# mimbres/neural-audio-fp

Hardware: AMD Instinct MI355X
Metric: fingerprint generation throughput (1-s segments/s) (higher is better)
Workload: dtype f32

## Files before the change

### include/nafp.h

```cpp
#ifndef NAFP_H
#define NAFP_H

#include <stdint.h>

#ifdef __cplusplus
extern "C" {
#endif

#define NAFP_ABI_VERSION 1

enum {
    NAFP_OK = 0,
    NAFP_ERR_INVALID_ARG = 1,
    NAFP_ERR_UNSUPPORTED = 2,
    NAFP_ERR_HIP = 3,
    NAFP_ERR_WORKSPACE = 4,
    NAFP_ERR_NO_WEIGHTS = 5
};

typedef struct nafp_melspec nafp_melspec;
typedef struct nafp_encoder nafp_encoder;

int nafp_abi_version(void);
const char* nafp_status_string(int status);
// ... 162 lines not shown
    int64_t n_indexed;
    int64_t indexed_samples;
    int32_t rate, channels, bps, min_block, max_block, refusal;
    uint8_t md5[16];
} nafp_flac_info;

typedef struct nafp_flac_index_entry {
    int64_t offset;
    int64_t first_sample;
    int64_t n_bytes;
    int32_t block_size;
    int32_t reserved;
} nafp_flac_index_entry;

typedef struct nafp_flac_frame {
    int64_t raw_off;
    int64_t scratch_off;
    int32_t n_bytes;
    int32_t block_size;
    int32_t channels;
    int32_t bps;
    int32_t rate;
    int32_t reserved;
} nafp_flac_frame;

int nafp_flac_streaminfo_host(const void* bytes, int64_t n_bytes, nafp_flac_info* info);
int nafp_flac_index_host(const void* bytes, int64_t n_bytes, nafp_flac_info* info, nafp_flac_index_entry* frames_out, int64_t cap);
int nafp_flac_decode_host(const void* raw, int64_t raw_size, const nafp_flac_frame* frames_host, int64_t n_frames, void* scratch,
                          int64_t scratch_size, int32_t* status_out);
int nafp_flac_check_frames_host(const nafp_flac_frame* frames_host, int64_t n_frames, int64_t raw_size, int64_t scratch_size);
int nafp_flac_decode(const uint8_t* raw, int64_t raw_size, const nafp_flac_frame* frames_dev, int64_t n_frames, uint8_t* scratch,
                     int64_t scratch_size, int32_t* status_dev, void* stream);


int nafp_encoder_create(nafp_encoder** enc, int in_f, int in_t, int emb_sz);
int nafp_encoder_destroy(nafp_encoder* enc);

#define NAFP_NORM_LAYER2D 0
#define NAFP_NORM_LAYER1D 1
#define NAFP_NORM_BATCH 2
int nafp_encoder_create_ex(nafp_encoder** enc, int in_f, int in_t, int emb_sz, int norm);
int nafp_encoder_norm(const nafp_encoder* enc);
int nafp_encoder_n_trainable(const nafp_encoder* enc);

int nafp_encoder_n_tensors(const nafp_encoder* enc);
int64_t nafp_encoder_tensor_numel(const nafp_encoder* enc, int index);
int nafp_encoder_tensor_shape(const nafp_encoder* enc, int index, int64_t dims_out[4]);
int64_t nafp_encoder_flat_dim(const nafp_encoder* enc);

int nafp_encoder_set_weights(nafp_encoder* enc, const float* const* tensors_host_array,
                             void* stream);

int64_t nafp_encoder_workspace_bytes(const nafp_encoder* enc, int64_t n_seg);

int nafp_encoder_forward(nafp_encoder* enc, const float* feat, int64_t n_seg,
                         void* workspace, int64_t workspace_bytes,
                         float* out_flat, float* out_emb, int l2norm, void* stream);

int nafp_encoder_forward_raw(nafp_encoder* enc, const float* raw_feat, const float* group_stat, int group_size,
                             int segment_norm, int64_t n_seg, void* workspace, int64_t workspace_bytes,
                             float* out_flat, float* out_emb, int l2norm, void* stream);

int64_t nafp_encoder_conv0_numel(const nafp_encoder* enc);
int nafp_encoder_conv0(nafp_encoder* enc, const float* feat, const float* group_stat, int group_size, int segment_norm,
                       int64_t n_seg, float* z0_out, long long* stats_out, void* stream);

#define NAFP_ENCODER_PROFILE_KERNELS 17
int nafp_encoder_profile_enable(nafp_encoder* enc, int max_forwards);
int nafp_encoder_profile_count(const nafp_encoder* enc);
int nafp_encoder_profile_coarse(nafp_encoder* enc, int coarse);
int nafp_encoder_profile_read(nafp_encoder* enc, int slot, float* ms_out_host);
int nafp_conv_timeline(void* dev_buf, int64_t capacity_u64, int cin, int cout, int positions);
int nafp_conv_timeline_grid(int* out5_host);
#define NAFP_CONV_PLAN_FIELDS 30
#define NAFP_PLAN_PLAIN 1
#define NAFP_PLAN_DGRAD 2
#define NAFP_PLAN_V_OUT 4
#define NAFP_PLAN_TICKETS 8
#define NAFP_PLAN_SPLIT_WEIGHTS 16
#define NAFP_PLAN_FUSE0 32
#define NAFP_PLAN_SIZE_DGRAD 64
int nafp_conv_plan(int in_f, int in_t, int layer, int64_t n_seg, int64_t plan_b, int flags, int64_t slab_floats,
                   int64_t* record_host, char* kernel_name_host, int name_capacity);

int64_t nafp_encoder_train_workspace_bytes(const nafp_encoder* enc, int64_t n_seg);
int nafp_encoder_forward_train(nafp_encoder* enc, const float* feat, int64_t n_seg, void* workspace,
                               int64_t workspace_bytes, float* out_emb, int l2norm, void* stream);
int nafp_encoder_backward(nafp_encoder* enc, const float* feat, const float* d_emb, int64_t n_seg,
                          void* workspace, int64_t workspace_bytes, float* const* grads_host_array,
                          int l2norm, void* stream);

#define NAFP_GRAD_GROUPS 4
int nafp_encoder_grad_group_range(const nafp_encoder* enc, int group, int* first_tensor, int* last_tensor);
int nafp_encoder_grad_group_wait(nafp_encoder* enc, int group, void* stream);

#define NAFP_OPT_FUSE_CONV0 1
#define NAFP_OPT_FUSED_LN_BWD 2
#define NAFP_OPT_BWD_OVERLAP 4
#define NAFP_OPT_SMALLNET 5
#define NAFP_OPT_BF16X3 3
#define NAFP_OPT_NONMATRIX 8
#define NAFP_NONMATRIX_CONV0 1
#define NAFP_NONMATRIX_KEEP_OWN 2
#define NAFP_NONMATRIX_ALL 3
#define NAFP_NONMATRIX_DEFAULT NAFP_NONMATRIX_ALL
int nafp_encoder_set_option(nafp_encoder* enc, int option, int value);

int nafp_encoder_div_enc(nafp_encoder* enc, const float* flat, int64_t n_seg,
                         float* out_emb, int l2norm, void* stream);

int nafp_l2_normalize_rows(const float* x, int64_t n_rows, int dim, float* out, void* stream);

int nafp_pack_embedding_grads(const float* d_a_all, const float* d_b_all, const float* loss_sum, float loss_scale,
                              int64_t world, int64_t n_anchors, int dim, float* send, void* stream);


int64_t nafp_ntxent_workspace_bytes(int64_t n_local, int64_t n_global);

int nafp_ntxent_forward(const float* emb_org_local, const float* emb_rep_local,
                        const float* emb_org_all, const float* emb_rep_all,
                        int64_t n_local, int64_t n_global, int64_t rank_offset, int d,
                        float tau, float* loss_sum, float* sim_mtx,
                        float* d_org_all, float* d_rep_all,
                        void* workspace, int64_t workspace_bytes, void* stream);


typedef struct { int f0, f1, t0, t1; } nafp_rect;

int nafp_specaug_apply(float* feat, int64_t n_seg, int F, int T, const nafp_rect* rects_host,
                       int n_rects, const unsigned char* active, float fill_value, void* stream);

int nafp_specaug_apply_fill_dev(float* feat, int64_t n_seg, int F, int T, const nafp_rect* rects_host,
                                int n_rects, const unsigned char* active, const float* fill_value_dev,
                                void* stream);
int64_t nafp_specaug_mean_workspace_bytes(void);
int nafp_specaug_mean(const float* feat, int64_t n, float* mean_out, void* workspace, int64_t workspace_bytes,
                      void* stream);

int nafp_specaug_apply_ex(float* feat, int64_t n_seg, int F, int T, const int32_t* rects_dev, int n_rects, int64_t n_sets,
                          const unsigned char* active_dev, const float* filler, int64_t n_fill_seg,
                          const float* scale_offset_dev, void* stream);
int nafp_specaug_range(const float* feat, int64_t n, float* scale_offset_out, void* workspace, int64_t workspace_bytes,
                       void* stream);


typedef struct {
    float* param; const float* grad; float* m; float* v;
    int64_t numel; int64_t var_len;
} nafp_opt_tensor;

float nafp_cosine_decay_lr_host(float lr0, int64_t step, int64_t decay_steps, float alpha);
float nafp_cosine_decay_restarts_lr_host(float lr0, int64_t step, int64_t first_decay_steps, float t_mul,
                                         float m_mul, float alpha);

int nafp_adam_step(const nafp_opt_tensor* tensors_host, int n, float lr, float beta1, float beta2,
                   float eps, int64_t step, void* stream);

int64_t nafp_lamb_workspace_bytes(const nafp_opt_tensor* tensors_host, int n);
int nafp_lamb_step(const nafp_opt_tensor* tensors_host, int n, float lr, float beta1, float beta2,
                   float eps, float weight_decay, int64_t step, void* workspace,
                   int64_t workspace_bytes, void* stream);

int64_t nafp_triplet_workspace_bytes(int64_t n_anchor, int64_t n_pos);
int nafp_triplet_forward(const float* emb_anchor, const float* emb_pos, int64_t n_anchor, int64_t n_pos, int dim,
                         int mode, float margin, float* loss_out, float* pairwise_dist, float* d_anchor,
                         float* d_pos, void* workspace, int64_t workspace_bytes, void* stream);

typedef struct nafp_aug_row {
    int64_t ev_off;
    int64_t nz_off;
    int64_t nz2_off;
    int64_t ir_off;
    int32_t ev_valid;
    int32_t nz_valid, nz2_valid;
    int32_t ir_len;
    float snr_db;
    float amp;
    int32_t mix;
    int32_t reserved;
} nafp_aug_row;

int nafp_augment_rows(const int16_t* pcm, const nafp_aug_row* rows, int64_t n_rows, int seg_len, float* out,
                      void* stream);


int64_t nafp_search_index_aux_floats(int64_t n_index);
int nafp_search_index_prepare(const float* index, int64_t n_index, int dim, float* aux, void* stream);

// ... 134 lines not shown
```

### neural-audio-fp_amd/_lib.py

```python
import ctypes
import os

import torch

_HERE = os.path.dirname(os.path.abspath(__file__))
LIB_PATH = os.environ.get('NAFP_LIB') or os.path.join(_HERE, 'libnafp.so')

c_i64 = ctypes.c_int64
c_int = ctypes.c_int
c_float = ctypes.c_float
c_void_p = ctypes.c_void_p

PROTOTYPES = {
    'nafp_abi_version': (c_int, []),
    'nafp_status_string': (ctypes.c_char_p, [c_int]),
    'nafp_last_hip_error': (c_int, []),
    'nafp_crc32c_host': (ctypes.c_uint32, [c_void_p, c_i64, ctypes.c_uint32]),
    'nafp_mel_filterbank_host': (c_int, [c_int, c_int, c_int, c_float, c_float, c_void_p]),
    'nafp_melspec_create': (c_int, [ctypes.POINTER(c_void_p), c_int, c_int, c_int, c_int, c_int, c_float, c_float]),
    'nafp_melspec_create_ex': (c_int, [ctypes.POINTER(c_void_p), c_int, c_int, c_int, c_int, c_int, c_float, c_float, c_int]),
    'nafp_melspec_plan_host': (c_int, [c_int, c_int, c_int, c_int, c_int, c_float, c_float, c_int, c_void_p]),
    'nafp_melspec_kernel': (c_int, [c_void_p]),
    'nafp_melspec_destroy': (c_int, [c_void_p]),
    'nafp_melspec_n_frames': (c_int, [c_void_p]),
    'nafp_melspec_n_mels': (c_int, [c_void_p]),
    'nafp_melspec_forward_f32': (c_int, [c_void_p, c_void_p, c_i64, c_int, c_int, c_void_p, c_void_p, c_void_p]),
    'nafp_melspec_forward_i16': (c_int, [c_void_p, c_void_p, c_i64, c_int, c_int, c_void_p, c_void_p, c_void_p]),
    'nafp_melspec_finish': (c_int, [c_void_p, c_void_p, c_void_p, c_i64, c_int, c_int, c_void_p]),
    'nafp_melspec_forward_windows_i16': (c_int, [c_void_p, c_void_p, c_void_p, c_void_p, c_i64, c_int, c_int, c_void_p,
                                                 c_void_p, c_void_p]),
    'nafp_resample_geometry': (c_int, [c_int, c_int, ctypes.POINTER(c_int), ctypes.POINTER(c_int), ctypes.POINTER(c_int),
                                       ctypes.POINTER(c_int)]),
    'nafp_resample_table_host': (c_int, [c_int, c_int, c_void_p]),
    'nafp_resample_n_out': (c_i64, [c_i64, c_int, c_int]),
    'nafp_resample_input_range': (c_int, [c_i64, c_i64, c_i64, c_int, c_int, ctypes.POINTER(c_i64), ctypes.POINTER(c_i64)]),
    'nafp_resample_check_pieces_host': (c_int, [c_int, c_int, c_void_p, c_i64, c_i64, c_i64]),
    'nafp_resample_create': (c_int, [ctypes.POINTER(c_void_p), c_int, c_int]),
    'nafp_resample_destroy': (c_int, [c_void_p]),
    'nafp_resample_i16': (c_int, [c_void_p, c_void_p, c_i64, c_void_p, c_i64, c_void_p, c_i64, c_void_p]),
    'nafp_ingest_geometry': (c_int, [c_int, c_int, ctypes.POINTER(c_int), ctypes.POINTER(c_int), ctypes.POINTER(c_int),
                                     ctypes.POINTER(c_int)]),
    'nafp_ingest_table_host': (c_int, [c_int, c_int, c_void_p]),
    'nafp_ingest_n_out': (c_i64, [c_i64, c_int, c_int]),
    'nafp_ingest_input_range': (c_int, [c_i64, c_i64, c_i64, c_int, c_int, ctypes.POINTER(c_i64), ctypes.POINTER(c_i64)]),
    'nafp_ingest_decode_host': (c_int, [c_int, c_void_p, c_i64, c_void_p]),
    'nafp_ingest_check_pieces_host': (c_int, [c_int, c_int, c_void_p, c_i64, c_i64, c_i64]),
    'nafp_ingest_create': (c_int, [ctypes.POINTER(c_void_p), c_int, c_int]),
    'nafp_ingest_destroy': (c_int, [c_void_p]),
    'nafp_ingest_i16': (c_int, [c_void_p, c_void_p, c_i64, c_void_p, c_i64, c_void_p, c_i64, c_void_p]),
    'nafp_varispeed_geometry': (c_int, [ctypes.c_uint32, ctypes.POINTER(c_int), ctypes.POINTER(c_int)]),
    'nafp_varispeed_table_host': (c_int, [ctypes.c_uint32, c_void_p]),
    'nafp_varispeed_n_out': (c_i64, [c_i64, ctypes.c_uint32]),
    'nafp_varispeed_input_range': (c_int, [c_i64, c_i64, c_i64, ctypes.c_uint32, ctypes.POINTER(c_i64), ctypes.POINTER(c_i64)]),
    'nafp_varispeed_check_pieces_host': (c_int, [ctypes.c_uint32, c_void_p, c_i64, c_i64, c_i64]),
    'nafp_varispeed_create': (c_int, [ctypes.POINTER(c_void_p), ctypes.c_uint32]),
    'nafp_varispeed_destroy': (c_int, [c_void_p]),
    'nafp_varispeed_i16': (c_int, [c_void_p, c_void_p, c_i64, c_void_p, c_i64, c_void_p, c_i64, c_void_p]),
    'nafp_codec_samples_per_block': (c_int, [c_int, c_int, c_int]),
    'nafp_codec_blocks_per_group': (c_int, [c_int, c_int, c_int]),
    'nafp_codec_decode_host': (c_int, [c_int, c_int, c_int, c_void_p, c_i64, c_void_p]),
    'nafp_codec_check_pieces_host': (c_int, [c_void_p, c_i64, c_i64, c_i64]),
    'nafp_codec_decode_i16': (c_int, [c_void_p, c_i64, c_void_p, c_i64, c_void_p, c_i64, c_void_p]),
    'nafp_flac_streaminfo_host': (c_int, [c_void_p, c_i64, c_void_p]),
    'nafp_flac_index_host': (c_int, [c_void_p, c_i64, c_void_p, c_void_p, c_i64]),
    'nafp_flac_decode_host': (c_int, [c_void_p, c_i64, c_void_p, c_i64, c_void_p, c_i64, c_void_p]),
    'nafp_flac_check_frames_host': (c_int, [c_void_p, c_i64, c_i64, c_i64]),
    'nafp_flac_decode': (c_int, [c_void_p, c_i64, c_void_p, c_i64, c_void_p, c_i64, c_void_p, c_void_p]),
    'nafp_encoder_create': (c_int, [ctypes.POINTER(c_void_p), c_int, c_int, c_int]),
    'nafp_encoder_create_ex': (c_int, [ctypes.POINTER(c_void_p), c_int, c_int, c_int, c_int]),
    'nafp_encoder_norm': (c_int, [c_void_p]),
    'nafp_encoder_n_trainable': (c_int, [c_void_p]),
    'nafp_encoder_destroy': (c_int, [c_void_p]),
    'nafp_encoder_n_tensors': (c_int, [c_void_p]),
    'nafp_encoder_tensor_numel': (c_i64, [c_void_p, c_int]),
    'nafp_encoder_tensor_shape': (c_int, [c_void_p, c_int, ctypes.POINTER(c_i64)]),
    'nafp_encoder_flat_dim': (c_i64, [c_void_p]),
    'nafp_encoder_set_weights': (c_int, [c_void_p, ctypes.POINTER(c_void_p), c_void_p]),
    'nafp_encoder_workspace_bytes': (c_i64, [c_void_p, c_i64]),
    'nafp_encoder_forward': (c_int, [c_void_p, c_void_p, c_i64, c_void_p, c_i64, c_void_p, c_void_p, c_int, c_void_p]),
    'nafp_encoder_forward_raw': (c_int, [c_void_p, c_void_p, c_void_p, c_int, c_int, c_i64, c_void_p, c_i64, c_void_p, c_void_p,
                                         c_int, c_void_p]),
    'nafp_encoder_conv0_numel': (c_i64, [c_void_p]),
    'nafp_encoder_conv0': (c_int, [c_void_p, c_void_p, c_void_p, c_int, c_int, c_i64, c_void_p, c_void_p, c_void_p]),
    'nafp_encoder_profile_enable': (c_int, [c_void_p, c_int]),
    'nafp_encoder_profile_count': (c_int, [c_void_p]),
    'nafp_encoder_profile_coarse': (c_int, [c_void_p, c_int]),
    'nafp_encoder_profile_read': (c_int, [c_void_p, c_int, c_void_p]),
    'nafp_conv_timeline': (c_int, [c_void_p, c_i64, c_int, c_int, c_int]),
    'nafp_conv_timeline_grid': (c_int, [c_void_p]),
    'nafp_conv_plan': (c_int, [c_int, c_int, c_int, c_i64, c_i64, c_int, c_i64, c_void_p, c_void_p, c_int]),
    'nafp_encoder_set_option': (c_int, [c_void_p, c_int, c_int]),
    'nafp_encoder_train_workspace_bytes': (c_i64, [c_void_p, c_i64]),
    'nafp_encoder_forward_train': (c_int, [c_void_p, c_void_p, c_i64, c_void_p, c_i64, c_void_p, c_int, c_void_p]),
    'nafp_encoder_backward': (c_int, [c_void_p, c_void_p, c_void_p, c_i64, c_void_p, c_i64,
                                      ctypes.POINTER(c_void_p), c_int, c_void_p]),
    'nafp_encoder_grad_group_range': (c_int, [c_void_p, c_int, ctypes.POINTER(c_int), ctypes.POINTER(c_int)]),
    'nafp_encoder_grad_group_wait': (c_int, [c_void_p, c_int, c_void_p]),
    'nafp_encoder_div_enc': (c_int, [c_void_p, c_void_p, c_i64, c_void_p, c_int, c_void_p]),
    'nafp_ntxent_workspace_bytes': (c_i64, [c_i64, c_i64]),
    'nafp_ntxent_forward': (c_int, [c_void_p, c_void_p, c_void_p, c_void_p, c_i64, c_i64, c_i64, c_int,
                                    c_float, c_void_p, c_void_p, c_void_p, c_void_p, c_void_p, c_i64, c_void_p]),
    'nafp_specaug_apply': (c_int, [c_void_p, c_i64, c_int, c_int, c_void_p, c_int, c_void_p, c_float, c_void_p]),
    'nafp_specaug_apply_fill_dev': (c_int, [c_void_p, c_i64, c_int, c_int, c_void_p, c_int, c_void_p, c_void_p, c_void_p]),
    'nafp_specaug_mean_workspace_bytes': (c_i64, []),
    'nafp_specaug_mean': (c_int, [c_void_p, c_i64, c_void_p, c_void_p, c_i64, c_void_p]),
    'nafp_specaug_apply_ex': (c_int, [c_void_p, c_i64, c_int, c_int, c_void_p, c_int, c_i64, c_void_p, c_void_p, c_i64, c_void_p, c_void_p]),
    'nafp_specaug_range': (c_int, [c_void_p, c_i64, c_void_p, c_void_p, c_i64, c_void_p]),
    'nafp_l2_normalize_rows': (c_int, [c_void_p, c_i64, c_int, c_void_p, c_void_p]),
    'nafp_pack_embedding_grads': (c_int, [c_void_p, c_void_p, c_void_p, c_float, c_i64, c_i64, c_int, c_void_p, c_void_p]),
    'nafp_cosine_decay_lr_host': (c_float, [c_float, c_i64, c_i64, c_float]),
    'nafp_cosine_decay_restarts_lr_host': (c_float, [c_float, c_i64, c_i64, c_float, c_float, c_float]),
    'nafp_adam_step': (c_int, [c_void_p, c_int, c_float, c_float, c_float, c_float, c_i64, c_void_p]),
    'nafp_lamb_workspace_bytes': (c_i64, [c_void_p, c_int]),
    'nafp_triplet_workspace_bytes': (c_i64, [c_i64, c_i64]),
    'nafp_triplet_forward': (c_int, [c_void_p, c_void_p, c_i64, c_i64, c_int, c_int, c_float, c_void_p, c_void_p, c_void_p,
                                     c_void_p, c_void_p, c_i64, c_void_p]),
    'nafp_augment_rows': (c_int, [c_void_p, c_void_p, c_i64, c_int, c_void_p, c_void_p]),
    'nafp_search_index_aux_floats': (c_i64, [c_i64]),
    'nafp_search_index_prepare': (c_int, [c_void_p, c_i64, c_int, c_void_p, c_void_p]),
    'nafp_search_workspace_bytes': (c_i64, [c_i64, c_i64, c_int]),
    'nafp_search_topk_l2': (c_int, [c_void_p, c_i64, c_void_p, c_void_p, c_i64, c_int, c_int, c_void_p, c_void_p,
                                    c_void_p, c_i64, c_void_p]),
    'nafp_search_topk_l2_excl': (c_int, [c_void_p, c_i64, c_void_p, c_void_p, c_i64, c_int, c_int, c_void_p, c_void_p, c_void_p,
                                         c_void_p, c_i64, c_void_p]),
    'nafp_search_seq_scores': (c_int, [c_void_p, c_void_p, c_i64, c_int, c_void_p, c_void_p, c_i64, c_void_p, c_int,
                                       c_void_p, c_void_p]),
    'nafp_search_seq_match': (c_int, [c_void_p, c_i64, c_void_p, c_i64, c_int, c_void_p, c_int, c_void_p, c_void_p, c_i64, c_int,
                                      c_int, c_void_p, c_void_p, c_void_p, c_void_p]),
    'nafp_search_identify': (c_int, [c_void_p, c_i64, c_void_p, c_i64, c_int, c_void_p, c_int, c_void_p, c_void_p, c_i64, c_int,
                                     c_void_p, c_int, c_int, c_int, c_int, c_int, c_void_p, c_void_p, c_void_p, c_void_p, c_void_p,
                                     c_void_p, c_void_p]),
    'nafp_search_identify_check_tracks_host': (c_int, [c_void_p, c_int, c_i64]),
    'nafp_search_identify_tempo': (c_int, [c_void_p, c_i64, c_void_p, c_i64, c_int, c_void_p, c_int, c_void_p, c_void_p, c_i64, c_int,
                                           c_void_p, c_int, c_void_p, c_int, c_int, c_int, c_int, c_int, c_void_p, c_void_p, c_void_p,
                                           c_void_p, c_void_p, c_void_p, c_void_p, c_void_p]),
    'nafp_ivf_bucket_workspace_bytes': (c_i64, [c_i64, c_int, c_int]),
    'nafp_ivf_bucket': (c_int, [c_void_p, c_int, c_i64, c_int, c_int, c_void_p, c_void_p, c_void_p, c_i64, c_void_p]),
    'nafp_ivf_kmeans_update': (c_int, [c_void_p, c_i64, c_int, c_int, c_void_p, c_void_p, c_int, c_void_p, c_void_p, c_void_p]),
    'nafp_ivf_residuals': (c_int, [c_void_p, c_i64, c_int, c_void_p, c_void_p, c_void_p, c_void_p]),
    'nafp_ivf_pq_encode': (c_int, [c_void_p, c_i64, c_int, c_void_p, c_void_p, c_void_p, c_int, c_void_p, c_void_p]),
    'nafp_ivf_probe': (c_int, [c_void_p, c_i64, c_void_p, c_int, c_int, c_int, c_void_p, c_void_p]),
    'nafp_ivf_flat_rows_bound': (c_i64, [c_i64, c_int]),
    'nafp_ivf_flat_lists': (c_int, [c_void_p, c_i64, c_int, c_void_p, c_void_p, c_int, c_void_p, c_void_p, c_void_p, c_void_p,
                                    c_void_p]),
    'nafp_ivf_pq_lists': (c_int, [c_void_p, c_i64, c_int, c_void_p, c_void_p, c_void_p]),
    'nafp_ivf_search_workspace_bytes': (c_i64, [c_i64, c_int, c_int, c_int, c_int]),
    'nafp_ivf_flat_search': (c_int, [c_void_p, c_i64, c_void_p, c_int, c_int, c_int, c_void_p, c_void_p, c_void_p, c_void_p, c_int,
                                     c_void_p, c_void_p, c_void_p, c_i64, c_void_p]),
    'nafp_ivf_pq_search': (c_int, [c_void_p, c_i64, c_void_p, c_int, c_int, c_int, c_void_p, c_int, c_void_p, c_void_p, c_void_p,
                                   c_int, c_void_p, c_void_p, c_void_p, c_i64, c_void_p]),
    'nafp_ivf_pq_search_ex': (c_int, [c_void_p, c_i64, c_void_p, c_int, c_int, c_int, c_void_p, c_int, c_void_p, c_void_p, c_void_p,
                                      c_int, c_void_p, c_void_p, c_int, c_void_p, c_i64, c_void_p]),
    'nafp_ivf_pq_adc_tables': (c_int, [c_void_p, c_i64, c_void_p, c_void_p, c_i64, c_void_p, c_int, c_int, c_void_p, c_int, c_int,
                                       c_void_p, c_void_p]),
    'nafp_ivf_pq_residuals': (c_int, [c_void_p, c_i64, c_int, c_void_p, c_int, c_void_p, c_void_p, c_void_p]),
    'nafp_ivf_refine_encode': (c_int, [c_void_p, c_i64, c_int, c_void_p, c_int, c_int, c_int, c_void_p, c_void_p]),
    'nafp_ivf_pq_wide_workspace_bytes': (c_i64, [c_i64, c_int, c_int, c_int]),
    'nafp_ivf_pq_search_wide': (c_int, [c_void_p, c_i64, c_void_p, c_int, c_int, c_int, c_void_p, c_int, c_void_p, c_void_p, c_void_p,
                                        c_int, c_void_p, c_void_p, c_int, c_void_p, c_i64, c_void_p]),
    'nafp_ivf_pqr_rerank': (c_int, [c_void_p, c_i64, c_int, c_void_p, c_int, c_void_p, c_void_p, c_void_p, c_int, c_void_p, c_void_p,
                                    c_int, c_int, c_void_p, c_i64, c_int, c_void_p, c_void_p, c_void_p]),
    'nafp_ivf_pqr_search': (c_int, [c_void_p, c_i64, c_void_p, c_int, c_int, c_int, c_void_p, c_int, c_void_p, c_void_p, c_void_p,
                                    c_void_p, c_void_p, c_void_p, c_int, c_int, c_void_p, c_i64, c_int, c_int, c_void_p, c_void_p,
                                    c_void_p, c_void_p, c_int, c_void_p, c_i64, c_void_p]),
    'nafp_hnsw_default_max_expansions': (c_int, [c_int]),
    'nafp_hnsw_reverse_workspace_bytes': (c_i64, [c_i64, c_i64, c_int, c_int]),
    'nafp_hnsw_search_workspace_bytes': (c_i64, [c_i64, c_int, c_int]),
    'nafp_hnsw_search_layer': (c_int, [c_void_p, c_i64, c_int, c_void_p, c_void_p, c_i64, c_i64, c_int, c_int, c_void_p, c_i64, c_void_p,
                                       c_void_p, c_int, c_int, c_int, c_void_p, c_void_p, c_void_p]),
    'nafp_hnsw_select_forward': (c_int, [c_void_p, c_i64, c_int, c_i64, c_i64, c_void_p, c_int, c_int, c_void_p, c_void_p, c_int, c_void_p,
                                         c_void_p, c_i64, c_i64, c_void_p]),
    'nafp_hnsw_reverse_links': (c_int, [c_void_p, c_i64, c_int, c_i64, c_i64, c_void_p, c_int, c_int, c_void_p, c_void_p, c_i64, c_i64,
                                        c_void_p, c_i64, c_void_p]),
# ... 96 lines not shown
```

### neural-audio-fp_amd/csrc/api.hip

```cpp
#include "nafp_common.h"

#include <algorithm>
#include <cstdio>
#include <cstdlib>
#include <cstring>
#include <vector>

namespace nafp {

thread_local int g_last_hip_error = 0;

static const int kHiddenCh[8] = {128, 128, 256, 256, 512, 512, 1024, 1024};
static const int kStrideT[8] = {2, 2, 2, 2, 1, 2, 1, 2};

std::vector<ConvGeom> encoder_geometry(int in_f, int in_t) {
    std::vector<ConvGeom> g;
    int F = in_f, T = in_t, C = 1;
    for (int i = 0; i < 8; ++i) {
        SamePad pt = same_pad(T, 3, kStrideT[i]);
        g.push_back(ConvGeom{0, F, T, C, F, pt.n_out, kHiddenCh[i], kStrideT[i], pt.before});
        T = pt.n_out; C = kHiddenCh[i];
        SamePad pf = same_pad(F, 3, 2);
        g.push_back(ConvGeom{1, F, T, C, pf.n_out, T, kHiddenCh[i], 2, pf.before});
        F = pf.n_out;
    }
    return g;
}

struct CopyTable { const float* src[96]; float* dst[96]; int64_t n[96]; int nz[96]; int count; int* nonfinite; };
__device__ __forceinline__ float nz_scale(float g) { return fabsf(g) < 1e-30f ? copysignf(1e-30f, g) : g; }
__device__ __forceinline__ bool nonfinite4(float4 v) {
    return !(fabsf(v.x) <= 3.4028234664e38f) || !(fabsf(v.y) <= 3.4028234664e38f) || !(fabsf(v.z) <= 3.4028234664e38f) || !(fabsf(v.w) <= 3.4028234664e38f);
}
__global__ __launch_bounds__(256) void multi_copy_kernel(const CopyTable t) {
    const int e = blockIdx.y;
    const float* __restrict__ s = t.src[e]; float* __restrict__ d = t.dst[e];
    const int64_t n = t.n[e];
    const bool nz = t.nz[e] != 0;
    bool bad = false;
    if ((((uintptr_t)s | (uintptr_t)d) & 15) == 0) {
        for (int64_t i = blockIdx.x * 256ll + threadIdx.x; i < n / 4; i += (int64_t)gridDim.x * 256) {
            float4 v = ((const float4*)s)[i];
            bad = bad || nonfinite4(v);
            if (nz) { v.x = nz_scale(v.x); v.y = nz_scale(v.y); v.z = nz_scale(v.z); v.w = nz_scale(v.w); }
            ((float4*)d)[i] = v;
        }
        for (int64_t i = n / 4 * 4 + blockIdx.x * 256ll + threadIdx.x; i < n; i += (int64_t)gridDim.x * 256) {
            bad = bad || !(fabsf(s[i]) <= 3.4028234664e38f);
            d[i] = nz ? nz_scale(s[i]) : s[i];
        }
    } else {
        for (int64_t i = blockIdx.x * 256ll + threadIdx.x; i < n; i += (int64_t)gridDim.x * 256) {
            bad = bad || !(fabsf(s[i]) <= 3.4028234664e38f);
            d[i] = nz ? nz_scale(s[i]) : s[i];
        }
    }
    if (bad && t.nonfinite) atomicOr(t.nonfinite, 1);
}
#define NAFP_OPT_DEBUG_SIDE_DELAY 6
#define NAFP_OPT_DEBUG_SW_DELAY 7
__global__ void debug_delay_kernel(long long us) {
    const unsigned long long t0 = __builtin_amdgcn_s_memrealtime();
    while ((long long)(__builtin_amdgcn_s_memrealtime() - t0) < us * 100) __builtin_amdgcn_s_sleep(32);
}
struct BiasTable { float* hb[16]; const float* bias[16]; int64_t n[16]; int cout[16]; int count; };
__global__ __launch_bounds__(256) void add_bias_kernel(const BiasTable t) {
    const int e = blockIdx.y;
    float* __restrict__ h = t.hb[e]; const float* __restrict__ b = t.bias[e];
    const int64_t n = t.n[e]; const int C = t.cout[e];
    for (int64_t i = blockIdx.x * 256ll + threadIdx.x; i < n; i += (int64_t)gridDim.x * 256) h[i] += b[i % C];
}

}

using namespace nafp;

constexpr int NAFP_PROF_EV = 34;
struct nafp_encoder {
    int in_f, in_t, emb_sz;
    int norm = NAFP_NORM_LAYER2D;
    int n_trainable = 68;
    std::vector<float*> d_gc, d_bc, d_mm, d_mv;
    bool ln1d_images_set = false;
    std::vector<ConvGeom> geom;
    int64_t flat_dim; int S;
    std::vector<std::vector<int64_t>> shapes;
    float* d_blob = nullptr;
    int64_t blob_floats = 0;
    std::vector<float*> d_w;
    std::vector<float*> d_bias, d_gamma, d_beta;
    std::vector<float*> d_G, d_Hb;
    float *d_w1p = nullptr, *d_b1p = nullptr, *d_w2p = nullptr, *d_b2 = nullptr;
    std::vector<float*> d_wd;
    float *d_w1k = nullptr, *d_b1k = nullptr, *d_w2k = nullptr;
    double* d_inv_n = nullptr;
    int* d_wflag = nullptr;
    float* d_sw_slab = nullptr; int64_t sw_slab_floats = 0;
    bool has_weights = false;
    hipEvent_t sw_copied = nullptr, sw_l1 = nullptr, sw_done = nullptr;
    hipStream_t sw_stream = nullptr;
    bool sw_recorded = false;
    bool opt_fuse_conv0 = []() { const char* v = getenv("NAFP_FUSE0"); return v && v[0] == '1'; }();
    int opt_fused_ln_bwd = []() { const char* v = getenv("NAFP_DGRAD_LN"); return v ? atoi(v) : 0; }();
    int64_t bufA_per_seg = 0, bufB_per_seg = 0;
    std::vector<hipEvent_t> prof_events;
    int prof_max = 0, prof_count = 0;
    int opt_nonmatrix = []() { const char* v = getenv("NAFP_NONMATRIX"); return v ? (int)strtol(v, nullptr, 0) & NAFP_NONMATRIX_ALL : NAFP_NONMATRIX_DEFAULT; }();
    int opt_bf16x3 = 0;
    float* d_x6_blob = nullptr; std::vector<float*> d_whm; std::vector<void*> d_wl; bool x6_dirty = true;
    std::vector<float*> d_wdhm; std::vector<void*> d_wdl;
    int prof_coarse = 0;
    hipEvent_t grad_events[NAFP_GRAD_GROUPS] = {nullptr, nullptr, nullptr, nullptr};
    bool grad_events_valid = false;
    int opt_bwd_overlap = []() { const char* v = getenv("NAFP_BWD_OVERLAP"); return v ? atoi(v) : 2; }();
    bool keep_t_env = []() { const char* v = getenv("NAFP_KEEP_T"); return v && v[0] == '1'; }();
    bool keep_t() const { return keep_t_env || (opt_fused_ln_bwd != 0 && norm == NAFP_NORM_LAYER2D) || norm == NAFP_NORM_LAYER1D; }
    struct TrainRec { const void* ws; int64_t B; bool keep_t; };
    std::vector<TrainRec> train_recs;
    void train_rec_put(const void* ws, int64_t B, bool kt) {
        for (auto& r : train_recs) if (r.ws == ws) { r.B = B; r.keep_t = kt; return; }
        if (train_recs.size() >= 16) train_recs.erase(train_recs.begin());
        train_recs.push_back({ws, B, kt});
    }
    bool train_rec_ok(const void* ws, int64_t B, bool kt) const {
        for (const auto& r : train_recs) if (r.ws == ws) return r.B == B && r.keep_t == kt;
        return false;
    }
    hipStream_t side_stream = nullptr;
    hipEvent_t ev_main[16] = {}, ev_side[16] = {};
    int debug_side_delay_us = 0;
    int debug_sw_delay_us = 0;
    static constexpr int NAFP_SW_STREAMS = 4;
    hipStream_t sw_streams[NAFP_SW_STREAMS] = {};
    hipEvent_t sw_fork = nullptr, sw_join[NAFP_SW_STREAMS] = {};
};

static const int kGroupFirst[NAFP_GRAD_GROUPS] = {48, 32, 16, 0};
static const int kGroupLast[NAFP_GRAD_GROUPS] = {67, 47, 31, 15};

static void profile_free(nafp_encoder* e) {
    for (auto ev : e->prof_events) (void)hipEventDestroy(ev);
    e->prof_events.clear();
    e->prof_max = 0; e->prof_count = 0;
}

static int64_t numel(const std::vector<int64_t>& s) {
    int64_t n = 1;
    for (auto d : s) n *= d;
    return n;
}

extern "C" int nafp_abi_version(void) { return NAFP_ABI_VERSION; }

extern "C" const char* nafp_status_string(int status) {
    switch (status) {
        case NAFP_OK: return "ok";
        case NAFP_ERR_INVALID_ARG: return "invalid argument";
        case NAFP_ERR_UNSUPPORTED: return "unsupported geometry or option";
        case NAFP_ERR_HIP: return "HIP runtime error";
        case NAFP_ERR_WORKSPACE: return "workspace too small";
        case NAFP_ERR_NO_WEIGHTS: return "encoder weights not set";
        default: return "unknown status";
    }
}

extern "C" int nafp_last_hip_error(void) { return g_last_hip_error; }

extern "C" uint32_t nafp_crc32c_host(const void* data, int64_t n, uint32_t crc) {
    static uint32_t T[8][256];
    static bool init = false;
    if (!init) {
        for (uint32_t i = 0; i < 256; ++i) {
            uint32_t c = i;
            for (int k = 0; k < 8; ++k) c = (c >> 1) ^ (0x82F63B78u & (0u - (c & 1u)));
            T[0][i] = c;
        }
        for (uint32_t i = 0; i < 256; ++i)
            for (int t = 1; t < 8; ++t) T[t][i] = (T[t - 1][i] >> 8) ^ T[0][T[t - 1][i] & 0xffu];
        init = true;
    }
    const unsigned char* p = (const unsigned char*)data;
    uint32_t c = ~crc;
    while (n > 0 && ((uintptr_t)p & 7)) { c = (c >> 8) ^ T[0][(c ^ *p++) & 0xffu]; --n; }
    while (n >= 8) {
        uint64_t w; memcpy(&w, p, 8);
        w ^= c;
        c = T[7][w & 0xff] ^ T[6][(w >> 8) & 0xff] ^ T[5][(w >> 16) & 0xff] ^ T[4][(w >> 24) & 0xff] ^
            T[3][(w >> 32) & 0xff] ^ T[2][(w >> 40) & 0xff] ^ T[1][(w >> 48) & 0xff] ^ T[0][(w >> 56) & 0xff];
        p += 8; n -= 8;
    }
// ... 75 lines not shown
        for (int j = 0; j < 16; ++j) inv_n[j] = 1.0 / ((double)e->geom[j].Fout * e->geom[j].Tout * e->geom[j].Cout);
        err = hipMemcpy(e->d_inv_n, inv_n, sizeof(inv_n), hipMemcpyHostToDevice);
        if (err != hipSuccess) { g_last_hip_error = (int)err; (void)hipFree(e->d_blob); delete e; return NAFP_ERR_HIP; }
    }
    for (int j = 0; j < 16; ++j) {
        const ConvGeom& g = e->geom[j];
        const int64_t n = (int64_t)g.Fout * g.Tout * g.Cout;
        if (j % 2 == 0) e->bufA_per_seg = std::max(e->bufA_per_seg, n);
        else            e->bufB_per_seg = std::max(e->bufB_per_seg, n);
    }
    if (norm != NAFP_NORM_LAYER2D) {
        for (int j = 0; j < 16; ++j) { e->shapes[4 * j + 2] = {e->geom[j].Cout}; e->shapes[4 * j + 3] = {e->geom[j].Cout}; }
        if (norm == NAFP_NORM_BATCH)
            for (int j = 0; j < 16; ++j) { e->shapes.push_back({e->geom[j].Cout}); e->shapes.push_back({e->geom[j].Cout}); }
    }
    *out = e;
    return NAFP_OK;
}

extern "C" int nafp_encoder_destroy(nafp_encoder* e) {
    if (!e) return NAFP_OK;
    if (e->d_blob) (void)hipFree(e->d_blob);
    if (e->d_x6_blob) (void)hipFree(e->d_x6_blob);
    profile_free(e);
    for (auto& ev : e->grad_events) if (ev) (void)hipEventDestroy(ev);
    for (auto& ev : e->ev_main) if (ev) (void)hipEventDestroy(ev);
    for (auto& ev : e->ev_side) if (ev) (void)hipEventDestroy(ev);
    if (e->side_stream) (void)hipStreamDestroy(e->side_stream);
    for (auto& q : e->sw_streams) if (q) (void)hipStreamDestroy(q);
    for (auto& ev : e->sw_join) if (ev) (void)hipEventDestroy(ev);
    if (e->sw_fork) (void)hipEventDestroy(e->sw_fork);
    if (e->sw_copied) (void)hipEventDestroy(e->sw_copied);
    if (e->sw_l1) (void)hipEventDestroy(e->sw_l1);
    if (e->sw_done) (void)hipEventDestroy(e->sw_done);
    delete e;
    return NAFP_OK;
}

static int split_weights(nafp_encoder* e, hipStream_t st, int j_lo, int j_hi) {
    SplitTable t; t.count = 0;
    for (int j = j_lo; j <= j_hi; ++j) {
        const int64_t n = (int64_t)e->geom[j].Cout * 3 * e->geom[j].Cin;
        t.wp[t.count] = e->d_w[j]; t.hm[t.count] = e->d_whm[j]; t.wl[t.count] = e->d_wl[j]; t.n8[t.count] = n / 8; t.K[t.count] = 3 * e->geom[j].Cin; ++t.count;
        if (e->geom[j].Cout % 16 == 0 && e->d_wd[j]) {
            t.wp[t.count] = e->d_wd[j]; t.hm[t.count] = e->d_wdhm[j]; t.wl[t.count] = e->d_wdl[j]; t.n8[t.count] = n / 8; t.K[t.count] = 3 * e->geom[j].Cout; ++t.count;
        }
    }
    return launch_split_weights_multi(t, st);
}
static int split_all_weights(nafp_encoder* e, hipStream_t st) {
    { int rcs = split_weights(e, st, 1, 15); if (rcs != NAFP_OK) return rcs; }
    e->x6_dirty = false;
    return NAFP_OK;
}

extern "C" int nafp_encoder_set_option(nafp_encoder* e, int option, int value) {
    if (!e) return NAFP_ERR_INVALID_ARG;
    switch (option) {
        case NAFP_OPT_FUSE_CONV0: e->opt_fuse_conv0 = value != 0; return NAFP_OK;
        case NAFP_OPT_BF16X3:
            if (value < 0 || value > 2) return NAFP_ERR_INVALID_ARG;
            if (value == 2 && !e->d_x6_blob) {
                int64_t tot = 0;
                for (int j = 1; j < 16; ++j) tot += 2 * (((int64_t)e->geom[j].Cout * 3 * e->geom[j].Cin * 3 / 2 + 63) / 64 * 64);
                hipError_t er = hipMalloc(&e->d_x6_blob, sizeof(float) * tot);
                if (er != hipSuccess) { g_last_hip_error = (int)er; e->d_x6_blob = nullptr; return NAFP_ERR_HIP; }
                float* q = e->d_x6_blob;
                e->d_whm.assign(16, nullptr); e->d_wl.assign(16, nullptr); e->d_wdhm.assign(16, nullptr); e->d_wdl.assign(16, nullptr);
                for (int j = 1; j < 16; ++j) {
                    const int64_t n = (int64_t)e->geom[j].Cout * 3 * e->geom[j].Cin;
                    e->d_whm[j] = q; e->d_wl[j] = q + n; q += (n * 3 / 2 + 63) / 64 * 64;
                    e->d_wdhm[j] = q; e->d_wdl[j] = q + n; q += (n * 3 / 2 + 63) / 64 * 64;
                }
                e->x6_dirty = true;
            }
            e->opt_bf16x3 = value; return NAFP_OK;
        case NAFP_OPT_FUSED_LN_BWD:
            if (value < 0 || value > 2) return NAFP_ERR_INVALID_ARG;
            e->opt_fused_ln_bwd = value; return NAFP_OK;
        case NAFP_OPT_BWD_OVERLAP: e->opt_bwd_overlap = value < 0 ? 0 : (value > 2 ? 1 : value); return NAFP_OK;
        case NAFP_OPT_NONMATRIX:
            if (value < 0 || (value & ~NAFP_NONMATRIX_ALL)) return NAFP_ERR_INVALID_ARG;
            e->opt_nonmatrix = value; return NAFP_OK;
        case NAFP_OPT_SMALLNET: return NAFP_OK;
        case NAFP_OPT_DEBUG_SIDE_DELAY:
        case NAFP_OPT_DEBUG_SW_DELAY: {
            static const bool hooks = []() { const char* v = getenv("NAFP_TEST_HOOKS"); return v && v[0] == '1'; }();
            if (!hooks) return NAFP_ERR_UNSUPPORTED;
            (option == NAFP_OPT_DEBUG_SIDE_DELAY ? e->debug_side_delay_us : e->debug_sw_delay_us) = value < 0 ? 0 : value; return NAFP_OK;
        }
        default: return NAFP_ERR_INVALID_ARG;
    }
}

extern "C" int nafp_encoder_n_tensors(const nafp_encoder* e) { return e ? (int)e->shapes.size() : -1; }

extern "C" int64_t nafp_encoder_tensor_numel(const nafp_encoder* e, int index) {
    if (!e || index < 0 || index >= (int)e->shapes.size()) return -1;
    return numel(e->shapes[index]);
}

extern "C" int nafp_encoder_tensor_shape(const nafp_encoder* e, int index, int64_t dims_out[4]) {
    if (!e || !dims_out || index < 0 || index >= (int)e->shapes.size()) return -1;
    const auto& s = e->shapes[index];
    for (size_t i = 0; i < s.size(); ++i) dims_out[i] = s[i];
    return (int)s.size();
}

extern "C" int64_t nafp_encoder_flat_dim(const nafp_encoder* e) { return e ? e->flat_dim : -1; }

extern "C" int nafp_encoder_set_weights(nafp_encoder* e, const float* const* t, void* stream) {
    if (!e || !t) return NAFP_ERR_INVALID_ARG;
    for (size_t i = 0; i < e->shapes.size(); ++i)
        if (!t[i]) return NAFP_ERR_INVALID_ARG;
    hipStream_t st = (hipStream_t)stream;
    CopyTable ct; ct.count = 0;
    auto add_copy = [&](const float* src, float* dst, int64_t n, int nz = 0) { ct.src[ct.count] = src; ct.dst[ct.count] = dst; ct.n[ct.count] = n; ct.nz[ct.count] = nz; ++ct.count; };
    add_copy(t[0], e->d_w[0], 3 * e->geom[0].Cout);
    for (int j = 0; j < 16; ++j) {
        const ConvGeom& g = e->geom[j];
        const int64_t nln = (int64_t)g.Fout * g.Tout * g.Cout;
        add_copy(t[4 * j + 1], e->d_bias[j], g.Cout);
        if (e->norm == NAFP_NORM_LAYER2D) {
            add_copy(t[4 * j + 2], e->d_gamma[j], nln, 1);
            add_copy(t[4 * j + 3], e->d_beta[j], nln);
        } else {
            add_copy(t[4 * j + 2], e->d_gc[j], g.Cout);
            add_copy(t[4 * j + 3], e->d_bc[j], g.Cout);
            if (e->norm == NAFP_NORM_BATCH) { add_copy(t[68 + 2 * j], e->d_mm[j], g.Cout); add_copy(t[69 + 2 * j], e->d_mv[j], g.Cout); }
        }
    }
    add_copy(t[64], e->d_w1k, numel(e->shapes[64]));
    add_copy(t[65], e->d_b1k, numel(e->shapes[65]));
    add_copy(t[66], e->d_w2k, numel(e->shapes[66]));
    add_copy(t[67], e->d_b2, e->emb_sz);
    if (!e->sw_copied) {
        NAFP_HIP_CHECK(hipEventCreateWithFlags(&e->sw_copied, hipEventDisableTiming));
        NAFP_HIP_CHECK(hipEventCreateWithFlags(&e->sw_done, hipEventDisableTiming));
        NAFP_HIP_CHECK(hipEventCreateWithFlags(&e->sw_l1, hipEventDisableTiming));
    }
    e->sw_recorded = false;
    NAFP_HIP_CHECK(hipMemsetAsync(e->d_wflag, 0, sizeof(int), st));
    ct.nonfinite = e->d_wflag;
    multi_copy_kernel<<<dim3(32, ct.count), 256, 0, st>>>(ct);
    NAFP_LAUNCH_CHECK();
    if (e->norm == NAFP_NORM_LAYER1D && !e->ln1d_images_set) {
        e->ln1d_images_set = true;
        for (int j = 0; j < 16; ++j) {
            const int64_t nln = (int64_t)e->geom[j].Fout * e->geom[j].Tout * e->geom[j].Cout;
            NAFP_HIP_CHECK(hipMemsetD32Async((hipDeviceptr_t)e->d_gamma[j], 0x3f800000, nln, st));
            NAFP_HIP_CHECK(hipMemsetAsync(e->d_beta[j], 0, sizeof(float) * nln, st));
        }
    } else if (e->norm == NAFP_NORM_BATCH) {
        BnExpandTable bx; bx.count = 16;
        for (int j = 0; j < 16; ++j) {
            bx.gamma_c[j] = e->d_gc[j]; bx.beta_c[j] = e->d_bc[j]; bx.mmean[j] = e->d_mm[j]; bx.mvar[j] = e->d_mv[j];
            bx.gamma_pos[j] = e->d_gamma[j]; bx.n[j] = (int64_t)e->geom[j].Fout * e->geom[j].Tout * e->geom[j].Cout; bx.C[j] = e->geom[j].Cout;
        }
        int rcx = launch_bn_expand(bx, st);
        if (rcx != NAFP_OK) return rcx;
    }
    NAFP_HIP_CHECK(hipEventRecord(e->sw_copied, st));
    auto sw_delay = [&]() -> int {
        if (e->debug_sw_delay_us <= 0) return NAFP_OK;
        debug_delay_kernel<<<1, 64, 0, st>>>((long long)e->debug_sw_delay_us);
        NAFP_LAUNCH_CHECK();
// ... 131 lines not shown
                                        int segment_norm, int64_t n_seg, void* workspace, int64_t workspace_bytes,
                                        float* out_flat, float* out_emb, int l2norm, void* stream) {
    if (!group_stat) return NAFP_ERR_INVALID_ARG;
    if (group_size <= 0 || group_size > n_seg) group_size = (int)std::min<int64_t>(n_seg, INT32_MAX);
    return encoder_forward_impl(e, raw_feat, group_stat, group_size, segment_norm & 1, n_seg, workspace, workspace_bytes,
                                out_flat, out_emb, l2norm, stream);
}

extern "C" int64_t nafp_encoder_conv0_numel(const nafp_encoder* e) {
    return e ? (int64_t)e->geom[0].Fout * e->geom[0].Tout * e->geom[0].Cout : -1;
}

extern "C" int nafp_encoder_conv0(nafp_encoder* e, const float* feat, const float* gstat, int group_size, int segment_norm,
                                  int64_t n_seg, float* z0_out, long long* stats_out, void* stream) {
    if (!e || !feat || !z0_out || !stats_out || n_seg < 0) return NAFP_ERR_INVALID_ARG;
    if (!e->has_weights) return NAFP_ERR_NO_WEIGHTS;
    if (n_seg == 0) return NAFP_OK;
    hipStream_t st = (hipStream_t)stream;
    { int wrc = wait_weights(e, st); if (wrc != NAFP_OK) return wrc; }
    if (gstat && (group_size <= 0 || group_size > n_seg)) group_size = (int)std::min<int64_t>(n_seg, INT32_MAX);
    NAFP_HIP_CHECK(hipMemsetAsync(stats_out, 0, sizeof(stat_t) * 2 * n_seg, st));
    return launch_conv0(feat, e->d_w[0], e->d_bias[0], e->d_gamma[0], z0_out, nullptr, (stat_t*)stats_out, n_seg, e->geom[0], st,
                        gstat, group_size, segment_norm & 1, e->norm != NAFP_NORM_LAYER2D, (e->opt_nonmatrix & NAFP_NONMATRIX_CONV0) != 0);
}

static int encoder_forward_impl(nafp_encoder* e, const float* feat, const float* gstat, int group_size, int segment_norm,
                                int64_t n_seg, void* workspace, int64_t workspace_bytes, float* out_flat,
                                float* out_emb, int l2norm, void* stream) {
    if (!e || !feat || !workspace || n_seg < 0) return NAFP_ERR_INVALID_ARG;
    if (!e->has_weights) return NAFP_ERR_NO_WEIGHTS;
    if (n_seg == 0) return NAFP_OK;
    if (workspace_bytes < nafp_encoder_workspace_bytes(e, n_seg)) return NAFP_ERR_WORKSPACE;
    if (n_seg * e->bufA_per_seg >= ((int64_t)1 << 40)) return NAFP_ERR_UNSUPPORTED;
    hipStream_t st = (hipStream_t)stream;
    char* ws = (char*)align_up((int64_t)(uintptr_t)workspace, 256);
    const int64_t stats_only = align_up((int64_t)sizeof(double) * 2 * 16 * n_seg, 256);
    const int64_t stats_bytes = stats_only + NAFP_TICKET_SLOTS * (int64_t)sizeof(unsigned);
    stat_t* stats = (stat_t*)ws;
    unsigned* tickets = (unsigned*)(ws + stats_only);
    float* bufA = (float*)(ws + stats_bytes);
    float* bufB = (float*)(ws + stats_bytes + align_up((int64_t)sizeof(float) * e->bufA_per_seg * n_seg, 256));
    float* slab = (float*)((char*)bufB + align_up((int64_t)sizeof(float) * e->bufB_per_seg * n_seg, 256));
    const int64_t slab_floats = forward_slab_floats(e, n_seg);
    { int wrc = wait_weights(e, st); if (wrc != NAFP_OK) return wrc; }
    if (e->opt_bf16x3 == 2 && e->x6_dirty) {
        { int rcs = split_all_weights(e, st); if (rcs != NAFP_OK) return rcs; }
        if (!e->sw_done) NAFP_HIP_CHECK(hipEventCreateWithFlags(&e->sw_done, hipEventDisableTiming));
        NAFP_HIP_CHECK(hipEventRecord(e->sw_done, st));
        e->sw_stream = st; e->sw_recorded = true;
    }
    NAFP_HIP_CHECK(hipMemsetAsync(stats, 0, stats_bytes, st));
    hipEvent_t* ev = nullptr;
    if (e->prof_max > 0 && e->prof_count < e->prof_max) ev = e->prof_events.data() + (size_t)NAFP_PROF_EV * e->prof_count++;
    if (ev && e->prof_coarse < 2) NAFP_HIP_CHECK(hipEventRecord(ev[0], st));

    const bool alt = e->norm != NAFP_NORM_LAYER2D;
    auto stats_of = [&](int j) { return stats + 2 * n_seg * j; };
    auto row_pass = [&](float* z, int j) -> int {
        if (e->norm != NAFP_NORM_LAYER1D) return NAFP_OK;
        return launch_ln1d_fwd(z, n_seg * e->geom[j].Fout * e->geom[j].Tout, e->geom[j].Cout, e->d_gc[j], e->d_bc[j], st);
    };
    static const bool x6_fuse0 = []() { const char* v = getenv("NAFP_X6_FUSE0"); return !v || v[0] != '0'; }();
    const bool fuse0 = !alt && (e->opt_fuse_conv0 || (e->opt_bf16x3 == 2 && x6_fuse0)) && e->geom[1].axis == 1 && e->geom[1].Cin % 16 == 0 &&
                       e->geom[0].Tin <= 64 && (e->opt_bf16x3 != 2 || e->geom[1].Cin == 128);
    int rc = fuse0 ? launch_conv0_stats(feat, e->d_w[0], e->d_bias[0], stats, n_seg, e->geom[0], st, gstat, group_size, segment_norm)
                   : launch_conv0(feat, e->d_w[0], e->d_bias[0], e->d_gamma[0], bufA, nullptr, stats, n_seg, e->geom[0], st,
                                  gstat, group_size, segment_norm, alt, (e->opt_nonmatrix & NAFP_NONMATRIX_CONV0) != 0);
    if (rc != NAFP_OK) return rc;
    if (!fuse0) { rc = row_pass(bufA, 0); if (rc != NAFP_OK) return rc; }
    if (ev && e->prof_coarse < 2) NAFP_HIP_CHECK(hipEventRecord(ev[1], st));
    float* cur = bufA;
    for (int j = 1; j < 16; ++j) {
        float* nxt = (j % 2 == 0) ? bufA : bufB;
        ConvGemmArgs a{};
        a.x = cur; a.stats_in = stats_of(j - 1); a.ident_stats = alt;
        a.wp = e->d_w[j]; a.G = e->d_G[j]; a.Hb = e->d_Hb[j]; a.gamma_out = e->d_gamma[j];
        a.y = nxt; a.stats_out = stats + 2 * n_seg * j; a.plain = false;
        a.slab = slab_floats ? slab : nullptr; a.slab_floats = slab_floats; a.tickets = tickets; a.bf16x3 = e->opt_bf16x3;
        static const int x6_layers = []() { const char* v = getenv("NAFP_X6_LAYERS"); return v ? (int)strtol(v, nullptr, 0) : 0xffff; }();
        if (!((x6_layers >> j) & 1)) a.bf16x3 = 0;
        if (a.bf16x3 == 2) { a.wp_hm = e->d_whm[j]; a.wp_l = e->d_wl[j]; }
        a.plan_b = fwd_plan_b();
        a.nonmatrix = e->opt_nonmatrix;
        if (j == 1 && fuse0) {
            a.x = nullptr; a.f0_feat = feat; a.f0_w = e->d_w[0]; a.f0_bias = e->d_bias[0];
            a.f0_gamma = e->d_gamma[0]; a.f0_geom = &e->geom[0];
            a.f0_gstat = gstat; a.f0_group = group_size; a.f0_segnorm = segment_norm;
        }
        if (ev && e->prof_coarse == 0) { a.ev_start = ev[2 * j]; a.ev_stop = ev[2 * j + 1]; }
        if (ev && e->prof_coarse == 2) {
            if (j == 1) a.ev_start = ev[2];
            if (j == 15) a.ev_stop = ev[31];
        }
        rc = launch_conv_gemm(a, n_seg, e->geom[j], st);
        if (rc != NAFP_OK) return rc;
        rc = row_pass(nxt, j);
        if (rc != NAFP_OK) return rc;
        cur = nxt;
    }
    TailArgs t;
    t.x = cur; t.stats = stats_of(15); t.ident_stats = alt; t.gamma = e->d_gamma[15]; t.beta = e->d_beta[15];
    t.w1p = e->d_w1p; t.b1p = e->d_b1p; t.w2p = e->d_w2p; t.b2 = e->d_b2;
    t.out_flat = out_flat; t.out_emb = out_emb;
    t.D = (int)e->flat_dim; t.Q = e->emb_sz; t.S = e->S; t.l2norm = l2norm; t.nonfinite_weights = e->d_wflag; t.launch_error = nullptr;
    if (ev && e->prof_coarse < 2) NAFP_HIP_CHECK(hipEventRecord(ev[32], st));
    rc = launch_tail(t, n_seg, st);
    if (rc != NAFP_OK) return rc;
    if (ev && e->prof_coarse < 2) NAFP_HIP_CHECK(hipEventRecord(ev[33], st));
    return NAFP_OK;
}

extern "C" int nafp_encoder_profile_enable(nafp_encoder* e, int max_forwards) {
    if (!e || max_forwards < 0 || max_forwards > 4096) return NAFP_ERR_INVALID_ARG;
    profile_free(e);
    for (int i = 0; i < max_forwards * NAFP_PROF_EV; ++i) {
        hipEvent_t ev;
        static const int ev_mode = []() { const char* v = getenv("NAFP_PROF_EVENT_FENCE"); return v ? atoi(v) : 0; }();
        hipError_t err = ev_mode == 1 ? hipEventCreate(&ev)
                         : hipEventCreateWithFlags(&ev, ev_mode == 2 ? hipEventReleaseToDevice : hipEventDisableSystemFence);
        if (err != hipSuccess) { g_last_hip_error = (int)err; profile_free(e); return NAFP_ERR_HIP; }
        e->prof_events.push_back(ev);
    }
    e->prof_max = max_forwards;
    return NAFP_OK;
}

extern "C" int nafp_encoder_profile_coarse(nafp_encoder* e, int coarse) {
    if (!e) return NAFP_ERR_INVALID_ARG;
    e->prof_coarse = coarse < 0 ? 0 : (coarse > 2 ? 2 : coarse);
    return NAFP_OK;
}

extern "C" int nafp_encoder_profile_count(const nafp_encoder* e) { return e ? e->prof_count : -1; }

extern "C" int nafp_encoder_profile_read(nafp_encoder* e, int slot, float* ms_out_host) {
    if (!e || !ms_out_host || slot < 0 || slot >= e->prof_count) return NAFP_ERR_INVALID_ARG;
    hipEvent_t* ev = e->prof_events.data() + (size_t)NAFP_PROF_EV * slot;
    NAFP_HIP_CHECK(hipEventSynchronize(e->prof_coarse == 2 ? ev[31] : ev[33]));
    for (int k = 0; k < 17; ++k) ms_out_host[k] = 0.f;
    if (e->prof_coarse == 2) {
        NAFP_HIP_CHECK(hipEventElapsedTime(ms_out_host + 1, ev[2], ev[31]));
        return NAFP_OK;
    }
    NAFP_HIP_CHECK(hipEventElapsedTime(ms_out_host + 0, ev[0], ev[1]));
    NAFP_HIP_CHECK(hipEventElapsedTime(ms_out_host + 16, ev[32], ev[33]));
    if (e->prof_coarse) {
        NAFP_HIP_CHECK(hipEventElapsedTime(ms_out_host + 1, ev[1], ev[32]));
        return NAFP_OK;
    }
    for (int j = 1; j < 16; ++j) NAFP_HIP_CHECK(hipEventElapsedTime(ms_out_host + j, ev[2 * j], ev[2 * j + 1]));
    return NAFP_OK;
}

extern "C" int nafp_conv_timeline(void* dev_buf, int64_t capacity_u64, int cin, int cout, int positions) {
    if (dev_buf && capacity_u64 <= 0) return NAFP_ERR_INVALID_ARG;
    return conv_timeline_set((unsigned long long*)dev_buf, capacity_u64, cin, cout, positions);
}
extern "C" int nafp_conv_timeline_grid(int* out5_host) {
    if (!out5_host) return NAFP_ERR_INVALID_ARG;
    return conv_timeline_grid(out5_host);
}

extern "C" int nafp_conv_plan(int in_f, int in_t, int layer, int64_t n_seg, int64_t plan_b, int flags, int64_t slab_floats,
                              int64_t* record_host, char* kernel_name_host, int name_capacity) {
    if (in_f <= 0 || in_t <= 0 || layer < 1 || layer > 15 || n_seg <= 0 || plan_b < 0 || slab_floats < 0 || !record_host) return NAFP_ERR_INVALID_ARG;
    const std::vector<ConvGeom> geom = encoder_geometry(in_f, in_t);
    ConvPlanIn in{};
    in.B = n_seg; in.plan_b = plan_b; in.slab_floats = slab_floats;
    in.plain = flags & NAFP_PLAN_PLAIN; in.dgrad = flags & NAFP_PLAN_DGRAD; in.v_out = flags & NAFP_PLAN_V_OUT; in.tickets = flags & NAFP_PLAN_TICKETS;
    in.split_weights = flags & NAFP_PLAN_SPLIT_WEIGHTS; in.bf16x3 = (flags >> 8) & 3;
    in.fuse0 = flags & NAFP_PLAN_FUSE0; in.f0_geom = in.fuse0 ? &geom[0] : nullptr;
    const ConvPlan pl = plan_conv_gemm(in, geom[layer], conv_knobs());
    for (int i = 0; i < NAFP_CONV_PLAN_FIELDS; ++i) record_host[i] = 0;
    record_host[29] = conv_gemm_slab_floats(n_seg, geom[layer], (flags & NAFP_PLAN_SIZE_DGRAD) != 0, plan_b);
    if (pl.rc != NAFP_OK) return pl.rc;
    const ConvKernelRow& row = conv_kernel_rows[pl.kernel];
    const int64_t rec[29] = {pl.kernel, pl.BM, pl.bn, row.ring, pl.lds_bytes, pl.grid.x, pl.grid.y, pl.grid.z, pl.PT, pl.ST, pl.n_sg, pl.n_pb, pl.k_steps,
                             pl.S, pl.finish, pl.finish_f4, pl.finish_grid, pl.mode, row.epi, row.arith, pl.perm_on, pl.perm_n0, pl.perm_c0,
                             pl.opt, pl.xcd_group, pl.xcd_full, pl.log2_ncol, pl.range_step, pl.abl};
    for (int i = 0; i < 29; ++i) record_host[i] = rec[i];
    if (kernel_name_host && name_capacity > 0) snprintf(kernel_name_host, (size_t)name_capacity, "%s", row.name);
    return NAFP_OK;
}

extern "C" int nafp_encoder_div_enc(nafp_encoder* e, const float* flat, int64_t n_seg,
                                    float* out_emb, int l2norm, void* stream) {
    if (!e || !flat || !out_emb || n_seg < 0) return NAFP_ERR_INVALID_ARG;
    if (!e->has_weights) return NAFP_ERR_NO_WEIGHTS;
    TailArgs t;
    t.x = flat; t.stats = nullptr; t.ident_stats = false; t.gamma = nullptr; t.beta = nullptr;
    t.w1p = e->d_w1p; t.b1p = e->d_b1p; t.w2p = e->d_w2p; t.b2 = e->d_b2;
    t.out_flat = nullptr; t.out_emb = out_emb;
    t.D = (int)e->flat_dim; t.Q = e->emb_sz; t.S = e->S; t.l2norm = l2norm; t.nonfinite_weights = e->d_wflag; t.launch_error = nullptr;
    { int wrc = wait_weights(e, (hipStream_t)stream); if (wrc != NAFP_OK) return wrc; }
    return launch_tail(t, n_seg, (hipStream_t)stream);
}


namespace {
struct TrainLayout {
    int64_t B;
    stat_t* stats; unsigned* tickets; float* mr; float* sc;
    char* zero_begin; int64_t zero_bytes;
    double* lnsum[16]; float* S1[16]; float* S2[16];
    float* z[16]; float* v[16];
    float* slab; int64_t slab_floats;
    float* slab2; int64_t slab2_floats; unsigned* tickets2;
    float* dA; float* dB; float* dy;
    float* dts[16];
    float* dgp; float* dbp;
    int64_t bytes;
};

TrainLayout train_layout(const nafp_encoder* e, int64_t B, void* ws) {
    TrainLayout L; L.B = B;
    char* p = (char*)(((uintptr_t)ws + 255) & ~(uintptr_t)255);
    char* p0 = p;
    auto take = [&](int64_t bytes) { char* r = p; p += (bytes + 255) / 256 * 256; return r; };
    L.stats = (stat_t*)take((int64_t)sizeof(stat_t) * 2 * 16 * B);
    L.tickets = (unsigned*)take(2 * NAFP_TICKET_SLOTS * (int64_t)sizeof(unsigned));
    L.tickets2 = L.tickets + NAFP_TICKET_SLOTS;
    L.mr = (float*)take((int64_t)sizeof(float) * 2 * 16 * B);
    L.sc = (float*)take((int64_t)sizeof(float) * 8 * B);
    L.zero_begin = p;
    for (int j = 0; j < 16; ++j) L.lnsum[j] = (double*)take((int64_t)sizeof(double) * 2 * B);
    for (int j = 0; j < 16; ++j) {
        const int64_t n = (int64_t)e->geom[j].Fout * e->geom[j].Tout * e->geom[j].Cout;
        L.S1[j] = (float*)take((int64_t)sizeof(float) * n);
        L.S2[j] = (float*)take((int64_t)sizeof(float) * n);
    }
    L.zero_bytes = p - L.zero_begin;
    int64_t max_n = 0;
    for (int j = 0; j < 16; ++j) {
        const int64_t n = (int64_t)e->geom[j].Fout * e->geom[j].Tout * e->geom[j].Cout;
        max_n = std::max(max_n, n);
        L.z[j] = (float*)take((int64_t)sizeof(float) * n * B);
        L.v[j] = ((j == 0 && e->norm != NAFP_NORM_LAYER1D) || !e->keep_t()) ? nullptr : (float*)take((int64_t)sizeof(float) * n * B);
    }
    L.slab_floats = 0;
    for (int j = 1; j < 16; ++j)
        L.slab_floats = std::max(L.slab_floats, std::max(conv_gemm_slab_floats(B, e->geom[j], true), wgrad_slab_floats(B, e->geom[j])));
    L.slab = (float*)take((int64_t)sizeof(float) * L.slab_floats);
    L.slab2_floats = 0;
    for (int j = 1; j < 16; ++j)
        if (e->geom[j].Fout * e->geom[j].Tout < 16) L.slab2_floats = std::max(L.slab2_floats, wgrad_slab_floats(B, e->geom[j]));
    L.slab2 = (float*)take((int64_t)sizeof(float) * L.slab2_floats);
    L.dA = (float*)take((int64_t)sizeof(float) * max_n * B);
    L.dB = (float*)take((int64_t)sizeof(float) * max_n * B);
    L.dy = (float*)take((int64_t)sizeof(float) * e->emb_sz * B);
    for (int j = 0; j < 16; ++j) {
        const int64_t n = (int64_t)e->geom[j].Fout * e->geom[j].Tout * e->geom[j].Cout;
        L.dts[j] = (j >= 1 && e->geom[j].Fout * e->geom[j].Tout < 16) ? (float*)take((int64_t)sizeof(float) * n * B) : nullptr;
    }
    L.dgp = nullptr; L.dbp = nullptr;
// ... 265 lines not shown
```

### neural-audio-fp_amd/csrc/conv.hip

```cpp
#include "nafp_common.h"
#include <hip/hip_ext.h>

#include <cstdlib>

namespace nafp {

using f32x16 = __attribute__((ext_vector_type(16))) float;
using f32x2 = __attribute__((ext_vector_type(2))) float;
#ifndef NAFP_Z_AUX
#define NAFP_Z_AUX 0
#endif
#ifndef NAFP_T_AUX
#define NAFP_T_AUX 2
#endif
__device__ __forceinline__ int f2i(float x) { return __builtin_bit_cast(int, x); }

__device__ __forceinline__ f32x2 elu2(f32x2 t) {
    const f32x2 m = t * 1.44269504088896341f;
    f32x2 e;
    e.x = fminf(fmaxf(__builtin_amdgcn_exp2f(m.x), 0.f), 1.f);
    e.y = fminf(fmaxf(__builtin_amdgcn_exp2f(m.y), 0.f), 1.f);
    e = e - 1.0f;
    f32x2 r;
    r.x = fmaxf(t.x, e.x); r.y = fmaxf(t.y, e.y);
// ... 372 lines not shown
    u32x4 r;
    r.x = __builtin_amdgcn_readfirstlane((unsigned)a);
    r.y = __builtin_amdgcn_readfirstlane((unsigned)(a >> 32) & 0xffffu);
    r.z = __builtin_amdgcn_readfirstlane(bytes);
    r.w = 0x00020000u;
    return r;
}

__device__ __forceinline__ void lds_dma16(unsigned lds_addr, unsigned voff, u32x4 rsrc, unsigned soff) {
    unsigned keep;
    lds_addr = __builtin_amdgcn_readfirstlane(lds_addr);
    soff = __builtin_amdgcn_readfirstlane(soff);
    asm volatile("s_mov_b32 %0, m0\n\ts_mov_b32 m0, %1\n\ts_nop 4\n\t"
                 "buffer_load_dwordx4 %2, %3, %4 offen lds\n\ts_mov_b32 m0, %0"
                 : "=&s"(keep) : "s"(lds_addr), "v"(voff), "s"(rsrc), "s"(soff) : "memory");
}

struct RowGeom { int inner; unsigned mask; };
__device__ __forceinline__ RowGeom row_geom(const ConvKernelParams& p, int pos) {
    const int fo = pos / p.Tout, to = pos - fo * p.Tout;
    RowGeom g; g.mask = 0;
    if (!p.dgrad) {
        int pos0, lim;
        if (p.axis == 0) { pos0 = to * p.stride - p.pad; lim = p.Tin; g.inner = (fo * p.Tin + pos0) * p.Cin; }
        else             { pos0 = fo * p.stride - p.pad; lim = p.Fin; g.inner = (pos0 * p.Tin + to) * p.Cin; }
#pragma unroll
        for (int t = 0; t < 3; ++t)
            if (pos0 + t >= 0 && pos0 + t < lim) g.mask |= 1u << t;
    } else {
        const int u = (p.axis == 0 ? to : fo) + p.pad;
        const int n_out = p.axis == 0 ? p.Tin : p.Fin;
        const int S = p.axis == 0 ? p.Cin : p.Tin * p.Cin;
        const int A0 = p.axis == 0 ? (fo * p.Tin) * p.Cin : to * p.Cin;
        const int sh = p.stride == 2 ? 1 : 0;
        g.inner = A0 + ((u * S) >> sh);
#pragma unroll
        for (int k = 0; k < 3; ++k) {
            const int d = u - k;
            if (d >= 0 && (d & sh) == 0 && (d >> sh) < n_out) g.mask |= 1u << k;
        }
    }
    return g;
}

__device__ __forceinline__ int tile_pos(const ConvKernelParams& p, int idx) {
    if (!p.perm_on || idx >= p.P) return idx;
    if (p.perm_on == 2) {
        const int L = p.Tout, lines = p.P / L, n0 = L - 1;
        if (idx < lines * n0) { const int line = idx / n0; return line * L + (idx - line * n0); }
        return (idx - lines * n0) * L + n0;
    }
    const int n0 = p.perm_n0;
    if (p.axis == 0) {
        const int L = p.Tout, lines = p.P / L, n1 = L - n0;
        if (idx < lines * n0) { const int line = idx / n0; return line * L + 2 * (idx - line * n0) + p.perm_c0; }
        const int j = idx - lines * n0, line = j / n1;
        return line * L + 2 * (j - line * n1) + 1 - p.perm_c0;
    }
    if (idx < n0 * p.Tout) { const int e = idx / p.Tout; return (2 * e + p.perm_c0) * p.Tout + (idx - e * p.Tout); }
    const int j = idx - n0 * p.Tout, e = j / p.Tout;
    return (2 * e + 1 - p.perm_c0) * p.Tout + (j - e * p.Tout);
}

__device__ __forceinline__ float half_wave_sum_dpp(float x) {
    int v = __builtin_bit_cast(int, x);
#define NAFP_DPP_ADD(ctrl_, rmask_)                                                                       \
    v = __builtin_bit_cast(int, __builtin_bit_cast(float, v) +                                            \
                                    __builtin_bit_cast(float, __builtin_amdgcn_update_dpp(0, v, ctrl_, rmask_, 0xf, true)));
    NAFP_DPP_ADD(0x111, 0xf)
    NAFP_DPP_ADD(0x112, 0xf)
    NAFP_DPP_ADD(0x114, 0xf)
    NAFP_DPP_ADD(0x118, 0xf)
    NAFP_DPP_ADD(0x142, 0xa)
#undef NAFP_DPP_ADD
    return __builtin_bit_cast(float, v);
}

#ifndef NAFP_EXP_X6_NOSPLIT
#define NAFP_EXP_X6_NOSPLIT 0
#endif
#ifndef NAFP_EXP_SKIP_TAP2
#define NAFP_EXP_SKIP_TAP2 0
#endif
template <int BM, int BNT, int BK, int NSTAGE, bool FUSE0, int EPI, int PREC = 0>
__device__ __forceinline__ bool conv_gemm_body(const ConvKernelParams& p) {
    static_assert(!FUSE0 || (BK == 16 && BM == 128), "the in-kernel conv0 generator is written for BK = 16, BM = 128");
    static_assert(BM == 128 || BM == 256, "tile rows");
    static_assert(BNT == 128 || (BNT == 64 && BM == 128 && !FUSE0), "tile columns");
    constexpr int NIW = BNT / 64;
    constexpr int NT = 2 * BM;
    constexpr int NW = BM / 32;
    constexpr int CH = BK / 4;
    constexpr int RPI = 64 / CH;
    constexpr int NI = 32 / RPI;
    constexpr int BROWS = BNT / NW;
    constexpr int NIB = BROWS / RPI;
    static_assert(NIB >= 1, "B rows per wave");
    constexpr int TILE = (FUSE0 && PREC == 2) ? BM * 24 : BM * BK;
    constexpr int TILEB = BNT * BK;
    constexpr int LROWS = BNT / NW;
    constexpr int TILEL = PREC == 2 ? BNT * 8 : 0;
    constexpr int STAGE = TILE + TILEB + TILEL;
    constexpr int NDMA = NI + NIB + (PREC == 2 ? 1 : 0);
    extern __shared__ __attribute__((aligned(16))) float smem[];
    float* sRB = smem + NSTAGE * STAGE;
    float* sCB = sRB + BM;
    int* sPos = (int*)(sCB + BM);
    int* sInner = sPos + 32;
    unsigned* sMask = (unsigned*)(sPos + 64);
    float* sW0 = sCB + BM + 96;
    const int tid = threadIdx.x, lane = tid & 63;
    const int wave = __builtin_amdgcn_readfirstlane(tid >> 6);
    const int wm = wave >> 1, wn = wave & 1;
    int sg = blockIdx.x, pb = blockIdx.y, colz = blockIdx.z, zsp = 0;
    if (p.opt & 8) {
        const unsigned lin = blockIdx.x, G = (unsigned)p.xcd_group;
        unsigned v = lin;
        if (lin < (unsigned)p.xcd_full) {
            const unsigned xcd = lin & 7u, j = lin >> 3;
            const unsigned blk = j / G, i = j - blk * G;
            v = (blk * 8u + xcd) * G + i;
        }
        unsigned rt;
        if (p.opt & 16) {
            const unsigned n_rt = (unsigned)(p.n_sg * p.n_pb);
            unsigned t = v / n_rt; rt = v - t * n_rt;
            if (p.n_split > 1) { const unsigned c = t / (unsigned)p.n_split; zsp = (int)(t - c * (unsigned)p.n_split); t = c; }
            colz = (int)t;
        } else {
            colz = (int)(v & ((1u << p.log2_ncol) - 1u)); v >>= p.log2_ncol;
            if (p.n_split > 1) { const unsigned r = v / (unsigned)p.n_split; zsp = (int)(v - r * (unsigned)p.n_split); v = r; }
            rt = v;
        }
        pb = (int)(rt / (unsigned)p.n_sg); sg = (int)(rt - (unsigned)pb * (unsigned)p.n_sg);
    } else
    if (!(p.opt & 4)) { pb = blockIdx.x / p.n_sg; sg = blockIdx.x - pb * p.n_sg; colz = blockIdx.y; zsp = blockIdx.z; }
    if ((EPI == 3 || EPI == 5) && p.sj.sc) {
        const long long wg = blockIdx.x + (long long)gridDim.x * (blockIdx.y + (long long)gridDim.y * blockIdx.z);
        const long long n_wg = (long long)gridDim.x * gridDim.y * gridDim.z;
        for (long long b = wg * NT + tid; b < p.sj.B; b += n_wg * NT) {
            const float mean = p.sj.mr[2 * b], rstd = p.sj.mr[2 * b + 1];
            float* o = p.sj.sc + 8 * b;
            o[0] = mean; o[1] = rstd;
            o[2] = (float)(p.sj.lnsum[2 * b] * p.sj.inv_n); o[3] = (float)(p.sj.lnsum[2 * b + 1] * p.sj.inv_n);
            o[4] = 1.f / rstd;
            o[5] = p.sj.mr_prev ? p.sj.mr_prev[2 * b + 1] : 1.f;
            o[6] = p.sj.mr_prev ? -p.sj.mr_prev[2 * b] : 0.f;
            o[7] = 0.f;
        }
    }
    const int tile_n0 = colz * BNT;
    const int K = 3 * p.Cin;
#define NAFP_TL(k_)                                                                            \
    if (p.tl && lane == 0)                                                                                 \
        p.tl[(((size_t)blockIdx.x + (size_t)gridDim.x * (blockIdx.y + (size_t)gridDim.y * blockIdx.z)) * 8 + wave) * 8 + (k_)] = \
            __builtin_readcyclecounter();
    if (p.tl && lane == 0)
        p.tl[(((size_t)blockIdx.x + (size_t)gridDim.x * (blockIdx.y + (size_t)gridDim.y * blockIdx.z)) * 8 + wave) * 8] =
            (unsigned long long)__builtin_amdgcn_s_getreg(0xF804) |
            ((unsigned long long)__builtin_amdgcn_s_getreg(0xF814) << 32);
    NAFP_TL(1)
    if (p.opt & 1) __builtin_amdgcn_s_setprio(3);
    const int ST1 = p.ST - 1;
    const int b0 = sg * p.ST;
    const int nb = min(p.ST, p.B - b0);

    const bool stat_thread = tid >= 64 && tid < 64 + p.ST;
    double st_sum = 0.0, st_sq = 0.0;
    if (stat_thread && p.mode != 1 && b0 + tid - 64 < p.B) {
        st_sum = stat_get(p.stats_in + 2 * (int64_t)(b0 + tid - 64));
        st_sq = stat_get(p.stats_in + 2 * (int64_t)(b0 + tid - 64) + 1);
        if (st_sq != st_sq && p.stats_out) stat_poison(p.stats_out + 2 * (int64_t)(b0 + tid - 64));
    }
    if (tid < 32) {
        int pos = p.P, inner = 0; unsigned mask = 0;
        if (tid < p.PT) {
            pos = tile_pos(p, pb * p.PT + tid);
            if (pos < p.P) { const RowGeom rg = row_geom(p, pos); inner = rg.inner; mask = rg.mask; }
        }
        sPos[tid] = pos; sInner[tid] = inner; sMask[tid] = mask;
    }
    __syncthreads();

    constexpr unsigned OOB = 0x80000000u;
    unsigned voffA[NI];
    unsigned vmaskA[NI];
    unsigned voffB[NIB];
#pragma unroll
    for (int q = 0; q < NIB; ++q) {
        const int lr = wave * BROWS + q * RPI + lane / CH;
        const int pc = lane % CH;
        const int swz = BK == 32 ? ((lr >> 1) & 7) : ((lr >> 2) & 3);
        voffB[q] = (unsigned)((tile_n0 + lr) * K + (pc ^ swz) * 4) * 4u;
    }
#pragma unroll
    for (int q = 0; q < NI; ++q) {
        const int lr = wave * 32 + q * RPI + lane / CH;
        const int pc = lane % CH;
        const int swz = BK == 32 ? ((lr >> 1) & 7) : ((lr >> 2) & 3);
        const int lc = pc ^ swz;
        const int slot_q = lr >> p.log2ST;
        const int sl = lr & ST1;
        voffA[q] = 0; vmaskA[q] = 0;
        if (sPos[slot_q] < p.P && sl < nb) {
            voffA[q] = (unsigned)(sl * (int)p.sample_in + sInner[slot_q] + lc * 4) * 4u;
            vmaskA[q] = sMask[slot_q];
        }
    }
    float x0[3][3];
    unsigned g_valid = 0;
    int g_off = 0;
    const int g_row = tid >> 1, g_ch = (tid & 1) * 8;
    const int g_swz = (g_row >> 2) & 3;
    if (FUSE0) {
        for (int i = tid; i < 4 * p.Cin; i += NT) sW0[i] = i < 3 * p.Cin ? p.f0_w[i] : p.f0_bias[i - 3 * p.Cin];
#pragma unroll
        for (int t = 0; t < 3; ++t) { x0[t][0] = 0.f; x0[t][1] = 0.f; x0[t][2] = 0.f; }
        const int pos = pb * p.PT + (g_row >> p.log2ST);
        const int sl = g_row & ST1;
        if (pos < p.P && sl < nb) {
            float f0_gmax = 0.f, f0_nh = 0.f, f0_nd = 1.f;
            if (p.f0_gstat) {
                const int64_t gi = p.f0_group > 0 ? (int64_t)(b0 + sl) / p.f0_group : 0;
                f0_gmax = p.f0_gstat[2 * gi];
                if (p.f0_segnorm) { const float mn = fmaxf(p.f0_gstat[2 * gi + 1] - f0_gmax, -80.f); f0_nh = mn / 2.f; f0_nd = fabsf(f0_nh + 1e-10f); }
            }
            const int fo = pos / p.Tout, to = pos - fo * p.Tout;
            const int f00 = fo * p.stride - p.pad;
            g_off = (f00 * p.Tin + to) * p.Cin;
            const int t00 = to * p.f0_stride - p.f0_pad;
            const float* fb = p.f0_feat + ((int64_t)(b0 + sl) * p.Fin) * p.f0_T;
#pragma unroll
            for (int t = 0; t < 3; ++t) {
                const int f = f00 + t;
                if (f >= 0 && f < p.Fin) {
                    g_valid |= 1u << t;
#pragma unroll
                    for (int k = 0; k < 3; ++k) {
                        const int tt = t00 + k;
                        float xv = 0.f;
                        if (tt >= 0 && tt < p.f0_T) {
                            xv = fb[(int64_t)f * p.f0_T + tt];
                            if (p.f0_gstat) {
                                xv = max_keep_nan(xv - f0_gmax, -80.f);
                                if (p.f0_segnorm) xv = (xv - f0_nh) / f0_nd;
                            }
                        }
                        x0[t][k] = xv;
                    }
                }
            }
        }
        __syncthreads();
    }
    unsigned live = 0;
    {
        const unsigned m = sMask[lane & 31];
#pragma unroll
        for (int t = 0; t < 3; ++t)
            if (__ballot((m >> t) & 1u) != 0ull) live |= 1u << t;
    }
    unsigned tap_pack = 0; int n_live = 0;
#pragma unroll
    for (int t = 0; t < 3; ++t)
        if (live & (1u << t)) { tap_pack |= (unsigned)t << (2 * n_live); ++n_live; }
    const int cpt = p.Cin / BK;
    const int n_steps_all = n_live * cpt;
    int s_begin = 0, n_steps = n_steps_all;
    if (p.n_split > 1) {
        s_begin = (int)((unsigned)(n_steps_all * zsp) / (unsigned)p.n_split);
        n_steps = (int)((unsigned)(n_steps_all * (zsp + 1)) / (unsigned)p.n_split);
    }
#define NAFP_STEP_AT(step_, tsel_, c0_)                                                        \
    const int tsel_ = s_begin == 0 ? ((step_) >= cpt ? 1 : 0) : (step_) / cpt;                 \
    const int c0_ = ((step_) - tsel_ * cpt) * BK;

    const u32x4 rsA = make_rsrc(p.x + (int64_t)b0 * p.sample_in,
                                NAFP_ABL(p, 512) ? 0u : (unsigned)nb * (unsigned)p.sample_in * 4u);
    const u32x4 rsB = make_rsrc(PREC == 2 ? p.wp_hm : p.wp, NAFP_ABL(p, 4096) ? 0u : p.wp_bytes);
    const unsigned lds0 = (unsigned)(unsigned long long)(lds_ptr_t)smem + (unsigned)(wave * 32 * BK * 4);
    const unsigned ldsB0 = (unsigned)(unsigned long long)(lds_ptr_t)smem + (unsigned)((TILE + wave * BROWS * BK) * 4);
    const u32x4 rsL = make_rsrc((const float*)p.wp_l, NAFP_ABL(p, 4096) ? 0u : p.wp_bytes / 2);
    const unsigned ldsL0 = (unsigned)(unsigned long long)(lds_ptr_t)smem + (unsigned)((TILE + TILEB) * 4 + wave * LROWS * 32);
    const unsigned voffL = (unsigned)((tile_n0 + wave * LROWS + (lane >> 1)) * K) * 2u + (unsigned)(lane & 1) * 16u;
#define NAFP_DMA_L(slot_, k0_)                                                                 \
    if (PREC == 2 && lane < 2 * LROWS) lds_dma16(ldsL0 + (unsigned)((slot_) * STAGE * 4), voffL, rsL, (unsigned)((k0_) * 2));

#define NAFP_DMA_STEP(s_, slot_)                                                              \
    {                                                                                          \
        NAFP_STEP_AT(s_, tsel_l, c0_l)                                                         \
        const int tap_l = (int)((tap_pack >> (2 * tsel_l)) & 3u);                              \
        const unsigned la_l = lds0 + (unsigned)((slot_) * STAGE * 4);                          \
        const unsigned lb_l = ldsB0 + (unsigned)((slot_) * STAGE * 4);                         \
        const unsigned tapb_l = (unsigned)(tap_l * p.tap_stride) * 4u;                         \
        _Pragma("unroll") for (int q = 0; q < NI; ++q) {                                       \
            const unsigned va = ((vmaskA[q] >> tap_l) & 1u) ? voffA[q] + tapb_l : OOB;         \
            if (!FUSE0) lds_dma16(la_l + q * RPI * BK * 4, va, rsA, (unsigned)(c0_l * 4));     \
            if (q < NIB) lds_dma16(lb_l + q * RPI * BK * 4, voffB[q], rsB,                      \
                                   (unsigned)((tap_l * p.Cin + c0_l) * 4));                    \
        }                                                                                      \
        NAFP_DMA_L(slot_, tap_l * p.Cin + c0_l)                                                \
    }
    float4 gg0 = make_float4(0.f, 0.f, 0.f, 0.f), gg1 = gg0;
#define NAFP_GEN_LOAD(s_)                                                                     \
    {                                                                                          \
        const int tsel_l = (s_) / cpt;                                                         \
        const int tap_l = (int)((tap_pack >> (2 * tsel_l)) & 3u);                              \
        const int c0_l = ((s_) - tsel_l * cpt) * BK;                                           \
        const int go_l = ((g_valid >> tap_l) & 1u) ? g_off + tap_l * p.tap_stride + c0_l + g_ch : 0; \
        gg0 = *(const float4*)(p.f0_gamma + go_l);                                             \
        gg1 = *(const float4*)(p.f0_gamma + go_l + 4);                                         \
    }
#define NAFP_GEN_ONE(j_, G_) \
    __fmul_rn((ok_l ? elu1(fmaf(xc_l, wt_l[2 * p.Cin + (j_)], fmaf(xb_l, wt_l[p.Cin + (j_)], fmaf(xa_l, wt_l[(j_)], wt_l[3 * p.Cin + (j_)])))) : 0.f), (G_))
#define NAFP_GEN_STORE(s_, slot_)                                                             \
    {                                                                                          \
        const int tsel_l = (s_) / cpt;                                                         \
        const int tap_l = (int)((tap_pack >> (2 * tsel_l)) & 3u);                              \
        const int c0_l = ((s_) - tsel_l * cpt) * BK;                                           \
        const bool ok_l = (g_valid >> tap_l) & 1u;                                             \
        const float xa_l = tap_l == 0 ? x0[0][0] : (tap_l == 1 ? x0[1][0] : x0[2][0]);         \
        const float xb_l = tap_l == 0 ? x0[0][1] : (tap_l == 1 ? x0[1][1] : x0[2][1]);         \
        const float xc_l = tap_l == 0 ? x0[0][2] : (tap_l == 1 ? x0[1][2] : x0[2][2]);         \
        const float* wt_l = sW0 + c0_l + g_ch;                                                 \
        float* dst_l = smem + (slot_) * STAGE + g_row * BK;                                    \
        *(float4*)(dst_l + (((2 * (tid & 1)) ^ g_swz) * 4)) = make_float4(                      \
            NAFP_GEN_ONE(0, gg0.x), NAFP_GEN_ONE(1, gg0.y), NAFP_GEN_ONE(2, gg0.z), NAFP_GEN_ONE(3, gg0.w)); \
        *(float4*)(dst_l + (((2 * (tid & 1) + 1) ^ g_swz) * 4)) = make_float4(                  \
            NAFP_GEN_ONE(4, gg1.x), NAFP_GEN_ONE(5, gg1.y), NAFP_GEN_ONE(6, gg1.z), NAFP_GEN_ONE(7, gg1.w)); \
    }

    f32x16 acc[2][NIW];
#pragma unroll
    for (int mi = 0; mi < 2; ++mi)
#pragma unroll
        for (int ni = 0; ni < NIW; ++ni)
#pragma unroll
            for (int r = 0; r < 16; ++r) acc[mi][ni][r] = 0.f;

    NAFP_TL(2)
    if (p.opt & 1) __builtin_amdgcn_s_setprio(0);
#pragma unroll
    for (int s = 0; s < NSTAGE - 1; ++s)
        if (s_begin + s < n_steps) {
            NAFP_DMA_STEP(s_begin + s, s)
            if (FUSE0 && PREC != 2) {
                NAFP_GEN_LOAD(s_begin + s)
                NAFP_GEN_STORE(s_begin + s, s)
            }
        }

    if (stat_thread) {
        float r = 0.f, c = 0.f;
        if (p.mode != 1 && b0 + tid - 64 < p.B) {
            if (p.inv_n_in < 0.0) {
                const double z = st_sq * 0.0;
                r = (float)(1.0 + z); c = (float)z;
            } else {
                const double mean = st_sum * p.inv_n_in;
                double var = st_sq * p.inv_n_in - mean * mean;
                var = var < 0.0 ? 0.0 : var;
                const double rstd = 1.0 / sqrt(var + (double)LN_EPS);
                r = (float)rstd; c = (float)(-mean * rstd);
            }
        }
        sRB[tid - 64] = r; sCB[tid - 64] = c;
    }

    const int rl = lane & 31, hh = lane >> 5;
    const int rswz = BK == 32 ? ((rl >> 1) & 7) : ((rl >> 2) & 3);
    const int aoff = (wm * 64 + rl) * BK, boff = TILE + (wn * (BNT / 2) + rl) * BK;
    const int ncol = lane & 31;
    const int n_base = tile_n0 + wn * (BNT / 2) + ncol;
    const int g4 = p.ST >> 2;
    constexpr int MIL = 1;
    float Gv[MIL][4][NIW], Hv[MIL][4][NIW], gv[MIL][4][NIW];
    const int pc_bytes = p.P * p.Cout * 4;
    const __amdgpu_buffer_rsrc_t rsG = __builtin_amdgcn_make_buffer_rsrc(const_cast<float*>(p.G), 0, pc_bytes, 0x00020000);
    const __amdgpu_buffer_rsrc_t rsH = __builtin_amdgcn_make_buffer_rsrc(const_cast<float*>(p.Hb), 0, pc_bytes, 0x00020000);
    const __amdgpu_buffer_rsrc_t rsg = __builtin_amdgcn_make_buffer_rsrc(const_cast<float*>(p.gamma_out), 0, pc_bytes, 0x00020000);
#define NAFP_EPI_LOAD(mi_, slot_)                                                              \
    _Pragma("unroll") for (int rg = 0; rg < 4; ++rg) {                                         \
        const int grp_l = wm * 16 + (mi_) * 8 + 2 * rg + (lane >> 5);                          \
        const int pos_l = sPos[grp_l >> (p.log2ST - 2)];                \
        const int pofs_l = pos_l < p.P ? (pos_l * p.Cout + n_base) * 4 : (int)0x80000000;      \
        _Pragma("unroll") for (int ni = 0; ni < NIW; ++ni) {                                   \
            if NAFP_ABL(p, 32) { Gv[slot_][rg][ni] = 0.5f; Hv[slot_][rg][ni] = 0.25f; gv[slot_][rg][ni] = 1.5f; continue; } \
            Gv[slot_][rg][ni] = __builtin_bit_cast(float, __builtin_amdgcn_raw_buffer_load_b32(rsG, pofs_l, ni * 128, 0)); \
            Hv[slot_][rg][ni] = __builtin_bit_cast(float, __builtin_amdgcn_raw_buffer_load_b32(rsH, pofs_l, ni * 128, 0)); \
            gv[slot_][rg][ni] = __builtin_bit_cast(float, __builtin_amdgcn_raw_buffer_load_b32(rsg, pofs_l, ni * 128, 0)); \
        }                                                                                      \
    }
    int slot = 0;
    if NAFP_ABL(p, 8) {
        asm volatile("s_waitcnt vmcnt(0)" ::: "memory");
        if (acc[0][0][0] == 12345.678f) p.y[tid] = smem[tid];
        return false;
    }
#define NAFP_LD_FRAG(St_, kk_, a_, b_)                                                         \
    {                                                                                          \
        const int pc4_l = ((2 * (kk_) + hh) ^ rswz) * 4;                                       \
        _Pragma("unroll") for (int mi = 0; mi < 2; ++mi) a_[mi] = *(const float4*)((St_) + aoff + mi * 32 * BK + pc4_l);   \
        _Pragma("unroll") for (int ni = 0; ni < NIW; ++ni) b_[ni] = *(const float4*)((St_) + boff + ni * 32 * BK + pc4_l); \
    }
#define NAFP_MM_FRAG(a_, b_)                                                                   \
    _Pragma("unroll") for (int mi = 0; mi < 2; ++mi)                                           \
        _Pragma("unroll") for (int ni = 0; ni < NIW; ++ni) {                                   \
            acc[mi][ni] = __builtin_amdgcn_mfma_f32_32x32x2f32(a_[mi].x, b_[ni].x, acc[mi][ni], 0, 0, 0); \
            acc[mi][ni] = __builtin_amdgcn_mfma_f32_32x32x2f32(a_[mi].y, b_[ni].y, acc[mi][ni], 0, 0, 0); \
            acc[mi][ni] = __builtin_amdgcn_mfma_f32_32x32x2f32(a_[mi].z, b_[ni].z, acc[mi][ni], 0, 0, 0); \
            acc[mi][ni] = __builtin_amdgcn_mfma_f32_32x32x2f32(a_[mi].w, b_[ni].w, acc[mi][ni], 0, 0, 0); \
        }
#define NAFP_WAIT_STEP(s_)                                                                     \
    if (NSTAGE == 2 || (s_) + NSTAGE - 2 >= n_steps) asm volatile("s_waitcnt vmcnt(0)" ::: "memory"); \
    else asm volatile("s_waitcnt vmcnt(%0)" :: "i"((NSTAGE - 2) * NDMA) : "memory");
    if (!FUSE0 && BK == 16 && !NAFP_ABL(p, 4 | 2048) && s_begin < n_steps) {
        float4 a0[2], b0[NIW], a1[2], b1[NIW];
        NAFP_STEP_AT(s_begin + NSTAGE - 1, d_tsel0, d_c00)
        int d_tsel = d_tsel0, d_c0 = d_c00;
        int d_tap = 0; unsigned d_tapb = 0;
        unsigned cur_va[NI];
#define NAFP_DMA_TAP()                                                                         \
        {                                                                                      \
            d_tap = (int)((tap_pack >> (2 * d_tsel)) & 3u); d_tapb = (unsigned)(d_tap * p.tap_stride) * 4u; \
            _Pragma("unroll") for (int q = 0; q < NI; ++q) cur_va[q] = (((vmaskA[q] >> d_tap) & 1u) && !(NAFP_EXP_SKIP_TAP2 && d_tap == 2)) ? voffA[q] + d_tapb : OOB; \
        }
        NAFP_DMA_TAP()
#define NAFP_DMA_PIECE(q_, slot_)                                                              \
        {                                                                                      \
            lds_dma16(lds0 + (unsigned)((slot_) * STAGE * 4) + (q_) * RPI * BK * 4, cur_va[q_], rsA, (unsigned)(d_c0 * 4)); \
            if ((q_) < NIB) lds_dma16(ldsB0 + (unsigned)((slot_) * STAGE * 4) + (q_) * RPI * BK * 4, voffB[(q_) < NIB ? (q_) : 0], rsB, \
                                      (unsigned)((d_tap * p.Cin + d_c0) * 4));                 \
            if ((q_) == NI - 1) { d_c0 += BK; if (d_c0 == p.Cin) { d_c0 = 0; ++d_tsel; NAFP_DMA_TAP() } } \
        }
#define NAFP_MM_HALF(a_, b_, mi_)                                                              \
        _Pragma("unroll") for (int ni = 0; ni < NIW; ++ni) {                                   \
            acc[mi_][ni] = __builtin_amdgcn_mfma_f32_32x32x2f32(a_[mi_].x, b_[ni].x, acc[mi_][ni], 0, 0, 0); \
            acc[mi_][ni] = __builtin_amdgcn_mfma_f32_32x32x2f32(a_[mi_].y, b_[ni].y, acc[mi_][ni], 0, 0, 0); \
            acc[mi_][ni] = __builtin_amdgcn_mfma_f32_32x32x2f32(a_[mi_].z, b_[ni].z, acc[mi_][ni], 0, 0, 0); \
            acc[mi_][ni] = __builtin_amdgcn_mfma_f32_32x32x2f32(a_[mi_].w, b_[ni].w, acc[mi_][ni], 0, 0, 0); \
        }
        static_assert(NI == 2, "the DMA of a step is issued as two pieces");
        if (PREC >= 1) {
            typedef __bf16 bf16x8 __attribute__((ext_vector_type(8)));
            for (int s = s_begin; s < n_steps; ++s) {
                NAFP_WAIT_STEP(s)
                __builtin_amdgcn_s_barrier();
                if (s == s_begin) { NAFP_TL(3) }
                const bool has_next = s + NSTAGE - 1 < n_steps && !NAFP_ABL(p, 1);
                int nslot = slot + NSTAGE - 1; if (nslot >= NSTAGE) nslot -= NSTAGE;
                const float* St = smem + slot * STAGE;
                float4 af[2][2], bf[PREC == 2 ? 1 : NIW][2];
                bf16x8 ah[2], al[2], bh[NIW], bl[NIW];
                bf16x8 am[PREC == 2 ? 2 : 1], bm[PREC == 2 ? NIW : 1];
#pragma unroll
                for (int c = 0; c < 2; ++c) {
                    const int pc4 = ((2 * hh + c) ^ rswz) * 4;
#pragma unroll
                    for (int mi = 0; mi < 2; ++mi) af[mi][c] = *(const float4*)(St + aoff + mi * 32 * BK + pc4);
                    if (PREC != 2) {
#pragma unroll
                        for (int ni = 0; ni < NIW; ++ni) bf[ni][c] = *(const float4*)(St + boff + ni * 32 * BK + pc4);
                    }
                }
                if (PREC == 2) {
#pragma unroll
                    for (int ni = 0; ni < NIW; ++ni) {
                        bh[ni] = *(const bf16x8*)(St + boff + ni * 32 * BK + ((hh ^ rswz) * 4));
                        bm[ni] = *(const bf16x8*)(St + boff + ni * 32 * BK + (((2 + hh) ^ rswz) * 4));
                        bl[ni] = *(const bf16x8*)(St + TILE + TILEB + (wn * (BNT / 2) + ni * 32 + rl) * 8 + hh * 4);
                    }
                }
                if (has_next) { NAFP_DMA_PIECE(0, nslot) NAFP_DMA_L(nslot, d_tap * p.Cin + d_c0) NAFP_DMA_PIECE(1, nslot) }
#define NAFP_SPLIT8(f_, hi_, mid_, lo_)                                                        \
                {                                                                                  \
                    const float x_l[8] = {f_[0].x, f_[0].y, f_[0].z, f_[0].w, f_[1].x, f_[1].y, f_[1].z, f_[1].w}; \
                    _Pragma("unroll") for (int e = 0; e < 8; ++e) {                                \
                        const __bf16 h_l = (__bf16)x_l[e];                                         \
                        const float r1_l = x_l[e] - (float)h_l;                                    \
                        hi_[e] = h_l;                                                              \
                        if (PREC == 2 && NAFP_EXP_X6_NOSPLIT) {                                    \
                            mid_[e] = h_l; lo_[e] = h_l;       \
                        } else if (PREC == 2) {                                                    \
                            const __bf16 m_l = (__bf16)r1_l;                                       \
                            mid_[e] = m_l; lo_[e] = (__bf16)(r1_l - (float)m_l);                   \
                        } else {                                                                   \
                            lo_[e] = (__bf16)r1_l;                                                 \
                        }                                                                          \
                    }                                                                              \
                }
#define NAFP_SPLIT8_PAIRS(f_, hi_, mid_, lo_)                                                  \
                {                                                                                  \
                    typedef __bf16 bf16x2_l __attribute__((ext_vector_type(2)));                   \
                    typedef float f32x2_l __attribute__((ext_vector_type(2)));                     \
                    typedef unsigned u32x4_l __attribute__((ext_vector_type(4)));                  \
                    const float x_l[8] = {f_[0].x, f_[0].y, f_[0].z, f_[0].w, f_[1].x, f_[1].y, f_[1].z, f_[1].w}; \
                    u32x4_l uh_l, um_l, ul_l;                                                      \
                    _Pragma("unroll") for (int e = 0; e < 4; ++e) {                                \
                        f32x2_l x2; x2.x = x_l[2 * e]; x2.y = x_l[2 * e + 1];                      \
                        const unsigned h2 = __builtin_bit_cast(unsigned, __builtin_convertvector(x2, bf16x2_l)); \
                        f32x2_l r2; r2.x = x2.x - __uint_as_float(h2 << 16); r2.y = x2.y - __uint_as_float(h2 & 0xffff0000u); \
                        const unsigned m2 = __builtin_bit_cast(unsigned, __builtin_convertvector(r2, bf16x2_l)); \
                        f32x2_l t2; t2.x = r2.x - __uint_as_float(m2 << 16); t2.y = r2.y - __uint_as_float(m2 & 0xffff0000u); \
                        uh_l[e] = h2; um_l[e] = m2; ul_l[e] = __builtin_bit_cast(unsigned, __builtin_convertvector(t2, bf16x2_l)); \
                    }                                                                              \
                    hi_ = __builtin_bit_cast(bf16x8, uh_l); mid_ = __builtin_bit_cast(bf16x8, um_l); lo_ = __builtin_bit_cast(bf16x8, ul_l); \
                }
                if (PREC == 2 && !NAFP_EXP_X6_NOSPLIT) {
#pragma unroll
                    for (int mi = 0; mi < 2; ++mi) NAFP_SPLIT8_PAIRS(af[mi], ah[mi], am[PREC == 2 ? mi : 0], al[mi])
                } else {
#pragma unroll
                for (int mi = 0; mi < 2; ++mi) NAFP_SPLIT8(af[mi], ah[mi], am[PREC == 2 ? mi : 0], al[mi])
                }
#undef NAFP_SPLIT8_PAIRS
                if (PREC != 2) {
#pragma unroll
                    for (int ni = 0; ni < NIW; ++ni) NAFP_SPLIT8(bf[PREC == 2 ? 0 : ni], bh[ni], bm[0], bl[ni])
                }
#undef NAFP_SPLIT8
#pragma unroll
                for (int mi = 0; mi < 2; ++mi)
#pragma unroll
                    for (int ni = 0; ni < NIW; ++ni) {
                        if (PREC == 2) {
                            acc[mi][ni] = __builtin_amdgcn_mfma_f32_32x32x16_bf16(al[mi], bh[ni], acc[mi][ni], 0, 0, 0);
                            acc[mi][ni] = __builtin_amdgcn_mfma_f32_32x32x16_bf16(am[PREC == 2 ? mi : 0], bm[PREC == 2 ? ni : 0], acc[mi][ni], 0, 0, 0);
                            acc[mi][ni] = __builtin_amdgcn_mfma_f32_32x32x16_bf16(ah[mi], bl[ni], acc[mi][ni], 0, 0, 0);
                            acc[mi][ni] = __builtin_amdgcn_mfma_f32_32x32x16_bf16(am[PREC == 2 ? mi : 0], bh[ni], acc[mi][ni], 0, 0, 0);
                            acc[mi][ni] = __builtin_amdgcn_mfma_f32_32x32x16_bf16(ah[mi], bm[PREC == 2 ? ni : 0], acc[mi][ni], 0, 0, 0);
                            acc[mi][ni] = __builtin_amdgcn_mfma_f32_32x32x16_bf16(ah[mi], bh[ni], acc[mi][ni], 0, 0, 0);
                        } else {
                            acc[mi][ni] = __builtin_amdgcn_mfma_f32_32x32x16_bf16(al[mi], bh[ni], acc[mi][ni], 0, 0, 0);
                            acc[mi][ni] = __builtin_amdgcn_mfma_f32_32x32x16_bf16(ah[mi], bl[ni], acc[mi][ni], 0, 0, 0);
                            acc[mi][ni] = __builtin_amdgcn_mfma_f32_32x32x16_bf16(ah[mi], bh[ni], acc[mi][ni], 0, 0, 0);
                        }
                    }
                if (++slot == NSTAGE) slot = 0;
            }
        } else {
        {
            NAFP_WAIT_STEP(s_begin)
            __builtin_amdgcn_s_barrier();
            NAFP_TL(3)
            const float* St = smem + slot * STAGE;
            NAFP_LD_FRAG(St, 0, a0, b0)
            NAFP_LD_FRAG(St, 1, a1, b1)
            __builtin_amdgcn_sched_barrier(0);
            if (s_begin + NSTAGE - 1 < n_steps && !NAFP_ABL(p, 1)) { NAFP_DMA_PIECE(0, NSTAGE - 1) NAFP_DMA_PIECE(1, NSTAGE - 1) }
            __builtin_amdgcn_sched_barrier(0);
            NAFP_MM_FRAG(a0, b0)
            __builtin_amdgcn_sched_barrier(0);
            slot = 1;
        }
#define NAFP_K_STEP(SLOT_, NSLOT_)                                                             \
        {                                                                                      \
             \
            asm volatile("s_waitcnt lgkmcnt(0)" ::: "memory");                                 \
            NAFP_WAIT_STEP(s)                                                                  \
            __builtin_amdgcn_s_barrier();                                                      \
            const bool has_next = s + NSTAGE - 1 < n_steps && !NAFP_ABL(p, 1);                 \
            const int nslot = (NSLOT_);                                                        \
            const float* St = smem + (SLOT_) * STAGE;                                          \
            NAFP_LD_FRAG(St, 0, a0, b0)                                                        \
            __builtin_amdgcn_sched_barrier(0);                                                 \
            NAFP_MM_HALF(a1, b1, 0)                                                            \
            __builtin_amdgcn_sched_barrier(0);                                                 \
            if (has_next) { NAFP_DMA_PIECE(0, nslot) }                                         \
            __builtin_amdgcn_sched_barrier(0);                                                 \
            NAFP_MM_HALF(a1, b1, 1)                                                            \
            __builtin_amdgcn_sched_barrier(0);                                                 \
            if (has_next) { NAFP_DMA_PIECE(1, nslot) }                                         \
            NAFP_LD_FRAG(St, 1, a1, b1)                                                        \
            __builtin_amdgcn_sched_barrier(0);                                                 \
            if (s == n_steps - 1) break;           \
            NAFP_MM_FRAG(a0, b0)                                                               \
            __builtin_amdgcn_sched_barrier(0);                                                 \
            ++s;                                                                               \
        }
        static_assert(PREC != 0 || NSTAGE == 3 || BNT == 64, "the K-loop body is written out once per ring slot (128-column tiles)");
        if (s_begin + 1 < n_steps) {
            if (BNT == 128) {
                for (int s = s_begin + 1;;) {
                    NAFP_K_STEP(1, 0)
                    NAFP_K_STEP(2, 1)
                    NAFP_K_STEP(0, 2)
                }
            } else {
                int rs = 1;
                int s = s_begin + 1;
                for (; s < n_steps - 1;) {
                    NAFP_K_STEP(rs, (rs == 0 ? NSTAGE - 1 : rs - 1))
                    if (++rs == NSTAGE) rs = 0;
                }
                do { NAFP_K_STEP(rs, (rs == 0 ? NSTAGE - 1 : rs - 1)) } while (false);
            }
        }
#undef NAFP_K_STEP
        if ((EPI == 0 || EPI == 1) && BM == 128) { NAFP_EPI_LOAD(0, 0) }
        __builtin_amdgcn_sched_barrier(0);
        if (s_begin + 1 < n_steps) { NAFP_MM_FRAG(a0, b0) }
        NAFP_MM_FRAG(a1, b1)
        }
#undef NAFP_DMA_PIECE
#undef NAFP_DMA_TAP
#undef NAFP_MM_HALF
    } else if (FUSE0 && PREC == 2) {
        typedef __bf16 bf16x8 __attribute__((ext_vector_type(8)));
        static_assert(!(FUSE0 && PREC == 2) || NSTAGE == 2, "two ring slots");
        constexpr int C0 = 128;
        const int a_rd = (wm * 64 + rl) * 8 + ((hh ^ ((rl >> 3) & 1)) * 4);
        const int a_wr = g_row * 8 + (((tid & 1) ^ ((g_row >> 3) & 1)) * 4);
        const __amdgpu_buffer_rsrc_t rsG0 = __builtin_amdgcn_make_buffer_rsrc(const_cast<float*>(p.f0_gamma), 0, (int)((unsigned)p.sample_in * 4u), 0x00020000);
        int gvoff0, gvoff1, gvoff2;
        gvoff0 = (g_valid & 1u) ? (g_off + g_ch) * 4 : (int)0x80000000;
        gvoff1 = (g_valid & 2u) ? (g_off + p.tap_stride + g_ch) * 4 : (int)0x80000000;
        gvoff2 = (g_valid & 4u) ? (g_off + 2 * p.tap_stride + g_ch) * 4 : (int)0x80000000;
        const float* wrow = sW0 + g_ch;
        int g_tsel = 0, g_c0 = 0;
        float4 wq[8], gq[2];
        float gxa = 0.f, gxb = 0.f, gxc = 0.f;
#define NAFP_X6_GEN_REQ()                                                                      \
        {                                                                                      \
            const int tap_l = (int)((tap_pack >> (2 * g_tsel)) & 3u);                          \
            gxa = tap_l == 0 ? x0[0][0] : (tap_l == 1 ? x0[1][0] : x0[2][0]);                  \
            gxb = tap_l == 0 ? x0[0][1] : (tap_l == 1 ? x0[1][1] : x0[2][1]);                  \
            gxc = tap_l == 0 ? x0[0][2] : (tap_l == 1 ? x0[1][2] : x0[2][2]);                  \
            const int gv_l = tap_l == 0 ? gvoff0 : (tap_l == 1 ? gvoff1 : gvoff2);             \
            gq[0] = __builtin_bit_cast(float4, __builtin_amdgcn_raw_buffer_load_b128(rsG0, gv_l, g_c0 * 4, 0));      \
            gq[1] = __builtin_bit_cast(float4, __builtin_amdgcn_raw_buffer_load_b128(rsG0, gv_l + 16, g_c0 * 4, 0)); \
            const float* w_l = wrow + g_c0;                                                    \
            _Pragma("unroll") for (int r_ = 0; r_ < 4; ++r_) {                                 \
                wq[2 * r_] = *(const float4*)(w_l + r_ * C0); wq[2 * r_ + 1] = *(const float4*)(w_l + r_ * C0 + 4); \
            }                                                                                  \
            g_c0 += BK; if (g_c0 == C0) { g_c0 = 0; ++g_tsel; }                                \
        }
#define NAFP_X6_GEN_ONE(e_) \
        __fmul_rn(elu1(fmaf(gxc, ((const float*)&wq[4])[e_], fmaf(gxb, ((const float*)&wq[2])[e_], fmaf(gxa, ((const float*)&wq[0])[e_], ((const float*)&wq[6])[e_])))), ((const float*)&gq[0])[e_])
#define NAFP_X6_GEN(slot_)                                                                     \
        {                                                                                      \
            bf16x8 h_l, m_l, l_l;                                                              \
            _Pragma("unroll") for (int e = 0; e < 8; ++e) {                                    \
                const float v_l = NAFP_X6_GEN_ONE(e);                                          \
                const __bf16 hh_l = (__bf16)v_l;                                               \
                const float r1_l = v_l - (float)hh_l;                                          \
                const __bf16 mm_l = (__bf16)r1_l;                                              \
                h_l[e] = hh_l; m_l[e] = mm_l; l_l[e] = (__bf16)(r1_l - (float)mm_l);           \
            }                                                                                  \
            float* dst_l = smem + (slot_) * STAGE + a_wr;                                      \
            *(bf16x8*)dst_l = h_l; *(bf16x8*)(dst_l + BM * 8) = m_l; *(bf16x8*)(dst_l + 2 * BM * 8) = l_l; \
        }
        NAFP_X6_GEN_REQ()
        NAFP_X6_GEN(0)
#define NAFP_X6_MFMAS()                                                                        \
        _Pragma("unroll") for (int mi = 0; mi < 2; ++mi)                                       \
            _Pragma("unroll") for (int ni = 0; ni < NIW; ++ni) {                               \
                acc[mi][ni] = __builtin_amdgcn_mfma_f32_32x32x16_bf16(al[mi], bh[ni], acc[mi][ni], 0, 0, 0); \
                acc[mi][ni] = __builtin_amdgcn_mfma_f32_32x32x16_bf16(am[mi], bm[ni], acc[mi][ni], 0, 0, 0); \
                acc[mi][ni] = __builtin_amdgcn_mfma_f32_32x32x16_bf16(ah[mi], bl[ni], acc[mi][ni], 0, 0, 0); \
                acc[mi][ni] = __builtin_amdgcn_mfma_f32_32x32x16_bf16(am[mi], bh[ni], acc[mi][ni], 0, 0, 0); \
                acc[mi][ni] = __builtin_amdgcn_mfma_f32_32x32x16_bf16(ah[mi], bm[ni], acc[mi][ni], 0, 0, 0); \
                acc[mi][ni] = __builtin_amdgcn_mfma_f32_32x32x16_bf16(ah[mi], bh[ni], acc[mi][ni], 0, 0, 0); \
            }
#define NAFP_X6_READ_FRAGS(St_)                                                                \
        _Pragma("unroll") for (int mi = 0; mi < 2; ++mi) {                                     \
            ah[mi] = *(const bf16x8*)((St_) + a_rd + mi * 32 * 8);                             \
            am[mi] = *(const bf16x8*)((St_) + BM * 8 + a_rd + mi * 32 * 8);                    \
            al[mi] = *(const bf16x8*)((St_) + 2 * BM * 8 + a_rd + mi * 32 * 8);                \
        }                                                                                      \
        _Pragma("unroll") for (int ni = 0; ni < NIW; ++ni) {                                   \
            bh[ni] = *(const bf16x8*)((St_) + boff + ni * 32 * BK + ((hh ^ rswz) * 4));        \
            bm[ni] = *(const bf16x8*)((St_) + boff + ni * 32 * BK + (((2 + hh) ^ rswz) * 4));  \
            bl[ni] = *(const bf16x8*)((St_) + TILE + TILEB + (wn * (BNT / 2) + ni * 32 + rl) * 8 + hh * 4); \
        }
        int s = 0;
        for (; s + 1 < n_steps; ++s) {
            asm volatile("s_waitcnt vmcnt(0) lgkmcnt(0)" ::: "memory");
            __builtin_amdgcn_s_barrier();
            if (s == 0) { NAFP_TL(3) }
            const int nslot = slot ^ 1;
            const float* St = smem + slot * STAGE;
            bf16x8 ah[2], am[2], al[2], bh[NIW], bm[NIW], bl[NIW];
            NAFP_X6_READ_FRAGS(St)
            NAFP_DMA_STEP(s + 1, nslot)
            NAFP_X6_GEN_REQ()
            NAFP_X6_MFMAS()
            NAFP_X6_GEN(nslot)
            slot = nslot;
        }
        {
            asm volatile("s_waitcnt vmcnt(0) lgkmcnt(0)" ::: "memory");
            __builtin_amdgcn_s_barrier();
            const float* St = smem + slot * STAGE;
            bf16x8 ah[2], am[2], al[2], bh[NIW], bm[NIW], bl[NIW];
            NAFP_X6_READ_FRAGS(St)
            NAFP_X6_MFMAS()
        }
#undef NAFP_X6_GEN_REQ
#undef NAFP_X6_GEN_ONE
#undef NAFP_X6_GEN
#undef NAFP_X6_MFMAS
#undef NAFP_X6_READ_FRAGS
    } else
    for (int s = s_begin; s < n_steps; ++s) {
        if (FUSE0) asm volatile("s_waitcnt vmcnt(0) lgkmcnt(0)" ::: "memory");
        else if (NSTAGE == 2 || s + NSTAGE - 2 >= n_steps) asm volatile("s_waitcnt vmcnt(0)" ::: "memory");
        else asm volatile("s_waitcnt vmcnt(%0)" :: "i"((NSTAGE - 2) * (NI + NIB)) : "memory");
        __builtin_amdgcn_s_barrier();
        const bool has_next = s + NSTAGE - 1 < n_steps && !NAFP_ABL(p, 1);
        int nslot = slot + NSTAGE - 1; if (nslot >= NSTAGE) nslot -= NSTAGE;
        const float* St = smem + slot * STAGE;
        if NAFP_ABL(p, 4) {
            if (has_next) { NAFP_DMA_STEP(s + NSTAGE - 1, nslot) }
            if (++slot == NSTAGE) slot = 0;
            continue;
        }
        float4 a0[2], b0[NIW];
        {
            const int pc4 = ((0 + hh) ^ rswz) * 4;
#pragma unroll
            for (int mi = 0; mi < 2; ++mi) a0[mi] = *(const float4*)(St + aoff + mi * 32 * BK + pc4);
#pragma unroll
            for (int ni = 0; ni < NIW; ++ni) b0[ni] = *(const float4*)(St + boff + ni * 32 * BK + pc4);
        }
        if (has_next) {
            NAFP_DMA_STEP(s + NSTAGE - 1, nslot)
            if (FUSE0) NAFP_GEN_LOAD(s + NSTAGE - 1)
        }
#pragma unroll
        for (int kk = 0; kk < BK / 8; ++kk) {
            const int pc4 = ((2 * kk + hh) ^ rswz) * 4;
            float4 a[2], b[NIW];
#pragma unroll
            for (int mi = 0; mi < 2; ++mi) a[mi] = kk == 0 ? a0[mi] : *(const float4*)(St + aoff + mi * 32 * BK + pc4);
#pragma unroll
            for (int ni = 0; ni < NIW; ++ni) b[ni] = kk == 0 ? b0[ni] : *(const float4*)(St + boff + ni * 32 * BK + pc4);
#pragma unroll
            for (int mi = 0; mi < 2; ++mi)
#pragma unroll
                for (int ni = 0; ni < NIW; ++ni) {
                    acc[mi][ni] = __builtin_amdgcn_mfma_f32_32x32x2f32(a[mi].x, b[ni].x, acc[mi][ni], 0, 0, 0);
                    acc[mi][ni] = __builtin_amdgcn_mfma_f32_32x32x2f32(a[mi].y, b[ni].y, acc[mi][ni], 0, 0, 0);
                    acc[mi][ni] = __builtin_amdgcn_mfma_f32_32x32x2f32(a[mi].z, b[ni].z, acc[mi][ni], 0, 0, 0);
                    acc[mi][ni] = __builtin_amdgcn_mfma_f32_32x32x2f32(a[mi].w, b[ni].w, acc[mi][ni], 0, 0, 0);
                }
        }
        if (FUSE0 && has_next) NAFP_GEN_STORE(s + NSTAGE - 1, nslot)
        if (++slot == NSTAGE) slot = 0;
    }
    NAFP_TL(4)
    if (p.opt & 2) __builtin_amdgcn_s_setprio(3);
    asm volatile("s_waitcnt lgkmcnt(0)" ::: "memory");
    __builtin_amdgcn_s_barrier();
    NAFP_TL(5)

    if NAFP_ABL(p, 2) {
// ... 198 lines not shown
#undef NAFP_EPI_MAIN
    NAFP_TL(6)
    if NAFP_ABL(p, 16) {
        if (s2[0].x + s2[0].y + s2[1].x + s2[1].y + q2[0].x + q2[0].y + q2[1].x + q2[1].y == 12345.678f) p.y[tid] = 1.f;
        return false;
    }
    if (fast_stats) {
        double* red = (double*)smem;
        float hs[4], hq[4];
#pragma unroll
        for (int q = 0; q < 4; ++q) { hs[q] = half_wave_sum_dpp(s2[q >> 1][q & 1]); hq[q] = half_wave_sum_dpp(q2[q >> 1][q & 1]); }
        if ((lane & 31) == 31) {
#pragma unroll
            for (int q = 0; q < 4; ++q) {
                red[wave * 16 + (lane >> 5) * 8 + q] = (double)hs[q];
                red[wave * 16 + (lane >> 5) * 8 + 4 + q] = (double)hq[q];
            }
        }
        __syncthreads();
        if (tid < 2 * p.ST) {
            const int which = tid / p.ST, sl = tid - which * p.ST;
            const int b = sg * p.ST + sl;
            if (b < p.B) {
                double t = 0.0;
                if (p.ST == 8) {
#pragma unroll
                    for (int w = 0; w < NW; ++w) t += red[w * 16 + (sl >> 2) * 8 + which * 4 + (sl & 3)];
                } else {
#pragma unroll
                    for (int w = 0; w < NW; ++w) t += red[w * 16 + which * 4 + sl] + red[w * 16 + 8 + which * 4 + sl];
                }
                stat_add(p.stats_out + 2 * (int64_t)b + which, t, p.inv_n_in < 0.0);
            }
        }
    } else {
        __syncthreads();
        if (tid < p.ST) {
            const int b = sg * p.ST + tid;
            if (b < p.B) {
                double ds = 0.0, dq = 0.0;
                for (int pl = 0; pl < p.PT; ++pl) { ds += (double)rowS[pl * p.ST + tid]; dq += (double)rowQ[pl * p.ST + tid]; }
                stat_add(p.stats_out + 2 * (int64_t)b, ds, p.inv_n_in < 0.0);
                stat_add(p.stats_out + 2 * (int64_t)b + 1, dq, p.inv_n_in < 0.0);
            }
        }
    }
    NAFP_TL(7)
#undef NAFP_TL
    return true;
}

#define NAFP_GEMM_KERNEL(name_, BM_, BN_, BK_, NSTAGE_, MINW_, FUSE0_, EPI_)                 \
    __global__ __launch_bounds__(2 * BM_, MINW_) void name_(const ConvKernelParams p) {       \
        conv_gemm_body<BM_, BN_, BK_, NSTAGE_, FUSE0_, EPI_>(p);                              \
    }
#define NAFP_GEMM_KERNEL_BF16X3(name_, BM_, BN_, NSTAGE_, MINW_)                                \
    __global__ __launch_bounds__(2 * BM_, MINW_) void name_(const ConvKernelParams p) {       \
        conv_gemm_body<BM_, BN_, 16, NSTAGE_, false, 0, 1>(p);                                \
    }
#define NAFP_GEMM_KERNEL_BF16X6(name_, BM_, BN_, NSTAGE_, MINW_, EPI_)                          \
    __global__ __launch_bounds__(2 * BM_, MINW_) void name_(const ConvKernelParams p) {       \
        conv_gemm_body<BM_, BN_, 16, NSTAGE_, false, EPI_, 2>(p);                             \
    }
#define NAFP_GEMM_KERNELS(name_, BM_, BN_, MINW_)                                             \
    NAFP_GEMM_KERNEL(name_##_infer, BM_, BN_, 16, 3, MINW_, false, 0)                         \
    NAFP_GEMM_KERNEL(name_##_train, BM_, BN_, 16, 3, MINW_, false, 1)                         \
    NAFP_GEMM_KERNEL(name_##_any, BM_, BN_, 16, 3, MINW_, false, 2)                           \
    NAFP_GEMM_KERNEL(name_##_plain, BM_, BN_, 16, 3, MINW_, false, 3)
NAFP_GEMM_KERNELS(conv_gemm_k16s3, 128, 128, 3)
NAFP_GEMM_KERNEL(conv_gemm_k16s3_fuse0, 128, 128, 16, 3, 3, true, 0)
NAFP_GEMM_KERNEL(conv_gemm_n64k16s3_infer, 128, 64, 16, 3, 4, false, 0)
NAFP_GEMM_KERNEL(conv_gemm_n64k16s3_train, 128, 64, 16, 3, 4, false, 1)
NAFP_GEMM_KERNEL(conv_gemm_n64k16s3_any, 128, 64, 16, 3, 4, false, 2)
NAFP_GEMM_KERNEL(conv_gemm_n64k16s3_plain, 128, 64, 16, 3, 4, false, 3)
NAFP_GEMM_KERNEL(conv_gemm_n64k16s3_splitfin, 128, 64, 16, 3, 4, false, 4)
NAFP_GEMM_KERNEL(conv_gemm_n64k16s3_plainfin, 128, 64, 16, 3, 4, false, 5)
NAFP_GEMM_KERNEL(conv_gemm_k16s3_plainfin, 128, 128, 16, 3, 3, false, 5)
NAFP_GEMM_KERNEL(conv_gemm_n64k16s2_infer, 128, 64, 16, 2, 5, false, 0)
NAFP_GEMM_KERNEL(conv_gemm_n64k16s2_train, 128, 64, 16, 2, 5, false, 1)
NAFP_GEMM_KERNEL(conv_gemm_n64k16s2_splitfin, 128, 64, 16, 2, 5, false, 4)
NAFP_GEMM_KERNEL(conv_gemm_m256k16s3_infer, 256, 128, 16, 3, 4, false, 0)
NAFP_GEMM_KERNEL(conv_gemm_m256k16s3_train, 256, 128, 16, 3, 4, false, 1)
NAFP_GEMM_KERNEL(conv_gemm_m256k16s3_plain, 256, 128, 16, 3, 4, false, 3)

NAFP_GEMM_KERNEL_BF16X3(conv_gemm_k16s3_infer_bf16x3, 128, 128, 3, 3)
NAFP_GEMM_KERNEL_BF16X3(conv_gemm_m256k16s3_infer_bf16x3, 256, 128, 3, 4)
NAFP_GEMM_KERNEL_BF16X3(conv_gemm_n64k16s2_infer_bf16x3, 128, 64, 2, 5)
#ifndef NAFP_X6_K16_NSTAGE
#define NAFP_X6_K16_NSTAGE 2
#endif
#ifndef NAFP_X6_K16_MINW
#define NAFP_X6_K16_MINW 3
#endif
NAFP_GEMM_KERNEL_BF16X6(conv_gemm_k16s3_infer_bf16x6, 128, 128, NAFP_X6_K16_NSTAGE, NAFP_X6_K16_MINW, 0)
NAFP_GEMM_KERNEL_BF16X6(conv_gemm_n64k16s2_infer_bf16x6, 128, 64, 2, 4, 0)
NAFP_GEMM_KERNEL_BF16X6(conv_gemm_k16s3_plain_bf16x6, 128, 128, NAFP_X6_K16_NSTAGE, NAFP_X6_K16_MINW, 3)
NAFP_GEMM_KERNEL_BF16X6(conv_gemm_k16s3_train_bf16x6, 128, 128, NAFP_X6_K16_NSTAGE, NAFP_X6_K16_MINW, 1)
NAFP_GEMM_KERNEL_BF16X6(conv_gemm_n64k16s2_train_bf16x6, 128, 64, 2, 4, 1)
NAFP_GEMM_KERNEL_BF16X6(conv_gemm_k16s3_any_bf16x6, 128, 128, NAFP_X6_K16_NSTAGE, NAFP_X6_K16_MINW, 2)
NAFP_GEMM_KERNEL_BF16X6(conv_gemm_n64k16s2_any_bf16x6, 128, 64, 2, 4, 2)
NAFP_GEMM_KERNEL_BF16X6(conv_gemm_n64k16s2_plain_bf16x6, 128, 64, 2, 4, 3)
__global__ __launch_bounds__(256, 3) void conv_gemm_k16s2_fuse0_bf16x6(const ConvKernelParams p) {
    conv_gemm_body<128, 128, 16, 2, true, 0, 2>(p);
}

#define NAFP_ROW(k_, BM_, bn_, ring_, extra_, epi_, arith_, fuse0_) {k_, #k_, BM_, bn_, ring_, extra_, epi_, arith_, fuse0_},
const ConvKernelRow conv_kernel_rows[] = {
    NAFP_ROW(conv_gemm_k16s3_infer, 128, 128, 3, 0, 0, 0, false)
    NAFP_ROW(conv_gemm_k16s3_train, 128, 128, 3, 0, 1, 0, false)
    NAFP_ROW(conv_gemm_k16s3_any, 128, 128, 3, 0, 2, 0, false)
    NAFP_ROW(conv_gemm_k16s3_plain, 128, 128, 3, 0, 3, 0, false)
    NAFP_ROW(conv_gemm_k16s3_plainfin, 128, 128, 3, 0, 5, 0, false)
    NAFP_ROW(conv_gemm_k16s3_fuse0, 128, 128, 3, 0, 0, 0, true)
    NAFP_ROW(conv_gemm_n64k16s3_infer, 128, 64, 3, 0, 0, 0, false)
    NAFP_ROW(conv_gemm_n64k16s3_train, 128, 64, 3, 0, 1, 0, false)
    NAFP_ROW(conv_gemm_n64k16s3_any, 128, 64, 3, 0, 2, 0, false)
    NAFP_ROW(conv_gemm_n64k16s3_plain, 128, 64, 3, 0, 3, 0, false)
    NAFP_ROW(conv_gemm_n64k16s3_splitfin, 128, 64, 3, 0, 4, 0, false)
    NAFP_ROW(conv_gemm_n64k16s3_plainfin, 128, 64, 3, 0, 5, 0, false)
    NAFP_ROW(conv_gemm_n64k16s2_infer, 128, 64, 2, 0, 0, 0, false)
    NAFP_ROW(conv_gemm_n64k16s2_train, 128, 64, 2, 0, 1, 0, false)
    NAFP_ROW(conv_gemm_n64k16s2_splitfin, 128, 64, 2, 0, 4, 0, false)
    NAFP_ROW(conv_gemm_m256k16s3_infer, 256, 128, 3, 0, 0, 0, false)
    NAFP_ROW(conv_gemm_m256k16s3_train, 256, 128, 3, 0, 1, 0, false)
    NAFP_ROW(conv_gemm_m256k16s3_plain, 256, 128, 3, 0, 3, 0, false)
    NAFP_ROW(conv_gemm_k16s3_infer_bf16x3, 128, 128, 3, 0, 0, 1, false)
    NAFP_ROW(conv_gemm_m256k16s3_infer_bf16x3, 256, 128, 3, 0, 0, 1, false)
    NAFP_ROW(conv_gemm_n64k16s2_infer_bf16x3, 128, 64, 2, 0, 0, 1, false)
    NAFP_ROW(conv_gemm_k16s3_infer_bf16x6, 128, 128, NAFP_X6_K16_NSTAGE, 128 * 8, 0, 2, false)
    NAFP_ROW(conv_gemm_k16s3_train_bf16x6, 128, 128, NAFP_X6_K16_NSTAGE, 128 * 8, 1, 2, false)
    NAFP_ROW(conv_gemm_k16s3_any_bf16x6, 128, 128, NAFP_X6_K16_NSTAGE, 128 * 8, 2, 2, false)
    NAFP_ROW(conv_gemm_k16s3_plain_bf16x6, 128, 128, NAFP_X6_K16_NSTAGE, 128 * 8, 3, 2, false)
    NAFP_ROW(conv_gemm_n64k16s2_infer_bf16x6, 128, 64, 2, 64 * 8, 0, 2, false)
    NAFP_ROW(conv_gemm_n64k16s2_train_bf16x6, 128, 64, 2, 64 * 8, 1, 2, false)
    NAFP_ROW(conv_gemm_n64k16s2_any_bf16x6, 128, 64, 2, 64 * 8, 2, 2, false)
    NAFP_ROW(conv_gemm_n64k16s2_plain_bf16x6, 128, 64, 2, 64 * 8, 3, 2, false)
    NAFP_ROW(conv_gemm_k16s2_fuse0_bf16x6, 128, 128, 2, 128 * 8 + 128 * 8, 0, 2, true)
};
#undef NAFP_ROW
const int conv_kernel_row_count = (int)(sizeof(conv_kernel_rows) / sizeof(conv_kernel_rows[0]));

__global__ __launch_bounds__(256) void split_weights_multi_kernel(const SplitTable t) {
    const float* __restrict__ wp = t.wp[blockIdx.y];
    unsigned short* __restrict__ hm = (unsigned short*)t.hm[blockIdx.y];
    unsigned short* __restrict__ wl = (unsigned short*)t.wl[blockIdx.y];
    const int64_t n8 = t.n8[blockIdx.y];
    const int K = t.K[blockIdx.y];
    typedef unsigned short u16x8 __attribute__((ext_vector_type(8)));
    for (int64_t i8 = blockIdx.x * 256ll + threadIdx.x; i8 < n8; i8 += (int64_t)gridDim.x * 256) {
        const int64_t i = i8 * 8;
        const float4 a = *(const float4*)(wp + i), b = *(const float4*)(wp + i + 4);
        const float x[8] = {a.x, a.y, a.z, a.w, b.x, b.y, b.z, b.w};
        u16x8 vh, vm, vl;
#pragma unroll
        for (int e = 0; e < 8; ++e) {
            const __bf16 h = (__bf16)x[e];
            const float r1 = x[e] - (float)h;
            const __bf16 m = (__bf16)r1;
            vh[e] = __builtin_bit_cast(unsigned short, h);
            vm[e] = __builtin_bit_cast(unsigned short, m);
            vl[e] = __builtin_bit_cast(unsigned short, (__bf16)(r1 - (float)m));
        }
        const int64_t row = i / K;
        const int k = (int)(i - row * K);
        const int64_t base = row * 2 * K + (int64_t)(k >> 4) * 32 + (k & 8);
        *(u16x8*)(hm + base) = vh;
        *(u16x8*)(hm + base + 16) = vm;
        *(u16x8*)(wl + i) = vl;
    }
}

int launch_split_weights_multi(const SplitTable& t, hipStream_t st) {
    if (t.count <= 0) return NAFP_OK;
    int64_t n8_max = 0;
    for (int j = 0; j < t.count; ++j) {
        if (t.K[j] % 16 != 0) return NAFP_ERR_UNSUPPORTED;
        n8_max = std::max(n8_max, t.n8[j]);
    }
    split_weights_multi_kernel<<<dim3((unsigned)std::min<int64_t>((n8_max + 255) / 256, 1024), (unsigned)t.count), 256, 0, st>>>(t);
    NAFP_LAUNCH_CHECK();
    return NAFP_OK;
}

static int launch_variant(const ConvKernelRow& row, int lds, ConvKernelParams p, dim3 grid, hipStream_t st, hipEvent_t ev_start, hipEvent_t ev_stop) {
    NAFP_HIP_CHECK(hipFuncSetAttribute((const void*)row.fn, hipFuncAttributeMaxDynamicSharedMemorySize, lds));
    if (ev_start || ev_stop) {
        void* args[] = {(void*)&p};
        NAFP_HIP_CHECK(hipExtLaunchKernel((const void*)row.fn, grid, dim3(2 * row.BM), args, (size_t)lds, st, ev_start, ev_stop, 0));
    } else {
        row.fn<<<grid, 2 * row.BM, lds, st>>>(p);
    }
    NAFP_LAUNCH_CHECK();
    return NAFP_OK;
}

constexpr int FIN_MAXS = 64;
template <int FIN_F4>
__global__ __launch_bounds__(256) void splitk_finish_kernel(
        const float* __restrict__ slab, int S, const float* __restrict__ G, const float* __restrict__ Hb,
        const float* __restrict__ gamma_out, const stat_t* __restrict__ stats_in,
        stat_t* __restrict__ stats_out, float* __restrict__ y, float* __restrict__ v_out, int B, int P, int Cout,
        double inv_n_in) {
    __shared__ float sR[FIN_MAXS], sC[FIN_MAXS];
    __shared__ float sPart[4][FIN_F4 / 256][2][2];
    __shared__ int sPartB[4][FIN_F4 / 256][2];
    const int tid = threadIdx.x, lane = tid & 63;
    const int c4 = Cout / 4;
    const int64_t total = (int64_t)B * P * c4;
    const int64_t i0 = (int64_t)blockIdx.x * FIN_F4;
    const int64_t i_last = std::min<int64_t>(total, i0 + FIN_F4) - 1;
    const int b_first = (int)((i0 / c4) / P), b_last = (int)((i_last / c4) / P);
    if (tid <= b_last - b_first) {
        const int b = b_first + tid;
        stat_ln_scalars(stats_in + 2 * (int64_t)b, inv_n_in, &sR[tid], &sC[tid]);
        stat_forward_poison(stats_in + 2 * (int64_t)b, stats_out + 2 * (int64_t)b);
    }
    __syncthreads();
    const int64_t slab_stride4 = total;
#pragma unroll 1
    for (int e = 0; e < FIN_F4 / 256; ++e) {
        const int64_t idx = i0 + e * 256 + tid;
        const bool live = idx < total;
        const int64_t ii = live ? idx : i0;
        const int64_t row = ii / c4;
        const int n = (int)(ii - row * c4) * 4;
        const int b = (int)(row / P), pos = (int)(row - (int64_t)b * P);
        const float4* src = (const float4*)slab + ii;
        float4 acc = src[0];
        for (int sp = 1; sp < S; ++sp) {
            const float4 t = src[sp * slab_stride4];
            acc.x += t.x; acc.y += t.y; acc.z += t.z; acc.w += t.w;
        }
        const float4 g4 = *(const float4*)(G + (int64_t)pos * Cout + n);
        const float4 h4 = *(const float4*)(Hb + (int64_t)pos * Cout + n);
        const float4 go = *(const float4*)(gamma_out + (int64_t)pos * Cout + n);
        const float rb = sR[b - b_first], cb = sC[b - b_first];
        float4 tq, v;
        tq.x = fmaf(rb, acc.x, fmaf(cb, g4.x, h4.x));
        tq.y = fmaf(rb, acc.y, fmaf(cb, g4.y, h4.y));
        tq.z = fmaf(rb, acc.z, fmaf(cb, g4.z, h4.z));
        tq.w = fmaf(rb, acc.w, fmaf(cb, g4.w, h4.w));
        v.x = elu1(tq.x); v.y = elu1(tq.y); v.z = elu1(tq.z); v.w = elu1(tq.w);
        float s = live ? (v.x + v.y) + (v.z + v.w) : 0.f;
        float q = live ? (v.x * v.x + v.y * v.y) + (v.z * v.z + v.w * v.w) : 0.f;
        if (live) {
            ((float4*)y)[idx] = make_float4(v.x * go.x, v.y * go.y, v.z * go.z, v.w * go.w);
            if (v_out) ((float4*)v_out)[idx] = tq;
        }
        const int b_lo = __shfl(b, 0, 64), b_hi = __shfl(b, 63, 64);
        const float s_lo = wave_sum(b == b_lo ? s : 0.f), q_lo = wave_sum(b == b_lo ? q : 0.f);
        const float s_hi = wave_sum(b != b_lo ? s : 0.f), q_hi = wave_sum(b != b_lo ? q : 0.f);
        if (lane == 0) {
            const int w = tid >> 6;
            sPart[w][e][0][0] = s_lo; sPart[w][e][0][1] = q_lo; sPartB[w][e][0] = b_lo;
            sPart[w][e][1][0] = s_hi; sPart[w][e][1][1] = q_hi; sPartB[w][e][1] = b_hi != b_lo ? b_hi : -1;
        }
    }
    __syncthreads();
    if (tid <= b_last - b_first) {
        const int b = b_first + tid;
        double ds = 0.0, dq = 0.0;
        for (int w = 0; w < 4; ++w)
            for (int e = 0; e < FIN_F4 / 256; ++e)
                for (int h = 0; h < 2; ++h)
                    if (sPartB[w][e][h] == b) { ds += (double)sPart[w][e][h][0]; dq += (double)sPart[w][e][h][1]; }
        stat_add(stats_out + 2 * (int64_t)b, ds, inv_n_in < 0.0);
        stat_add(stats_out + 2 * (int64_t)b + 1, dq, inv_n_in < 0.0);
    }
}

__global__ __launch_bounds__(256) void plain_finish_kernel(const float* __restrict__ slab, int S, const float* __restrict__ bias,
                                                          float* __restrict__ y, int64_t n4, int Cout) {
    for (int64_t i = blockIdx.x * 256ll + threadIdx.x; i < n4; i += (int64_t)gridDim.x * 256) {
        float4 acc = ((const float4*)slab)[i];
        for (int sp = 1; sp < S; ++sp) {
            const float4 t = ((const float4*)slab)[i + sp * n4];
            acc.x += t.x; acc.y += t.y; acc.z += t.z; acc.w += t.w;
        }
        if (bias) {
            const float4 bv = *(const float4*)(bias + (4 * i) % Cout);
            acc.x += bv.x; acc.y += bv.y; acc.z += bv.z; acc.w += bv.w;
        }
        ((float4*)y)[i] = acc;
    }
}

static struct { unsigned long long* buf; int64_t capacity; int cin, cout, positions; int last_grid[5]; } g_timeline = {};
int conv_timeline_set(unsigned long long* buf, int64_t capacity_u64, int cin, int cout, int positions) {
    g_timeline.buf = buf; g_timeline.capacity = capacity_u64; g_timeline.cin = cin; g_timeline.cout = cout; g_timeline.positions = positions;
    return NAFP_OK;
}
int conv_timeline_grid(int* out5) { for (int i = 0; i < 5; ++i) out5[i] = g_timeline.last_grid[i]; return NAFP_OK; }

template <int FIN_F4>
static void launch_splitk_finish(const ConvGemmArgs& a, const ConvPlan& pl, const ConvKernelParams& p, hipStream_t st) {
    if (a.ev_stop) hipExtLaunchKernelGGL(splitk_finish_kernel<FIN_F4>, dim3(pl.finish_grid), dim3(256), 0, st, nullptr, a.ev_stop, 0, (const float*)a.slab,
                                         pl.S, a.G, a.Hb, a.gamma_out, a.stats_in, a.stats_out, a.y, a.v_out, p.B, p.P, p.Cout, p.inv_n_in);
    else splitk_finish_kernel<FIN_F4><<<pl.finish_grid, 256, 0, st>>>(a.slab, pl.S, a.G, a.Hb, a.gamma_out, a.stats_in, a.stats_out, a.y, a.v_out,
                                                                     p.B, p.P, p.Cout, p.inv_n_in);
}

int launch_conv_gemm(const ConvGemmArgs& a, int64_t B, const ConvGeom& g, hipStream_t st) {
    ConvPlanIn in{};
    in.B = B; in.plan_b = a.plan_b; in.plain = a.plain; in.dgrad = a.dgrad; in.v_out = a.v_out != nullptr; in.tickets = a.tickets != nullptr;
    in.split_weights = a.wp_hm && a.wp_l; in.bf16x3 = a.bf16x3; in.slab_floats = a.slab ? a.slab_floats : 0;
    in.fuse0 = a.f0_feat != nullptr; in.f0_geom = a.f0_geom;
    const ConvPlan pl = plan_conv_gemm(in, g, conv_knobs());
    if (pl.rc != NAFP_OK) return pl.rc;
    const ConvKernelRow& row = conv_kernel_rows[pl.kernel];
    const bool d = a.dgrad, in_kernel = pl.finish == CONV_FINISH_IN_KERNEL_FULL || pl.finish == CONV_FINISH_IN_KERNEL_PLAIN;

    ConvKernelParams p;
    p.x = a.x; p.wp = a.wp; p.G = a.G; p.Hb = a.Hb; p.gamma_out = a.gamma_out; p.bias = a.bias;
    p.wp_hm = row.arith == 2 ? a.wp_hm : nullptr; p.wp_l = row.arith == 2 ? (const unsigned short*)a.wp_l : nullptr;
    p.stats_in = a.stats_in; p.stats_out = a.stats_out; p.y = a.y; p.v_out = a.v_out;
    p.Fin = d ? g.Fout : g.Fin; p.Tin = d ? g.Tout : g.Tin; p.Cin = d ? g.Cout : g.Cin; p.Tout = d ? g.Tin : g.Tout; p.Cout = d ? g.Cin : g.Cout;
    p.axis = g.axis; p.stride = g.stride; p.pad = g.pad;
    p.B = (int)B; p.P = pl.P;
    p.PT = pl.PT; p.ST = pl.ST;
    p.log2ST = 0;
    while ((1 << p.log2ST) < p.ST) ++p.log2ST;
    p.n_sg = pl.n_sg; p.n_pb = pl.n_pb; p.log2_ncol = pl.log2_ncol; p.xcd_group = pl.xcd_group; p.xcd_full = pl.xcd_full;
    p.sample_in = (int64_t)p.Fin * p.Tin * p.Cin;
    p.tap_stride = d ? -((g.axis == 0 ? g.Cout : g.Tout * g.Cout) / g.stride) : (g.axis == 0 ? g.Cin : g.Tin * g.Cin);
    p.inv_n_in = d ? 1.0 : a.ident_stats ? -1.0 : 1.0 / (double)p.sample_in;
    p.mode = pl.mode; p.dgrad = d;
    p.perm_on = pl.perm_on; p.perm_n0 = pl.perm_n0; p.perm_c0 = pl.perm_c0;
    p.wp_bytes = pl.wp_bytes; p.n_split = pl.S; p.abl = pl.abl; p.opt = pl.opt;
    if (pl.S > 1) { p.y = a.slab; p.bias = pl.finish == CONV_FINISH_IN_KERNEL_PLAIN ? a.bias : nullptr; }
    p.tickets = in_kernel ? a.tickets : nullptr; p.y_final = a.y;
    p.keep_own = (a.nonmatrix & NAFP_NONMATRIX_KEEP_OWN) && pl.finish == CONV_FINISH_IN_KERNEL_FULL && pl.S == 2;
    p.f0_feat = nullptr; p.f0_w = nullptr; p.f0_bias = nullptr; p.f0_gamma = nullptr;
    p.f0_T = 0; p.f0_stride = 1; p.f0_pad = 0; p.f0_gstat = nullptr; p.f0_group = 0; p.f0_segnorm = 0;
    if (a.f0_feat) {
        p.f0_feat = a.f0_feat; p.f0_w = a.f0_w; p.f0_bias = a.f0_bias; p.f0_gamma = a.f0_gamma;
        p.f0_T = a.f0_geom->Tin; p.f0_stride = a.f0_geom->stride; p.f0_pad = a.f0_geom->pad;
        p.f0_gstat = a.f0_gstat; p.f0_group = a.f0_group; p.f0_segnorm = a.f0_segnorm;
    }
    p.sj = (a.sj && a.plain) ? *a.sj : ScalarsJob{nullptr, nullptr, nullptr, nullptr, 0, 0.0};
    p.tl = nullptr;
    if (g_timeline.buf && ((!a.plain && !a.dgrad && g.Cin == g_timeline.cin) || (a.dgrad && g.Cin == -g_timeline.cin)) &&
        g.Cout == g_timeline.cout && g.Fout * g.Tout == g_timeline.positions &&
        (int64_t)pl.grid.x * pl.grid.y * pl.grid.z * 64 <= g_timeline.capacity) {
        p.tl = g_timeline.buf;
        g_timeline.last_grid[0] = (int)pl.grid.x; g_timeline.last_grid[1] = (int)pl.grid.y; g_timeline.last_grid[2] = (int)pl.grid.z;
        g_timeline.last_grid[3] = pl.BM; g_timeline.last_grid[4] = pl.bn;
    }

    const bool finish_follows = pl.finish == CONV_FINISH_KERNEL;
    hipEvent_t ev_stop = finish_follows ? nullptr : a.ev_stop;
    if (pl.range_step > 0) {
        const int64_t out_per_sample = (int64_t)p.P * p.Cout;
        int rc = NAFP_OK;
        for (int64_t b0 = 0; b0 < B && rc == NAFP_OK; b0 += pl.range_step) {
            ConvKernelParams q = p;
            const int64_t bc = std::min<int64_t>(pl.range_step, B - b0);
            q.B = (int)bc; q.n_sg = (int)((bc + p.ST - 1) / p.ST);
            q.x = p.x + b0 * p.sample_in; q.y_final = p.y_final + b0 * out_per_sample;
            if (p.v_out) q.v_out = p.v_out + b0 * out_per_sample;
            q.stats_in = p.stats_in + 2 * b0; q.stats_out = p.stats_out + 2 * b0;
            rc = launch_variant(row, pl.lds_bytes, q, dim3((unsigned)((int64_t)q.n_sg * pl.n_pb), pl.grid.y, pl.grid.z), st,
                                b0 == 0 ? a.ev_start : nullptr, b0 + pl.range_step >= B ? ev_stop : nullptr);
        }
        return rc;
    }
    const int rc = launch_variant(row, pl.lds_bytes, p, pl.grid, st, a.ev_start, ev_stop);
    if (rc != NAFP_OK || !finish_follows) return rc;
    if (a.plain) {
        const int64_t n4 = B * p.P * p.Cout / 4;
        if (a.ev_stop) hipExtLaunchKernelGGL(plain_finish_kernel, dim3(pl.finish_grid), dim3(256), 0, st, nullptr, a.ev_stop, 0, (const float*)a.slab, pl.S, a.bias, a.y, n4, p.Cout);
        else plain_finish_kernel<<<pl.finish_grid, 256, 0, st>>>(a.slab, pl.S, a.bias, a.y, n4, p.Cout);
    } else if (pl.finish_f4 == 1024) launch_splitk_finish<1024>(a, pl, p, st);
    else if (pl.finish_f4 == 512) launch_splitk_finish<512>(a, pl, p, st);
    else launch_splitk_finish<256>(a, pl, p, st);
    NAFP_LAUNCH_CHECK();
    return NAFP_OK;
}

struct DgradLnParams {
    ConvKernelParams c;
    const float* t;
    const float* gamma;
    const float* G; const float* Hb;
    const float* sc;
    float* dts;
    float* dgamma; float* dbeta; float* dbias;
    float* S1; float* S2;
    double* lnsum_below;
    int n_groups, groups_per_wg, n_chunks;
};

__global__ __launch_bounds__(256, 3) void dgrad_ln_kernel(const DgradLnParams q) {
// ... 395 lines not shown
```

### neural-audio-fp_amd/csrc/conv_plan.hip

```cpp
#include <algorithm>
#include <climits>

#include "nafp_common.h"

namespace nafp {

constexpr int BN = 128;

const ConvKnobs& conv_knobs() {
    static const ConvKnobs k;
    return k;
}

int64_t fwd_plan_b() { return conv_knobs().plan_b; }

static int live_k_steps(const ConvGeom& g) {
    const int n_in = g.axis == 0 ? g.Tin : g.Fin, n_out = g.axis == 0 ? g.Tout : g.Fout;
    int n_live = 0;
    for (int t = 0; t < 3; ++t) {
        bool live = false;
        for (int o = 0; o < n_out && !live; ++o) { const int i = o * g.stride - g.pad + t; live = i >= 0 && i < n_in; }
        n_live += live;
    }
    return n_live * g.Cin / 16;
// ... 23 lines not shown
        if (S > 1) score *= 0.93;
        if (score > best_score + 1e-9) { best_score = score; best = S; }
    }
    return best;
}

static int tile_pt(int P) {
    int pt = 1;
    while (pt * 2 <= P && pt * 2 <= 32) pt *= 2;
    return pt;
}

struct FwdTile { int pt, perm; double saved; };
static FwdTile fwd_tile(const ConvGeom& g, int BM, const ConvKnobs& knobs) {
    const int P = g.Fout * g.Tout;
    FwdTile r{tile_pt(P), 0, 0.0};
    const int L = g.axis == 0 ? g.Tout : g.Fout, n_in = g.axis == 0 ? g.Tin : g.Fin;
    if (!knobs.tapclass || L < 2) return r;
    auto mask = [&](int o) { unsigned m = 0; for (int t = 0; t < 3; ++t) { const int i = o * g.stride - g.pad + t; if (i >= 0 && i < n_in) m |= 1u << t; } return m; };
    unsigned m0 = 0;
    for (int o = 0; o + 1 < L; ++o) m0 |= mask(o);
    const unsigned m1 = mask(L - 1);
    const int n_all = __builtin_popcount(m0 | m1), n0 = __builtin_popcount(m0), n1 = __builtin_popcount(m1);
    const int64_t c1 = P / L, c0 = (int64_t)c1 * (L - 1);
    const double saved = n_all == 0 ? 0.0 : (double)(c0 * (n_all - n0) + c1 * (n_all - n1)) / ((double)P * n_all);
    if (saved < 0.03) return r;
    int pt = 1;
    while (pt * 2 <= 32 && c0 % (pt * 2) == 0 && c1 % (pt * 2) == 0) pt *= 2;
    const int st = BM / pt, st_def = BM / r.pt;
    const bool fast = st == 4 || st == 8, fast_def = st_def == 4 || st_def == 8;
    if (st < 4 || (fast_def && !fast)) return r;
    r.pt = pt; r.perm = g.axis == 0 ? 2 : 0; r.saved = saved;
    return r;
}

static int dgrad_tile_pt(const ConvGeom& g) {
    const int P = g.Fin * g.Tin;
    int pt = tile_pt(P);
    const int L = g.axis == 0 ? g.Tin : g.Fin;
    if (g.stride == 1 && g.axis == 0 && L == 2 && g.pad == 1) {
        while (pt > 1 && (P / 2) % pt != 0) pt >>= 1;
        return pt;
    }
    if (g.stride != 2 || L < 2) return pt;
    const int c0 = g.pad & 1, n0 = (L - c0 + 1) / 2;
    const int per = P / L;
    const int s0 = per * n0, s1 = per * (L - n0);
    while (pt > 1 && (s0 % pt != 0 || s1 % pt != 0)) pt >>= 1;
    return pt;
}

static int pick_bm(int64_t B, int P, int Cout, const ConvKnobs& knobs) {
    if (knobs.bm256_min_tiles <= 0) return 128;
    const int pt = tile_pt(P), ST = 128 / pt;
    const int64_t n_tiles = ((B + ST - 1) / ST) * ((P + pt - 1) / pt) * (Cout / BN);
    return n_tiles >= knobs.bm256_min_tiles ? 256 : 128;
}

static int pick_bn(int64_t n_tiles128, int Cout, const ConvKnobs& knobs) {
    if (knobs.bn64 == 0 || Cout % 64 != 0) return 128;
    if (knobs.bn64 == 2) return 64;
    return (n_tiles128 < knobs.bn64_tiles && n_tiles128 >= knobs.bn64_min) ? 64 : 128;
}

struct FwdPlan { int BM, pt, perm; };
static FwdPlan fwd_plan(int64_t B, const ConvGeom& g, bool full_epilogue, bool fuse0, bool force128, const ConvKnobs& knobs) {
    const int P = g.Fout * g.Tout;
    FwdPlan r{(fuse0 || force128) ? 128 : pick_bm(B, P, g.Cout, knobs), tile_pt(P), 0};
    if (r.BM == 256 && full_epilogue && 256 / r.pt != 8) r.BM = 128;
    if (full_epilogue && !fuse0) {
        FwdTile ft = fwd_tile(g, r.BM, knobs);
        if (r.BM == 256 && ft.saved == 0.0) {
            const FwdTile f2 = fwd_tile(g, 128, knobs);
            if (f2.saved >= 0.10) { r.BM = 128; ft = f2; }
        }
        r.pt = ft.pt; r.perm = ft.perm;
    }
    return r;
}

static int find_kernel(int BM, int bn, int ring, int epi, int arith, bool fuse0) {
    for (int i = 0; i < conv_kernel_row_count; ++i) {
        const ConvKernelRow& r = conv_kernel_rows[i];
        if (r.BM == BM && r.bn == bn && (ring == 0 || r.ring == ring) && r.epi == epi && r.arith == arith && r.fuse0 == fuse0) return i;
    }
    return -1;
}

ConvPlan plan_conv_gemm(const ConvPlanIn& in, const ConvGeom& g, const ConvKnobs& knobs) {
    ConvPlan pl{};
    pl.rc = NAFP_ERR_UNSUPPORTED;
    const int64_t B = in.B;
    const bool full = !in.plain && !in.dgrad;
    if (g.Cin % 32 != 0 || g.Cout % BN != 0 || B > (1 << 24)) return pl;
    if (in.dgrad && (!in.plain || g.Cout % 32 != 0 || g.Cin % BN != 0 || (g.stride != 1 && g.stride != 2))) return pl;
    const int P = in.dgrad ? g.Fin * g.Tin : g.Fout * g.Tout, N = in.dgrad ? g.Cin : g.Cout;
    const int64_t sample_in = in.dgrad ? (int64_t)g.Fout * g.Tout * g.Cout : (int64_t)g.Fin * g.Tin * g.Cin;
    const int64_t Bp = (in.plan_b > 0 && full && !in.fuse0) ? in.plan_b : B;
    const bool x6 = in.bf16x3 == 2 && full && in.split_weights, x6d = in.bf16x3 == 2 && in.plain && in.dgrad && in.split_weights;
    pl.P = P;
    if (in.dgrad) {
        pl.BM = x6d ? 128 : pick_bm(B, P, N, knobs);
        pl.PT = dgrad_tile_pt(g);
        pl.k_steps = dgrad_k_steps(g);
        const int L = g.axis == 0 ? g.Tin : g.Fin;
        if (g.stride == 2 && L >= 2) {
            pl.perm_on = 1; pl.perm_c0 = g.pad & 1;
            pl.perm_n0 = (L - pl.perm_c0 + 1) / 2;
        } else if (g.stride == 1 && g.axis == 0 && L == 2 && g.pad == 1) {
            pl.perm_on = 2;
        }
    } else {
        const FwdPlan fp = fwd_plan(Bp, g, full, in.fuse0, x6, knobs);
        pl.BM = fp.BM; pl.PT = fp.pt; pl.perm_on = fp.perm;
        pl.k_steps = live_k_steps(g);
    }
    const int BM = pl.BM, ST = pl.ST = BM / pl.PT;
    pl.n_sg = (int)((B + ST - 1) / ST);
    const int n_pb = pl.n_pb = (P + pl.PT - 1) / pl.PT;
    if ((int64_t)ST * sample_in * 4 >= ((int64_t)1 << 31)) return pl;
    const int64_t wbytes = (int64_t)g.Cout * 3 * g.Cin * 4;
    if (wbytes >= ((int64_t)1 << 31)) return pl;
    pl.wp_bytes = (unsigned)wbytes;
    pl.abl = in.plain ? 0 : knobs.abl;
    pl.opt = knobs.gemm_prio;

    const int64_t n_tiles128 = (int64_t)pl.n_sg * n_pb * (N / BN);
    const int64_t n_tiles128_plan = ((Bp + ST - 1) / ST) * n_pb * (N / BN);
    int bn = (BM == 256 || in.fuse0) ? 128 : pick_bn(n_tiles128_plan, N, knobs);
    const PlanOverride ov = (full && !in.fuse0) ? knobs.fwd_plan : in.dgrad ? knobs.dgrad_plan : PlanOverride{};
    const bool forced = BM == 128 && ov.bn > 0 && !in.sizing;
    if (forced && (ov.bn == 128 || N % 64 == 0)) bn = ov.bn;
    const int64_t n_tiles = n_tiles128 * (BN / bn), n_tiles_plan = n_tiles128_plan * (BN / bn);
    const int64_t out_floats = B * P * N;
    int S = 1;
    if (in.slab_floats > 0 && !in.fuse0 && BM == 128) {
        S = choose_split(n_tiles_plan, pl.k_steps, Bp * P * N, bn == 64 ? ((knobs.n64_two_stage && !in.plain) ? 1280.0 : 1024.0) : 768.0, knobs);
        if (forced && ov.S > 0) { S = ov.S; while (S > 1 && pl.k_steps / S < 4) --S; }
        if (in.sizing && ov.S > 0) S = std::max(S, ov.S);
        if (S * out_floats > in.slab_floats) S = 1;
        if (x6 && bn == 64 && S == 2 && (ST == 4 || ST == 8)) S = 1;
    }
    pl.bn = bn; pl.S = S;
    pl.mode = in.plain ? 1 : S > 1 ? 2 : 0;

    const bool in_kernel_finish = knobs.split_inkernel > 0 && S > 1 && !in.plain && bn == 64 && in.tickets && n_tiles_plan >= knobs.split_inkernel &&
                                  (int64_t)n_pb * (N / bn) <= NAFP_TICKET_SLOTS;
    const bool plain_in_kernel = knobs.plain_inkernel > 0 && S > 1 && in.plain && in.tickets && n_tiles <= NAFP_TICKET_SLOTS && !x6d;
    pl.finish = S == 1 ? CONV_FINISH_NONE : in_kernel_finish ? CONV_FINISH_IN_KERNEL_FULL : plain_in_kernel ? CONV_FINISH_IN_KERNEL_PLAIN : CONV_FINISH_KERNEL;
    if (pl.finish == CONV_FINISH_KERNEL && in.plain) {
        pl.finish_grid = (unsigned)std::min<int64_t>((out_floats / 4 + 255) / 256, 8192);
    } else if (pl.finish == CONV_FINISH_KERNEL) {
        const int64_t f4_plan = Bp * P * N / 4;
        pl.finish_f4 = f4_plan >= 1024 * 1024 ? 1024 : f4_plan >= 1024 * 512 ? 512 : 256;
        pl.finish_grid = (unsigned)((out_floats / 4 + pl.finish_f4 - 1) / pl.finish_f4);
    }

    const int n_col = N / bn;
    pl.xcd_group = 1;
    while ((1 << pl.log2_ncol) < n_col) ++pl.log2_ncol;
    const int64_t total_wg = (int64_t)pl.n_sg * n_pb * n_col * S;
    bool xm = knobs.xcdmap != 0 && !in.fuse0 && !in_kernel_finish && !plain_in_kernel && (1 << pl.log2_ncol) == n_col && total_wg < ((int64_t)1 << 31);
    if (xm) {
        const double a_bytes = (double)B * (double)sample_in * 4.0, w_bytes = (double)pl.k_steps * 16.0 * N * 4.0;
        const bool row_fast = knobs.xcdmap == 3 || (knobs.xcdmap == 1 && w_bytes > a_bytes);
        pl.xcd_group = row_fast ? pl.n_sg * n_pb : n_col * S;
        pl.xcd_full = (int)(total_wg / (8 * (int64_t)pl.xcd_group) * (8 * (int64_t)pl.xcd_group));
        if (pl.xcd_group <= 1 || pl.xcd_full == 0) xm = false;
        else pl.opt |= row_fast ? (8 | 16) : 8;
    }
    const bool g3 = !xm && S == 1 && knobs.grid3d != 0 && (knobs.grid3d == 1 || BM == 256 || bn == 128);
    if (g3) pl.opt |= 4;
    pl.grid = xm ? dim3((unsigned)total_wg)
            : g3 ? dim3((unsigned)pl.n_sg, (unsigned)n_pb, (unsigned)n_col)
                 : dim3((unsigned)((int64_t)pl.n_sg * n_pb), (unsigned)n_col, (unsigned)S);
    if (!xm && (n_pb > 65535 || n_col > 65535)) return pl;
    if (in_kernel_finish && n_tiles > NAFP_TICKET_SLOTS) pl.range_step = NAFP_TICKET_SLOTS / ((int64_t)n_pb * n_col) * ST;

    const bool fast_st = ST == 4 || ST == 8;
    int epi, arith = 0;
    if (in.fuse0) {
        const ConvGeom* f0 = in.f0_geom;
        if (in.plain || S != 1 || !f0 || g.axis != 1 || f0->Cout != g.Cin || f0->Tout != g.Tin || f0->Fin != g.Fin || g.Cin % 16 != 0 ||
            in.v_out || !fast_st)
            return pl;
        epi = 0;
        if (in.bf16x3 == 2 && in.split_weights) {
            if (g.Cin != 128) return pl;
            arith = 2;
        }
    } else {
        epi = plain_in_kernel ? 5 : in_kernel_finish ? 4 : pl.mode != 0 ? 3 : !fast_st ? 2 : in.v_out ? 1 : 0;
    }
    const bool two_stage = knobs.n64_two_stage && bn == 64 && (epi == 0 || epi == 1 || epi == 4);
    if (!in.fuse0) {
        const bool ring_ok = bn == 128 || two_stage;
        if (x6) arith = (epi <= 1 ? ring_ok : epi == 2 ? knobs.x6_any : epi == 3 ? bn == 128 : false) ? 2 : 0;
        if (x6d && epi == 3) arith = 2;
        if (!arith && in.bf16x3 && epi == 0 && ring_ok) arith = 1;
    }
    pl.kernel = find_kernel(BM, bn, arith ? 0 : two_stage ? 2 : 3, epi, arith, in.fuse0);
    if (pl.kernel < 0) return pl;
    const ConvKernelRow& row = conv_kernel_rows[pl.kernel];
    pl.lds_bytes = (row.ring * ((BM + bn) * 16 + row.extra_stage_floats) + 2 * BM + 96 + (in.fuse0 ? 4 * g.Cin : 0)) * (int)sizeof(float) + knobs.lds_pad;
    pl.rc = NAFP_OK;
    return pl;
}

int64_t conv_gemm_slab_floats(int64_t B, const ConvGeom& g, bool with_dgrad, int64_t plan_b) {
    ConvPlanIn in{};
    in.B = B; in.plan_b = plan_b; in.slab_floats = INT64_MAX; in.sizing = true;
    const ConvPlan fwd = plan_conv_gemm(in, g, conv_knobs());
    int64_t need = fwd.rc == NAFP_OK && fwd.S > 1 ? (int64_t)fwd.S * B * fwd.P * g.Cout : 0;
    if (with_dgrad) {
        in.plan_b = 0; in.plain = in.dgrad = true;
        const ConvPlan d = plan_conv_gemm(in, g, conv_knobs());
        if (d.rc == NAFP_OK && d.S > 1) need = std::max(need, (int64_t)d.S * B * d.P * g.Cin);
    }
    return need;
}

}
```

### neural-audio-fp_amd/csrc/nafp_common.h

```cpp
#pragma once
#include <hip/hip_runtime.h>
#include <stdint.h>
#include <stdio.h>
#include <stdlib.h>
#include <vector>

#include "../../include/nafp.h"

namespace nafp {

extern thread_local int g_last_hip_error;

#define NAFP_HIP_CHECK(expr)                                   \
    do {                                                       \
        hipError_t _e = (expr);                                \
        if (_e != hipSuccess) {                                \
            nafp::g_last_hip_error = (int)_e;                  \
            return NAFP_ERR_HIP;                               \
        }                                                      \
    } while (0)

#define NAFP_LAUNCH_CHECK() NAFP_HIP_CHECK(hipGetLastError())

constexpr float LN_EPS = 1e-3f;
// ... 42 lines not shown
    if (((uintptr_t)slot & 8) && (unsigned long long)x >= STAT_POISON) return __builtin_nan("");
    return (double)x * (1.0 / (double)(1 << STAT_FRAC_BITS));
}
__device__ __forceinline__ void stat_ln_scalars(const stat_t* sample_slots, double inv_n, float* r, float* c) {
    if (inv_n < 0.0) { const double z = stat_get(sample_slots + 1) * 0.0; *r = (float)(1.0 + z); *c = (float)z; return; }
    const double mean = stat_get(sample_slots) * inv_n;
    double var = stat_get(sample_slots + 1) * inv_n - mean * mean;
    var = var < 0.0 ? 0.0 : var;
    const double rstd = 1.0 / sqrt(var + (double)LN_EPS);
    *r = (float)rstd; *c = (float)(-mean * rstd);
}
__device__ __forceinline__ bool stat_is_poisoned(const stat_t* sample_slots) {
    return (unsigned long long)sample_slots[1] >= STAT_POISON;
}
__device__ __forceinline__ void stat_forward_poison(const stat_t* in_slots, stat_t* out_slots) {
    if (stat_is_poisoned(in_slots)) stat_poison(out_slots);
}
#endif

__device__ __forceinline__ float wave_sum(float v) {
#pragma unroll
    for (int o = 32; o > 0; o >>= 1) v += __shfl_xor(v, o, 64);
    return v;
}
__device__ __forceinline__ double wave_sum(double v) {
#pragma unroll
    for (int o = 32; o > 0; o >>= 1) v += __shfl_xor(v, o, 64);
    return v;
}
__device__ __forceinline__ float wave_max(float v) {
#pragma unroll
    for (int o = 32; o > 0; o >>= 1) v = fmaxf(v, __shfl_xor(v, o, 64));
    return v;
}
__device__ __forceinline__ float wave_min(float v) {
#pragma unroll
    for (int o = 32; o > 0; o >>= 1) v = fminf(v, __shfl_xor(v, o, 64));
    return v;
}

__device__ __forceinline__ void atomic_max_float(float* addr, float v) {
    if (v >= 0.f) atomicMax((int*)addr, __float_as_int(v));
    else          atomicMin((unsigned int*)addr, __float_as_uint(v));
}
__device__ __forceinline__ void atomic_min_float(float* addr, float v) {
    if (v >= 0.f) atomicMin((int*)addr, __float_as_int(v));
    else          atomicMax((unsigned int*)addr, __float_as_uint(v));
}


int launch_conv0(const float* feat, const float* w3, const float* bias, const float* gamma, float* y,
                 float* v_out, stat_t* stats, int64_t B, const ConvGeom& g, hipStream_t st,
                 const float* gstat = nullptr, int group_size = 0, int segment_norm = 0, bool ident_stats = false,
                 bool lean = false);

constexpr int NAFP_TICKET_SLOTS = 4096;
struct ScalarsJob { const float* mr; const double* lnsum; const float* mr_prev; float* sc; long long B; double inv_n; };
struct ConvGemmArgs {
    const float* x;
    const float* wp;
    const float* G;
    const float* Hb;
    const float* gamma_out;
    const float* bias;
    const stat_t* stats_in;
    bool ident_stats;
    stat_t* stats_out;
    float* y;
    float* v_out;
    bool plain;
    bool dgrad;
    float* slab;
    int64_t slab_floats;
    hipEvent_t ev_start, ev_stop;
    const float* wp_hm; const void* wp_l;
    int bf16x3;
    unsigned* tickets;
    const float* f0_feat; const float* f0_w; const float* f0_bias; const float* f0_gamma;
    const ConvGeom* f0_geom;
    const float* f0_gstat; int f0_group, f0_segnorm;
    const ScalarsJob* sj;
    int64_t plan_b;
    int nonmatrix;
};
int launch_conv0_stats(const float* feat, const float* w3, const float* bias, stat_t* stats, int64_t B,
                       const ConvGeom& g, hipStream_t st, const float* gstat = nullptr, int group_size = 0, int segment_norm = 0);
int64_t conv_gemm_slab_floats(int64_t B, const ConvGeom& g, bool with_dgrad = false, int64_t plan_b = 0);
int64_t fwd_plan_b();
int launch_conv_gemm(const ConvGemmArgs& a, int64_t B, const ConvGeom& g, hipStream_t st);


inline int64_t env_int(const char* name, int64_t dflt) { const char* e = getenv(name); return e ? atoll(e) : dflt; }
inline bool env_on(const char* name) { const char* e = getenv(name); return !e || e[0] != '0'; }
struct PlanOverride { int bn = 0, S = 0; };
inline PlanOverride env_plan(const char* name) { PlanOverride r; const char* e = getenv(name); if (e) sscanf(e, "%d:%d", &r.bn, &r.S); return r; }
struct ConvKnobs {
    int64_t bm256_min_tiles = env_int("NAFP_BM256", 2000);
    int bn64 = (int)env_int("NAFP_BN64", 1);
    int64_t bn64_tiles = env_int("NAFP_BN64_TILES", 1000);
    int64_t bn64_min = env_int("NAFP_BN64_MIN", 200);
    bool n64_two_stage = env_on("NAFP_N64S2");
    int splitk = (int)env_int("NAFP_SPLITK", -1);
    int split_inkernel = (int)env_int("NAFP_SPLIT_INKERNEL", 320);
    int plain_inkernel = (int)env_int("NAFP_PLAIN_INKERNEL", 1);
    PlanOverride fwd_plan = env_plan("NAFP_FWD_PLAN");
    PlanOverride dgrad_plan = env_plan("NAFP_DGRAD_PLAN");
    int tapclass = (int)env_int("NAFP_TAPCLASS", 1);
    int64_t plan_b = env_int("NAFP_PLAN_B", 640);
    int grid3d = (int)env_int("NAFP_GRID3D", 1);
    int xcdmap = (int)env_int("NAFP_XCDMAP", 1);
    int gemm_prio = (int)env_int("NAFP_GEMM_PRIO", 0);
    bool x6_any = env_on("NAFP_X6_ANY");
    int abl = (int)env_int("NAFP_ABL", 0);
    int lds_pad = (int)env_int("NAFP_LDS_PAD", 0);
};
const ConvKnobs& conv_knobs();

struct ConvKernelParams;
struct ConvKernelRow {
    void (*fn)(const ConvKernelParams);
    const char* name;
    int BM, bn, ring;
    int extra_stage_floats;
    int epi;
    int arith;
    bool fuse0;
};
extern const ConvKernelRow conv_kernel_rows[];
extern const int conv_kernel_row_count;

enum ConvFinish { CONV_FINISH_NONE = 0, CONV_FINISH_KERNEL = 1, CONV_FINISH_IN_KERNEL_FULL = 2, CONV_FINISH_IN_KERNEL_PLAIN = 3 };
struct ConvPlanIn {
    int64_t B, plan_b;
    bool plain, dgrad, v_out, tickets, split_weights;
    int bf16x3;
    int64_t slab_floats;
    bool fuse0; const ConvGeom* f0_geom;
    bool sizing;
};
struct ConvPlan {
    int rc;
    int kernel;
    int BM, bn, PT, ST;
    int P, n_sg, n_pb;
    int perm_on, perm_n0, perm_c0;
    int k_steps;
    int S;
    int finish;
    int finish_f4; unsigned finish_grid;
    int mode;
    int lds_bytes;
    dim3 grid;
    int opt, xcd_group, xcd_full, log2_ncol;
    int64_t range_step;
    int abl; unsigned wp_bytes;
};
ConvPlan plan_conv_gemm(const ConvPlanIn& in, const ConvGeom& g, const ConvKnobs& k);
int conv_timeline_set(unsigned long long* buf, int64_t capacity_u64, int cin, int cout, int positions);
int conv_timeline_grid(int* out5);

struct DgradLnArgs {
    const float* dts_in; const float* wd;
    const float* t; const float* gamma; const float* G; const float* Hb; const float* sc;
    float* dts_out; float* dgamma; float* dbeta; float* dbias; float* S1; float* S2; double* lnsum_below;
};
bool dgrad_ln_eligible(int64_t B, const ConvGeom& g, int mode);
int launch_dgrad_ln(const DgradLnArgs& a, int64_t B, const ConvGeom& g, hipStream_t st);
int launch_ln_bwd_scalars(const float* mr, const double* lnsum, const float* mr_prev, float* sc, int64_t B, int64_t n, hipStream_t st);

struct TailArgs {
    const float* x;
    const stat_t* stats;
    const float* gamma;
    const float* beta;
    const float* w1p;
    const float* b1p;
    const float* w2p;
    const float* b2;
    float* out_flat;
    float* out_emb;
    int D, Q, S, l2norm;
    bool ident_stats;
    const int* nonfinite_weights;
    const unsigned* launch_error;
};
int launch_tail(const TailArgs& a, int64_t B, hipStream_t st);

struct TailBwdArgs {
    const float* z; const stat_t* stats; const float* gamma; const float* beta;
    bool ident_stats;
    const float* w1; const float* b1; const float* w2; const float* b2;
    const float* w1p; const float* b1p; const float* w2p;
    const float* d_emb;
    float* dy;
    float* ln;
    float* dxh;
    float* dw1; float* db1; float* dw2; float* db2;
    int D, Q, S, l2norm;
};
int launch_tail_bwd(const TailBwdArgs& a, int64_t B, hipStream_t st);
int launch_stats_to_mr(const stat_t* stats, float* mr, const double* inv_n_dev, int64_t B, int n_layers, hipStream_t st, bool identity = false);
int launch_ln_bwd(float* d, const float* tpre, const float* gamma, const float* mr, const float* mr_prev,
                  double* lnsum, float* sc, float* dgamma, float* dbeta, float* dbias, float* S1, float* S2,
                  int64_t B, int P, int C, hipStream_t st, bool reduce_here, const float* Gj, const float* Hbj,
                  double* lnsum_below, const float* feat0 = nullptr, const float* w0 = nullptr, const float* bias0 = nullptr,
                  const ConvGeom* g0 = nullptr, float* dW0 = nullptr, bool scalars_done = false,
                  float* part_slab = nullptr, int64_t part_slab_floats = 0, unsigned* tickets = nullptr, bool tpre_is_z = false);
int launch_wgrad(const float* X, const float* D, float* dW, int64_t B, const ConvGeom& g, hipStream_t st,
                 const float* X2 = nullptr, const float* D2 = nullptr, float* slab = nullptr, int64_t slab_floats = 0,
                 unsigned* tickets = nullptr, const ScalarsJob* sj = nullptr, int prec = 0);
int64_t wgrad_slab_floats(int64_t B, const ConvGeom& g);
int launch_conv0_bwd(const float* feat, const float* dt, float* dW0, float* dbias0, int64_t B, const ConvGeom& g,
                     hipStream_t st);
int launch_pack_dgrad_weight(const float* k3, float* wd, int Cin, int Cout, hipStream_t st);

struct BnExpandTable { const float* gamma_c[16]; const float* beta_c[16]; const float* mmean[16]; const float* mvar[16];
                       float* gamma_pos[16]; int64_t n[16]; int C[16]; int count; };
int launch_bn_expand(const BnExpandTable& t, hipStream_t st);
int launch_bn_param_grad(const float* dgp, const float* dbp, int P, int C, const float* mmean, const float* mvar, float* dgamma_c,
                         float* dbeta_c, hipStream_t st);
int launch_ln1d_fwd(float* x, int64_t rows, int C, const float* gamma_c, const float* beta_c, hipStream_t st);
int launch_ln1d_bwd(float* d, const float* tpre, int64_t rows, int C, const float* gamma_c, float* dgamma_c, float* dbeta_c, hipStream_t st);

struct PackTable { const float* k3[16]; float* wp[16]; float* wd[16]; int cin[16], cout[16]; int unit0[17]; int count;
                   int* nonfinite; };
// ... 22 lines not shown
```

Baseline: 192,100.

## Add eight-wave variant of the f32 plain 128x128 conv GEMM for small grids

Adds a 512-thread (eight-wave) version of the f32 plain-epilogue 128x128 conv GEMM kernel. Each wave now owns a 64x32 sub-tile and issues one A and one B DMA piece per step. The planner picks it when the tile count times the split factor is small (at most 768) and the finish mode is a separate kernel. It is on by default for layers 1-15 through an env knob and a per-layer option mask. The aim is more latency hiding and wave-level parallelism on under-filled grids, at the cost of fewer accumulators per wave and more register and LDS pressure per block.

```diff
diff --git a/include/nafp.h b/include/nafp.h
--- a/include/nafp.h
+++ b/include/nafp.h
@@ -268,6 +268,8 @@
 #define NAFP_PLAN_SIZE_DGRAD 64
 int nafp_conv_plan(int in_f, int in_t, int layer, int64_t n_seg, int64_t plan_b, int flags, int64_t slab_floats,
                    int64_t* record_host, char* kernel_name_host, int name_capacity);
+int nafp_conv_plan_waves(int in_f, int in_t, int layer, int64_t n_seg, int64_t plan_b, int flags, int64_t slab_floats,
+                         char* kernel_name_host, int name_capacity);
 
 int64_t nafp_encoder_train_workspace_bytes(const nafp_encoder* enc, int64_t n_seg);
 int nafp_encoder_forward_train(nafp_encoder* enc, const float* feat, int64_t n_seg, void* workspace,
@@ -290,6 +292,7 @@
 #define NAFP_NONMATRIX_KEEP_OWN 2
 #define NAFP_NONMATRIX_ALL 3
 #define NAFP_NONMATRIX_DEFAULT NAFP_NONMATRIX_ALL
+#define NAFP_OPT_PLAIN8 9
 int nafp_encoder_set_option(nafp_encoder* enc, int option, int value);
 
 int nafp_encoder_div_enc(nafp_encoder* enc, const float* flat, int64_t n_seg,
diff --git a/neural-audio-fp_amd/_lib.py b/neural-audio-fp_amd/_lib.py
--- a/neural-audio-fp_amd/_lib.py
+++ b/neural-audio-fp_amd/_lib.py
@@ -89,6 +89,7 @@
     'nafp_conv_timeline': (c_int, [c_void_p, c_i64, c_int, c_int, c_int]),
     'nafp_conv_timeline_grid': (c_int, [c_void_p]),
     'nafp_conv_plan': (c_int, [c_int, c_int, c_int, c_i64, c_i64, c_int, c_i64, c_void_p, c_void_p, c_int]),
+    'nafp_conv_plan_waves': (c_int, [c_int, c_int, c_int, c_i64, c_i64, c_int, c_i64, c_void_p, c_int]),
     'nafp_encoder_set_option': (c_int, [c_void_p, c_int, c_int]),
     'nafp_encoder_train_workspace_bytes': (c_i64, [c_void_p, c_i64]),
     'nafp_encoder_forward_train': (c_int, [c_void_p, c_void_p, c_i64, c_void_p, c_i64, c_void_p, c_int, c_void_p]),
diff --git a/neural-audio-fp_amd/csrc/api.hip b/neural-audio-fp_amd/csrc/api.hip
--- a/neural-audio-fp_amd/csrc/api.hip
+++ b/neural-audio-fp_amd/csrc/api.hip
@@ -106,6 +106,7 @@
     std::vector<hipEvent_t> prof_events;
     int prof_max = 0, prof_count = 0;
     int opt_nonmatrix = []() { const char* v = getenv("NAFP_NONMATRIX"); return v ? (int)strtol(v, nullptr, 0) & NAFP_NONMATRIX_ALL : NAFP_NONMATRIX_DEFAULT; }();
+    int opt_plain8 = 0xfffe;
     int opt_bf16x3 = 0;
     float* d_x6_blob = nullptr; std::vector<float*> d_whm; std::vector<void*> d_wl; bool x6_dirty = true;
     std::vector<float*> d_wdhm; std::vector<void*> d_wdl;
@@ -347,6 +348,9 @@
         case NAFP_OPT_NONMATRIX:
             if (value < 0 || (value & ~NAFP_NONMATRIX_ALL)) return NAFP_ERR_INVALID_ARG;
             e->opt_nonmatrix = value; return NAFP_OK;
+        case NAFP_OPT_PLAIN8:
+            if (value < 0 || (value & ~0xfffe)) return NAFP_ERR_INVALID_ARG;
+            e->opt_plain8 = value; return NAFP_OK;
         case NAFP_OPT_SMALLNET: return NAFP_OK;
         case NAFP_OPT_DEBUG_SIDE_DELAY:
         case NAFP_OPT_DEBUG_SW_DELAY: {
@@ -644,6 +648,7 @@
         if (a.bf16x3 == 2) { a.wp_hm = e->d_whm[j]; a.wp_l = e->d_wl[j]; }
         a.plan_b = fwd_plan_b();
         a.nonmatrix = e->opt_nonmatrix;
+        a.no_plain8 = !((e->opt_plain8 >> j) & 1);
         if (j == 1 && fuse0) {
             a.x = nullptr; a.f0_feat = feat; a.f0_w = e->d_w[0]; a.f0_bias = e->d_bias[0];
             a.f0_gamma = e->d_gamma[0]; a.f0_geom = &e->geom[0];
@@ -723,15 +728,30 @@
     return conv_timeline_grid(out5_host);
 }
 
-extern "C" int nafp_conv_plan(int in_f, int in_t, int layer, int64_t n_seg, int64_t plan_b, int flags, int64_t slab_floats,
-                              int64_t* record_host, char* kernel_name_host, int name_capacity) {
-    if (in_f <= 0 || in_t <= 0 || layer < 1 || layer > 15 || n_seg <= 0 || plan_b < 0 || slab_floats < 0 || !record_host) return NAFP_ERR_INVALID_ARG;
-    const std::vector<ConvGeom> geom = encoder_geometry(in_f, in_t);
+static ConvPlanIn conv_plan_query(const std::vector<ConvGeom>& geom, int64_t n_seg, int64_t plan_b, int flags, int64_t slab_floats) {
     ConvPlanIn in{};
     in.B = n_seg; in.plan_b = plan_b; in.slab_floats = slab_floats;
     in.plain = flags & NAFP_PLAN_PLAIN; in.dgrad = flags & NAFP_PLAN_DGRAD; in.v_out = flags & NAFP_PLAN_V_OUT; in.tickets = flags & NAFP_PLAN_TICKETS;
     in.split_weights = flags & NAFP_PLAN_SPLIT_WEIGHTS; in.bf16x3 = (flags >> 8) & 3;
     in.fuse0 = flags & NAFP_PLAN_FUSE0; in.f0_geom = in.fuse0 ? &geom[0] : nullptr;
+    return in;
+}
+
+extern "C" int nafp_conv_plan_waves(int in_f, int in_t, int layer, int64_t n_seg, int64_t plan_b, int flags, int64_t slab_floats,
+                                    char* kernel_name_host, int name_capacity) {
+    if (in_f <= 0 || in_t <= 0 || layer < 1 || layer > 15 || n_seg <= 0 || plan_b < 0 || slab_floats < 0) return NAFP_ERR_INVALID_ARG;
+    const std::vector<ConvGeom> geom = encoder_geometry(in_f, in_t);
+    const ConvPlan pl = plan_conv_gemm(conv_plan_query(geom, n_seg, plan_b, flags, slab_floats), geom[layer], conv_knobs());
+    if (pl.rc != NAFP_OK) return pl.rc;
+    if (kernel_name_host && name_capacity > 0) snprintf(kernel_name_host, (size_t)name_capacity, "%s", conv_kernel_rows[pl.kernel_run].name);
+    return pl.waves;
+}
+
+extern "C" int nafp_conv_plan(int in_f, int in_t, int layer, int64_t n_seg, int64_t plan_b, int flags, int64_t slab_floats,
+                              int64_t* record_host, char* kernel_name_host, int name_capacity) {
+    if (in_f <= 0 || in_t <= 0 || layer < 1 || layer > 15 || n_seg <= 0 || plan_b < 0 || slab_floats < 0 || !record_host) return NAFP_ERR_INVALID_ARG;
+    const std::vector<ConvGeom> geom = encoder_geometry(in_f, in_t);
+    const ConvPlanIn in = conv_plan_query(geom, n_seg, plan_b, flags, slab_floats);
     const ConvPlan pl = plan_conv_gemm(in, geom[layer], conv_knobs());
     for (int i = 0; i < NAFP_CONV_PLAN_FIELDS; ++i) record_host[i] = 0;
     record_host[29] = conv_gemm_slab_floats(n_seg, geom[layer], (flags & NAFP_PLAN_SIZE_DGRAD) != 0, plan_b);
diff --git a/neural-audio-fp_amd/csrc/conv.hip b/neural-audio-fp_amd/csrc/conv.hip
--- a/neural-audio-fp_amd/csrc/conv.hip
+++ b/neural-audio-fp_amd/csrc/conv.hip
@@ -478,17 +478,19 @@
 #ifndef NAFP_EXP_SKIP_TAP2
 #define NAFP_EXP_SKIP_TAP2 0
 #endif
-template <int BM, int BNT, int BK, int NSTAGE, bool FUSE0, int EPI, int PREC = 0>
+template <int BM, int BNT, int BK, int NSTAGE, bool FUSE0, int EPI, int PREC = 0, int WN = 2>
 __device__ __forceinline__ bool conv_gemm_body(const ConvKernelParams& p) {
     static_assert(!FUSE0 || (BK == 16 && BM == 128), "the in-kernel conv0 generator is written for BK = 16, BM = 128");
     static_assert(BM == 128 || BM == 256, "tile rows");
     static_assert(BNT == 128 || (BNT == 64 && BM == 128 && !FUSE0), "tile columns");
-    constexpr int NIW = BNT / 64;
-    constexpr int NT = 2 * BM;
-    constexpr int NW = BM / 32;
+    static_assert(WN == 2 || (WN == 4 && BM == 128 && BNT == 128 && BK == 16 && !FUSE0 && EPI == 3 && PREC == 0), "eight waves: the f32 PLAIN 128 x 128 tile");
+    constexpr int NIW = BNT / (32 * WN);
+    constexpr int NW = (BM / 64) * WN;
+    constexpr int NT = 64 * NW;
+    constexpr int AROWS = BM / NW;
     constexpr int CH = BK / 4;
     constexpr int RPI = 64 / CH;
-    constexpr int NI = 32 / RPI;
+    constexpr int NI = AROWS / RPI;
     constexpr int BROWS = BNT / NW;
     constexpr int NIB = BROWS / RPI;
     static_assert(NIB >= 1, "B rows per wave");
@@ -507,7 +509,7 @@
     float* sW0 = sCB + BM + 96;
     const int tid = threadIdx.x, lane = tid & 63;
     const int wave = __builtin_amdgcn_readfirstlane(tid >> 6);
-    const int wm = wave >> 1, wn = wave & 1;
+    const int wm = wave / WN, wn = wave % WN;
     int sg = blockIdx.x, pb = blockIdx.y, colz = blockIdx.z, zsp = 0;
     if (p.opt & 8) {
         const unsigned lin = blockIdx.x, G = (unsigned)p.xcd_group;
@@ -591,7 +593,7 @@
     }
 #pragma unroll
     for (int q = 0; q < NI; ++q) {
-        const int lr = wave * 32 + q * RPI + lane / CH;
+        const int lr = wave * AROWS + q * RPI + lane / CH;
         const int pc = lane % CH;
         const int swz = BK == 32 ? ((lr >> 1) & 7) : ((lr >> 2) & 3);
         const int lc = pc ^ swz;
@@ -674,8 +676,8 @@
     const u32x4 rsA = make_rsrc(p.x + (int64_t)b0 * p.sample_in,
                                 NAFP_ABL(p, 512) ? 0u : (unsigned)nb * (unsigned)p.sample_in * 4u);
     const u32x4 rsB = make_rsrc(PREC == 2 ? p.wp_hm : p.wp, NAFP_ABL(p, 4096) ? 0u : p.wp_bytes);
-    const unsigned lds0 = (unsigned)(unsigned long long)(lds_ptr_t)smem + (unsigned)(wave * 32 * BK * 4);
-    const unsigned ldsB0 = (unsigned)(unsigned long long)(lds_ptr_t)smem + (unsigned)((TILE + wave * BROWS * BK) * 4);
+    const unsigned lds0 = (unsigned)(unsigned long long)(lds_ptr_t)smem + (unsigned)(wave * AROWS * BK * 4);
+    const unsigned ldsB0 =(unsigned)(unsigned long long)(lds_ptr_t)smem + (unsigned)((TILE + wave * BROWS * BK) * 4);
     const u32x4 rsL = make_rsrc((const float*)p.wp_l, NAFP_ABL(p, 4096) ? 0u : p.wp_bytes / 2);
     const unsigned ldsL0 = (unsigned)(unsigned long long)(lds_ptr_t)smem + (unsigned)((TILE + TILEB) * 4 + wave * LROWS * 32);
     const unsigned voffL = (unsigned)((tile_n0 + wave * LROWS + (lane >> 1)) * K) * 2u + (unsigned)(lane & 1) * 16u;
@@ -765,9 +767,9 @@
 
     const int rl = lane & 31, hh = lane >> 5;
     const int rswz = BK == 32 ? ((rl >> 1) & 7) : ((rl >> 2) & 3);
-    const int aoff = (wm * 64 + rl) * BK, boff = TILE + (wn * (BNT / 2) + rl) * BK;
+    const int aoff = (wm * 64 + rl) * BK, boff = TILE + (wn * (BNT / WN) + rl) * BK;
     const int ncol = lane & 31;
-    const int n_base = tile_n0 + wn * (BNT / 2) + ncol;
+    const int n_base = tile_n0 + wn * (BNT / WN) + ncol;
     const int g4 = p.ST >> 2;
     constexpr int MIL = 1;
     float Gv[MIL][4][NIW], Hv[MIL][4][NIW], gv[MIL][4][NIW];
@@ -824,10 +826,11 @@
         NAFP_DMA_TAP()
 #define NAFP_DMA_PIECE(q_, slot_)                                                              \
         {                                                                                      \
-            lds_dma16(lds0 + (unsigned)((slot_) * STAGE * 4) + (q_) * RPI * BK * 4, cur_va[q_], rsA, (unsigned)(d_c0 * 4)); \
-            if ((q_) < NIB) lds_dma16(ldsB0 + (unsigned)((slot_) * STAGE * 4) + (q_) * RPI * BK * 4, voffB[(q_) < NIB ? (q_) : 0], rsB, \
-                                      (unsigned)((d_tap * p.Cin + d_c0) * 4));                 \
-            if ((q_) == NI - 1) { d_c0 += BK; if (d_c0 == p.Cin) { d_c0 = 0; ++d_tsel; NAFP_DMA_TAP() } } \
+            if ((q_) < NI) lds_dma16(lds0 + (unsigned)((slot_) * STAGE * 4) + (q_) * RPI * BK * 4, cur_va[(q_) < NI ? (q_) : 0], rsA, (unsigned)(d_c0 * 4)); \
+            if (NI == 1 ? (q_) == 1 : (q_) < NIB)                                              \
+                lds_dma16(ldsB0 + (unsigned)((slot_) * STAGE * 4) + (NI == 1 ? 0 : (q_)) * RPI * BK * 4, voffB[(NI == 2 && (q_) < NIB) ? (q_) : 0], rsB, \
+                          (unsigned)((d_tap * p.Cin + d_c0) * 4));                             \
+            if ((q_) == 1) { d_c0 += BK; if (d_c0 == p.Cin) { d_c0 = 0; ++d_tsel; NAFP_DMA_TAP() } } \
         }
 #define NAFP_MM_HALF(a_, b_, mi_)                                                              \
         _Pragma("unroll") for (int ni = 0; ni < NIW; ++ni) {                                   \
@@ -836,7 +839,7 @@
             acc[mi_][ni] = __builtin_amdgcn_mfma_f32_32x32x2f32(a_[mi_].z, b_[ni].z, acc[mi_][ni], 0, 0, 0); \
             acc[mi_][ni] = __builtin_amdgcn_mfma_f32_32x32x2f32(a_[mi_].w, b_[ni].w, acc[mi_][ni], 0, 0, 0); \
         }
-        static_assert(NI == 2, "the DMA of a step is issued as two pieces");
+        static_assert(NI == 2 || (NI == 1 && NIB == 1), "the DMA of a step is issued as two pieces");
         if (PREC >= 1) {
             typedef __bf16 bf16x8 __attribute__((ext_vector_type(8)));
             for (int s = s_begin; s < n_steps; ++s) {
@@ -864,7 +867,7 @@
                     for (int ni = 0; ni < NIW; ++ni) {
                         bh[ni] = *(const bf16x8*)(St + boff + ni * 32 * BK + ((hh ^ rswz) * 4));
                         bm[ni] = *(const bf16x8*)(St + boff + ni * 32 * BK + (((2 + hh) ^ rswz) * 4));
-                        bl[ni] = *(const bf16x8*)(St + TILE + TILEB + (wn * (BNT / 2) + ni * 32 + rl) * 8 + hh * 4);
+                        bl[ni] = *(const bf16x8*)(St + TILE + TILEB + (wn * (BNT / WN) + ni * 32 + rl) * 8 + hh * 4);
                     }
                 }
                 if (has_next) { NAFP_DMA_PIECE(0, nslot) NAFP_DMA_L(nslot, d_tap * p.Cin + d_c0) NAFP_DMA_PIECE(1, nslot) }
@@ -976,7 +979,7 @@
         }
         static_assert(PREC != 0 || NSTAGE == 3 || BNT == 64, "the K-loop body is written out once per ring slot (128-column tiles)");
         if (s_begin + 1 < n_steps) {
-            if (BNT == 128) {
+            if (NIW == 2) {
                 for (int s = s_begin + 1;;) {
                     NAFP_K_STEP(1, 0)
                     NAFP_K_STEP(2, 1)
@@ -1067,7 +1070,7 @@
         _Pragma("unroll") for (int ni = 0; ni < NIW; ++ni) {                                   \
             bh[ni] = *(const bf16x8*)((St_) + boff + ni * 32 * BK + ((hh ^ rswz) * 4));        \
             bm[ni] = *(const bf16x8*)((St_) + boff + ni * 32 * BK + (((2 + hh) ^ rswz) * 4));  \
-            bl[ni] = *(const bf16x8*)((St_) + TILE + TILEB + (wn * (BNT / 2) + ni * 32 + rl) * 8 + hh * 4); \
+            bl[ni] = *(const bf16x8*)((St_) + TILE + TILEB + (wn * (BNT / WN) + ni * 32 + rl) * 8 + hh * 4); \
         }
         int s = 0;
         for (; s + 1 < n_steps; ++s) {
@@ -1432,6 +1435,9 @@
 NAFP_GEMM_KERNEL(conv_gemm_m256k16s3_infer, 256, 128, 16, 3, 4, false, 0)
 NAFP_GEMM_KERNEL(conv_gemm_m256k16s3_train, 256, 128, 16, 3, 4, false, 1)
 NAFP_GEMM_KERNEL(conv_gemm_m256k16s3_plain, 256, 128, 16, 3, 4, false, 3)
+__global__ __launch_bounds__(512, 6) void conv_gemm_k16s3_plain8(const ConvKernelParams p) {
+    conv_gemm_body<128, 128, 16, 3, false, 3, 0, 4>(p);
+}
 
 NAFP_GEMM_KERNEL_BF16X3(conv_gemm_k16s3_infer_bf16x3, 128, 128, 3, 3)
 NAFP_GEMM_KERNEL_BF16X3(conv_gemm_m256k16s3_infer_bf16x3, 256, 128, 3, 4)
@@ -1454,7 +1460,8 @@
     conv_gemm_body<128, 128, 16, 2, true, 0, 2>(p);
 }
 
-#define NAFP_ROW(k_, BM_, bn_, ring_, extra_, epi_, arith_, fuse0_) {k_, #k_, BM_, bn_, ring_, extra_, epi_, arith_, fuse0_},
+#define NAFP_ROW(k_, BM_, bn_, ring_, extra_, epi_, arith_, fuse0_) {k_, #k_, BM_, bn_, ring_, extra_, epi_, arith_, fuse0_, (BM_) / 32},
+#define NAFP_ROW_WAVES(k_, BM_, bn_, ring_, extra_, epi_, arith_, fuse0_, waves_) {k_, #k_, BM_, bn_, ring_, extra_, epi_, arith_, fuse0_, waves_},
 const ConvKernelRow conv_kernel_rows[] = {
     NAFP_ROW(conv_gemm_k16s3_infer, 128, 128, 3, 0, 0, 0, false)
     NAFP_ROW(conv_gemm_k16s3_train, 128, 128, 3, 0, 1, 0, false)
@@ -1486,7 +1493,9 @@
     NAFP_ROW(conv_gemm_n64k16s2_any_bf16x6, 128, 64, 2, 64 * 8, 2, 2, false)
     NAFP_ROW(conv_gemm_n64k16s2_plain_bf16x6, 128, 64, 2, 64 * 8, 3, 2, false)
     NAFP_ROW(conv_gemm_k16s2_fuse0_bf16x6, 128, 128, 2, 128 * 8 + 128 * 8, 0, 2, true)
+    NAFP_ROW_WAVES(conv_gemm_k16s3_plain8, 128, 128, 3, 0, 3, 0, false, 8)
 };
+#undef NAFP_ROW_WAVES
 #undef NAFP_ROW
 const int conv_kernel_row_count = (int)(sizeof(conv_kernel_rows) / sizeof(conv_kernel_rows[0]));
 
@@ -1536,9 +1545,9 @@
     NAFP_HIP_CHECK(hipFuncSetAttribute((const void*)row.fn, hipFuncAttributeMaxDynamicSharedMemorySize, lds));
     if (ev_start || ev_stop) {
         void* args[] = {(void*)&p};
-        NAFP_HIP_CHECK(hipExtLaunchKernel((const void*)row.fn, grid, dim3(2 * row.BM), args, (size_t)lds, st, ev_start, ev_stop, 0));
+        NAFP_HIP_CHECK(hipExtLaunchKernel((const void*)row.fn, grid, dim3(64 * row.waves), args, (size_t)lds, st, ev_start, ev_stop, 0));
     } else {
-        row.fn<<<grid, 2 * row.BM, lds, st>>>(p);
+        row.fn<<<grid, 64 * row.waves, lds, st>>>(p);
     }
     NAFP_LAUNCH_CHECK();
     return NAFP_OK;
@@ -1654,10 +1663,10 @@
     ConvPlanIn in{};
     in.B = B; in.plan_b = a.plan_b; in.plain = a.plain; in.dgrad = a.dgrad; in.v_out = a.v_out != nullptr; in.tickets = a.tickets != nullptr;
     in.split_weights = a.wp_hm && a.wp_l; in.bf16x3 = a.bf16x3; in.slab_floats = a.slab ? a.slab_floats : 0;
-    in.fuse0 = a.f0_feat != nullptr; in.f0_geom = a.f0_geom;
+    in.fuse0 = a.f0_feat != nullptr; in.f0_geom = a.f0_geom; in.no_plain8 = a.no_plain8;
     const ConvPlan pl = plan_conv_gemm(in, g, conv_knobs());
     if (pl.rc != NAFP_OK) return pl.rc;
-    const ConvKernelRow& row = conv_kernel_rows[pl.kernel];
+    const ConvKernelRow& row = conv_kernel_rows[pl.kernel_run];
     const bool d = a.dgrad, in_kernel = pl.finish == CONV_FINISH_IN_KERNEL_FULL || pl.finish == CONV_FINISH_IN_KERNEL_PLAIN;
 
     ConvKernelParams p;
diff --git a/neural-audio-fp_amd/csrc/conv_plan.hip b/neural-audio-fp_amd/csrc/conv_plan.hip
--- a/neural-audio-fp_amd/csrc/conv_plan.hip
+++ b/neural-audio-fp_amd/csrc/conv_plan.hip
@@ -129,7 +129,15 @@
 static int find_kernel(int BM, int bn, int ring, int epi, int arith, bool fuse0) {
     for (int i = 0; i < conv_kernel_row_count; ++i) {
         const ConvKernelRow& r = conv_kernel_rows[i];
-        if (r.BM == BM && r.bn == bn && (ring == 0 || r.ring == ring) && r.epi == epi && r.arith == arith && r.fuse0 == fuse0) return i;
+        if (r.BM == BM && r.bn == bn && (ring == 0 || r.ring == ring) && r.epi == epi && r.arith == arith && r.fuse0 == fuse0 && r.waves == BM / 32) return i;
+    }
+    return -1;
+}
+static int find_variant(int base, int waves) {
+    const ConvKernelRow& b = conv_kernel_rows[base];
+    for (int i = 0; i < conv_kernel_row_count; ++i) {
+        const ConvKernelRow& r = conv_kernel_rows[i];
+        if (r.waves == waves && r.BM == b.BM && r.bn == b.bn && r.ring == b.ring && r.epi == b.epi && r.arith == b.arith && r.fuse0 == b.fuse0) return i;
     }
     return -1;
 }
@@ -249,6 +257,12 @@
     pl.kernel = find_kernel(BM, bn, arith ? 0 : two_stage ? 2 : 3, epi, arith, in.fuse0);
     if (pl.kernel < 0) return pl;
     const ConvKernelRow& row = conv_kernel_rows[pl.kernel];
+    pl.waves = row.waves; pl.kernel_run = pl.kernel;
+    if (knobs.plain8 && !in.no_plain8 && full && !in.v_out && pl.mode == 2 && BM == 128 && bn == 128 && arith == 0 && epi == 3 &&
+        pl.finish == CONV_FINISH_KERNEL && n_tiles_plan * S <= 768) {
+        const int v = find_variant(pl.kernel, 8);
+        if (v >= 0) { pl.waves = 8; pl.kernel_run = v; }
+    }
     pl.lds_bytes = (row.ring * ((BM + bn) * 16 + row.extra_stage_floats) + 2 * BM + 96 + (in.fuse0 ? 4 * g.Cin : 0)) * (int)sizeof(float) + knobs.lds_pad;
     pl.rc = NAFP_OK;
     return pl;
diff --git a/neural-audio-fp_amd/csrc/nafp_common.h b/neural-audio-fp_amd/csrc/nafp_common.h
--- a/neural-audio-fp_amd/csrc/nafp_common.h
+++ b/neural-audio-fp_amd/csrc/nafp_common.h
@@ -148,6 +148,7 @@
     const ScalarsJob* sj;
     int64_t plan_b;
     int nonmatrix;
+    bool no_plain8;
 };
 int launch_conv0_stats(const float* feat, const float* w3, const float* bias, stat_t* stats, int64_t B,
                        const ConvGeom& g, hipStream_t st, const float* gstat = nullptr, int group_size = 0, int segment_norm = 0);
@@ -179,6 +180,7 @@
     bool x6_any = env_on("NAFP_X6_ANY");
     int abl = (int)env_int("NAFP_ABL", 0);
     int lds_pad = (int)env_int("NAFP_LDS_PAD", 0);
+    bool plain8 = env_on("NAFP_PLAIN8");
 };
 const ConvKnobs& conv_knobs();
 
@@ -191,6 +193,7 @@
     int epi;
     int arith;
     bool fuse0;
+    int waves;
 };
 extern const ConvKernelRow conv_kernel_rows[];
 extern const int conv_kernel_row_count;
@@ -203,10 +206,12 @@
     int64_t slab_floats;
     bool fuse0; const ConvGeom* f0_geom;
     bool sizing;
+    bool no_plain8;
 };
 struct ConvPlan {
     int rc;
     int kernel;
+    int waves, kernel_run;
     int BM, bn, PT, ST;
     int P, n_sg, n_pb;
     int perm_on, perm_n0, perm_c0;
```

Result: slower. 189,600 (-1.3%).
